# StractOrg/stract

Measured on AMD Instinct MI355X. Metric: HyperBall traversed edges/sec (GTEPS), higher is better.
Workload: dtype u8

## Files before the change

### include/hyperball.h

```cpp
#ifndef HYPERBALL_H
#define HYPERBALL_H

#include <stdint.h>

#ifdef __cplusplus
extern "C" {
#endif

#define HB_ABI_VERSION 6

#define HB_OK 0
#define HB_ERR_INVALID   (-1)
#define HB_ERR_NO_DEVICE (-2)
#define HB_ERR_HIP       (-3)
#define HB_ERR_NOMEM     (-4)
#define HB_ERR_RCCL      (-5)
#define HB_ERR_LIMIT     (-6)
#define HB_ERR_IO        (-7)


typedef struct hb_u128 {
    uint64_t lo;
    uint64_t hi;
} hb_u128;
// ... 258 lines not shown
    uint32_t rounds_run;
    uint64_t with_original;
    uint64_t filled[16];
    uint64_t unknown_orig;
    uint64_t unknown_keys;
    uint64_t no_seed;
    uint64_t seed_without_value;
    uint64_t results;
    uint64_t device_bytes;
    double   ms_total;
    double   ms_seed;
    double   ms_fill;
} hb_nearest_seed_stats;

int hb_nearest_seed(hb_ctx *ctx, const hb_nearest_seed_options *opt, hb_nearest_seed_stats *stats);
int hb_nearest_seed_count(hb_ctx *ctx, uint64_t *count);
int hb_nearest_seed_copy(hb_ctx *ctx, hb_u128 *ids, double *vals, uint64_t cap);
int hb_nearest_seed_all(hb_ctx *ctx, double *vals, uint64_t cap);
int hb_nearest_seed_top(hb_ctx *ctx, uint64_t k, hb_u128 *ids, double *vals, uint64_t *written);
int hb_nearest_seed_seeds(hb_ctx *ctx, hb_u128 *seed, uint8_t *has_seed, uint64_t cap);

int hb_rccl_unique_id(uint8_t out[128]);

#define HB_COLL_U8 0
#define HB_COLL_U32 1
#define HB_COLL_U64 2
#define HB_COLL_F64 3
#define HB_COLL_MAX 0
#define HB_COLL_SUM 1
typedef struct hb_collectives {
    void *user;
    int (*all_reduce)(void *user, void *buf, uint64_t count, int dtype, int op, void *stream);
    int (*all_gather)(void *user, const void *send, void *recv, uint64_t bytes_per_rank, void *stream);
    int (*broadcast)(void *user, void *buf, uint64_t bytes, int root, void *stream);
} hb_collectives;
int hb_set_collectives(hb_ctx *ctx, const hb_collectives *ops);
int hb_debug_staged_copy(void *dst, const void *src, uint64_t bytes, int to_device, void *stream);

int hb_pinned_alloc(uint64_t bytes, void **out);
void hb_pinned_free(void *p);

int hb_device_count(int *count);
int hb_device_name(const hb_ctx *ctx, char *name, uint64_t cap);
int hb_device_synchronize(hb_ctx *ctx);

int hb_debug_copy_registers(hb_ctx *ctx, uint8_t *out );
int hb_debug_copy_kahan(hb_ctx *ctx, double *sum, double *err);
int hb_debug_copy_sizes(hb_ctx *ctx, uint64_t *out);
int hb_debug_hll_size(hb_ctx *ctx, const uint8_t *regs, uint64_t count, uint64_t *out);
int hb_debug_state_hash(hb_ctx *ctx, uint64_t out[2]);
int hb_debug_copy_graph(hb_ctx *ctx, hb_u128 *ids, uint64_t *row_ptr, uint32_t *src);
int hb_debug_copy_plan(hb_ctx *ctx, uint64_t sizes[4], uint32_t *order, uint64_t *plan_row_ptr, uint32_t *plan_src,
                       uint64_t *level_begin);
int hb_debug_exchange(hb_ctx **ctxs, int count, int phase);
int hb_step_local(hb_ctx *ctx);
int hb_step_finish(hb_ctx *ctx, int *has_changes);

int hb_debug_h2d_rate(hb_ctx *ctx, const void *host, uint64_t bytes, int reps, double *gb_per_s);
int hb_debug_set_ingest_limits(hb_ctx *ctx, uint64_t max_records, uint64_t max_device_bytes, uint64_t chunk_records);

int hb_host_ingest(const hb_u128 *node_ids, uint64_t n, const hb_edge *edges, uint64_t m,
                   uint64_t *n_out, uint64_t *m_unique, uint64_t *m_eff, hb_u128 *ids,
                   uint64_t *row_ptr, uint32_t *src);
int hb_host_plan(uint64_t n, const uint64_t *row_ptr, const uint32_t *src, uint32_t flags,
                 uint32_t chunk, const uint32_t *tune , uint64_t sizes[4],
                 uint32_t *order, uint64_t *plan_row_ptr, uint32_t *plan_src, uint64_t *level_begin);
int hb_debug_tail_index(uint64_t n, const hb_u128 *sorted_ids, const uint32_t *dev_of, uint64_t n_pad, const hb_edge *records,
                        uint64_t count, uint64_t *ptr_out, uint32_t *to_out, uint64_t to_cap, uint64_t *to_len);

#ifdef __cplusplus
}
#endif
#endif
```

### stract_amd/_lib.py

```python
import ctypes
import os

os.environ.setdefault("OMP_WAIT_POLICY", "passive")

import numpy as np

_HERE = os.path.dirname(os.path.abspath(__file__))
LIB_PATH = os.environ.get("HB_LIB_PATH") or os.path.join(_HERE, "lib", "libhyperball.so")
LIB_EXP_PATH = os.environ.get("HB_LIB_PATH") or os.path.join(_HERE, "lib", "libhyperball_exp.so")

HB_OK = 0
HB_ERR_INVALID, HB_ERR_NO_DEVICE, HB_ERR_HIP, HB_ERR_NOMEM, HB_ERR_RCCL, HB_ERR_LIMIT, HB_ERR_IO = -1, -2, -3, -4, -5, -6, -7
HB_STORE_F64, HB_STORE_U64 = 0, 1
HB_COLL_U8, HB_COLL_U32, HB_COLL_U64, HB_COLL_F64 = 0, 1, 2, 3
HB_COLL_MAX, HB_COLL_SUM = 0, 1
HB_SKIPPED_REL_MASK = 0x6FED00

HB_FLAG_NO_FRONTIER = 0x01
HB_FLAG_NO_REORDER = 0x02
HB_FLAG_UNFUSED = 0x04
HB_FLAG_PASS_STATS = 0x08
HB_FLAG_NO_XCD_MAP = 0x20
HB_FLAG_NO_RCCL = 0x40
HB_FLAG_RCCL_SELF = 0x80
HB_FLAG_NO_SPARSE = 0x100
HB_FLAG_DEST_PARTITION = 0x200
HB_FLAG_HOST_INGEST = 0x400
HB_FLAG_HOST_PLAN = 0x800
HB_FLAG_CHANGED_ONLY = 0x1000
HB_FLAG_REFERENCE_TAIL = 0x2000
HB_FLAG_NO_INIT_PASS = 0x4000
HB_FLAG_ALL_RELS = 0x8000
HB_SAMPLE_MAX_LEVELS = 16

HB_X_TILE_EPILOGUE = 0x100
HB_X_SEED_3LAUNCH = 0x800
HB_X_NO_EDGE_OVERLAP = 0x1000
HB_X_BITMAP_SLOTWISE = 0x2000
HB_X_NO_STAGED_RESULTS = 0x4000
HB_X_SNAPSHOT_EVERY_PASS = 0x8000
HB_X_SHORT_FINAL_LIST = 0x10000
HB_X_ONE_SNAPSHOT = 0x20000
HB_X_NO_TAIL_PIPELINE = 0x100000
HB_X_TAIL_KERNEL = 0x200000
HB_X_TAIL_KERNEL_ANY = 0x400000
HB_X_FULL_INIT = 0x800000
HB_X_WIRE_64B = 0x1000000
HB_X_SCATTER_TRANSPOSE = 0x2000000
HB_X_SWEEP_ROUNDS = 0x4000000
HB_X_GENERIC_LEVEL1 = 0x8000000
HB_X_PROBE_NO_SIZE = 0x10000000

U128 = np.dtype([("lo", "<u8"), ("hi", "<u8")])
EDGE = np.dtype([("from", U128), ("to", U128), ("rel_flags", "<u8")])
assert U128.itemsize == 16 and EDGE.itemsize == 40


class HbOptions(ctypes.Structure):
    _fields_ = [
        ("struct_size", ctypes.c_uint32),
        ("device", ctypes.c_int32),
        ("flags", ctypes.c_uint32),
        ("chunk", ctypes.c_uint32),
        ("max_passes", ctypes.c_uint32),
        ("rank", ctypes.c_int32),
        ("world_size", ctypes.c_int32),
        ("rccl_id", ctypes.c_uint8 * 128),
        ("tune", ctypes.c_uint32 * 8),
    ]


class HbStats(ctypes.Structure):
    _fields_ = [
        ("n", ctypes.c_uint64),
        ("m_input", ctypes.c_uint64),
        ("m_unique", ctypes.c_uint64),
        ("m_eff", ctypes.c_uint64),
        ("passes", ctypes.c_uint64),
        ("results", ctypes.c_uint64),
        ("ms_ingest", ctypes.c_double),
        ("ms_plan", ctypes.c_double),
        ("ms_h2d", ctypes.c_double),
        ("ms_loop", ctypes.c_double),
        ("ms_loop_gpu", ctypes.c_double),
        ("ms_collective", ctypes.c_double),
        ("ms_d2h", ctypes.c_double),
        ("work_rows", ctypes.c_uint64),
        ("virtual_rows", ctypes.c_uint64),
        ("device_bytes", ctypes.c_uint64),
        ("virtual_edges", ctypes.c_uint64),
        ("levels", ctypes.c_uint64),
        ("level1_edges", ctypes.c_uint64),
        ("level1_rows", ctypes.c_uint64),
        ("direct_edges", ctypes.c_uint64),
        ("rows_with_in_edges", ctypes.c_uint64),
        ("wire_bytes", ctypes.c_uint64),
        ("ingest_peak_bytes", ctypes.c_uint64),
        ("pool_peak_bytes", ctypes.c_uint64),
        ("result_stages", ctypes.c_uint64),
        ("result_list", ctypes.c_uint64),
        ("pipelined_passes", ctypes.c_uint64),
        ("tail_kernel_passes", ctypes.c_uint64),
    ]

# ... 221 lines not shown
        return d


_P = ctypes.c_void_p
_U64 = ctypes.c_uint64
_SIGNATURES = [
    ("hb_abi_version", ctypes.c_int, []),
    ("hb_release_cached_memory", ctypes.c_int, [ctypes.c_void_p]),
    ("hb_create", ctypes.c_int, [ctypes.POINTER(HbOptions), ctypes.POINTER(_P)]),
    ("hb_destroy", None, [_P]),
    ("hb_last_error", ctypes.c_char_p, [_P]),
    ("hb_load_edges", ctypes.c_int, [_P, _P, _U64, _P, _U64]),
    ("hb_append_edges", ctypes.c_int, [_P, _P, _U64]),
    ("hb_finalize", ctypes.c_int, [_P, _P, _U64]),
    ("hb_discard_appended", ctypes.c_int, [_P]),
    ("hb_load_tail_edges", ctypes.c_int, [_P, _P, _U64]),
    ("hb_append_tail_edges", ctypes.c_int, [_P, _P, _U64]),
    ("hb_tail_segment_end", ctypes.c_int, [_P]),
    ("hb_debug_set_ingest_limits", ctypes.c_int, [_P, _U64, _U64, _U64]),
    ("hb_set_collectives", ctypes.c_int, [_P, _P]),
    ("hb_debug_staged_copy", ctypes.c_int, [_P, _P, _U64, ctypes.c_int, _P]),
    ("hb_pinned_alloc", ctypes.c_int, [_U64, ctypes.POINTER(ctypes.c_void_p)]),
    ("hb_pinned_free", None, [ctypes.c_void_p]),
    ("hb_debug_h2d_rate", ctypes.c_int, [_P, _P, _U64, ctypes.c_int, ctypes.POINTER(ctypes.c_double)]),
    ("hb_debug_tail_index", ctypes.c_int, [_U64, _P, _P, _U64, _P, _U64, _P, _P, _U64, ctypes.POINTER(ctypes.c_uint64)]),
    ("hb_load_dense", ctypes.c_int, [_P, _P, _U64, _P, _P, _U64]),
    ("hb_run", ctypes.c_int, [_P, ctypes.POINTER(HbStats)]),
    ("hb_begin", ctypes.c_int, [_P]),
    ("hb_step", ctypes.c_int, [_P, ctypes.POINTER(ctypes.c_int)]),
    ("hb_finish", ctypes.c_int, [_P]),
    ("hb_get_stats", ctypes.c_int, [_P, ctypes.POINTER(HbStats)]),
    ("hb_get_pass_stats", ctypes.c_int, [_P, _U64, ctypes.POINTER(HbPassStats)]),
    ("hb_result_count", ctypes.c_int, [_P, ctypes.POINTER(_U64)]),
    ("hb_result_copy", ctypes.c_int, [_P, _P, _P, _U64]),
    ("hb_result_ranks", ctypes.c_int, [_P, _P, _U64]),
    ("hb_result_top", ctypes.c_int, [_P, _U64, _P, _P, ctypes.POINTER(ctypes.c_uint64)]),
    ("hb_rccl_unique_id", ctypes.c_int, [_P]),
    ("hb_device_count", ctypes.c_int, [ctypes.POINTER(ctypes.c_int)]),
    ("hb_device_name", ctypes.c_int, [_P, ctypes.c_char_p, _U64]),
    ("hb_device_synchronize", ctypes.c_int, [_P]),
    ("hb_debug_copy_registers", ctypes.c_int, [_P, _P]),
    ("hb_debug_copy_kahan", ctypes.c_int, [_P, _P, _P]),
    ("hb_debug_copy_sizes", ctypes.c_int, [_P, _P]),
    ("hb_debug_hll_size", ctypes.c_int, [_P, _P, _U64, _P]),
    ("hb_debug_state_hash", ctypes.c_int, [_P, _P]),
    ("hb_debug_copy_graph", ctypes.c_int, [_P, _P, _P, _P]),
    ("hb_debug_copy_plan", ctypes.c_int, [_P, _P, _P, _P, _P, _P]),
    ("hb_debug_exchange", ctypes.c_int, [_P, ctypes.c_int, ctypes.c_int]),
    ("hb_step_local", ctypes.c_int, [_P]),
    ("hb_step_finish", ctypes.c_int, [_P, ctypes.POINTER(ctypes.c_int)]),
    ("hb_host_ingest", ctypes.c_int, [_P, _U64, _P, _U64, ctypes.POINTER(_U64), ctypes.POINTER(_U64),
                                      ctypes.POINTER(_U64), _P, _P, _P]),
    ("hb_host_plan", ctypes.c_int, [_U64, _P, _P, ctypes.c_uint32, ctypes.c_uint32, _P, _P, _P, _P, _P, _P]),
]
_SIGNATURES += [
    ("hbw_open", ctypes.c_int, [ctypes.c_char_p, ctypes.c_uint32, ctypes.POINTER(_P)]),
    ("hbw_close", None, [_P]),
    ("hbw_last_error", ctypes.c_char_p, [_P]),
    ("hbw_num_segments", ctypes.c_int, [_P, ctypes.POINTER(_U64)]),
    ("hbw_segment_info", ctypes.c_int, [_P, _U64, ctypes.c_char_p, ctypes.POINTER(_U64)]),
    ("hbw_total_rows", ctypes.c_int, [_P, ctypes.POINTER(_U64)]),
    ("hbw_read_host_edges", ctypes.c_int, [_P, _U64, _U64, _P]),
    ("hbw_read_page_edges", ctypes.c_int, [_P, _U64, _U64, _P]),
    ("hb_load_webgraph", ctypes.c_int, [_P, ctypes.c_char_p, ctypes.c_uint32]),
    ("hbw_debug_sstable", ctypes.c_int, [_P, _U64, ctypes.c_int, _P, _U64, _P, _U64, ctypes.POINTER(_U64)]),
    ("hbw_debug_crc32", ctypes.c_uint32, [_P, _U64]),
]
_SIGNATURES += [
    ("hbu_create", ctypes.c_int, [ctypes.c_int32, _U64, ctypes.POINTER(_P)]),
    ("hbu_destroy", None, [_P]),
    ("hbu_last_error", ctypes.c_char_p, [_P]),
    ("hbu_len", ctypes.c_int, [_P, ctypes.POINTER(_U64)]),
    ("hbu_batch_set", ctypes.c_int, [_P, _P, _P, _U64]),
    ("hbu_batch_get", ctypes.c_int, [_P, _P, _U64, _P, _P]),
    ("hbu_batch_upsert", ctypes.c_int, [_P, _P, _P, _U64, _P]),
    ("hbu_create_kind", ctypes.c_int, [ctypes.c_int32, _U64, ctypes.c_uint32, ctypes.POINTER(_P)]),
    ("hbu_kind", ctypes.c_int, [_P, ctypes.POINTER(ctypes.c_uint32), ctypes.POINTER(ctypes.c_uint32)]),
    ("hbu_batch_set_values", ctypes.c_int, [_P, _P, _P, _U64]),
    ("hbu_batch_get_values", ctypes.c_int, [_P, _P, _U64, _P, _P]),
    ("hbu_batch_upsert_values", ctypes.c_int, [_P, ctypes.c_uint32, _P, _P, _U64, _P]),
    ("hbu_wave_group_length", ctypes.c_uint32, []),
    ("hbu_clone", ctypes.c_int, [_P, ctypes.POINTER(_P)]),
    ("hbu_update_centralities", ctypes.c_int, [_P, _P, _P, _P, _P, _U64, _U64, ctypes.POINTER(_U64)]),
    ("hbu_update_counters", ctypes.c_int, [_P, _P, _P, _P, _U64, _P]),
    ("hbu_update_distances", ctypes.c_int, [_P, _P, _P, _P, _U64, _P, _P, ctypes.POINTER(_U64)]),
    ("hbu_graph_create", ctypes.c_int, [ctypes.c_int32, _P, _U64, _P, _P, _U64, _U64, ctypes.POINTER(_P)]),
    ("hbu_graph_len", ctypes.c_int, [_P, ctypes.POINTER(_U64), ctypes.POINTER(_U64)]),
    ("hbu_graph_destroy", None, [_P]),
    ("hbu_bloom_num_bits", _U64, [_U64, ctypes.c_double]),
    ("hbu_filter_create", ctypes.c_int, [ctypes.c_int32, ctypes.c_uint32, _U64, ctypes.POINTER(_P)]),
    ("hbu_filter_destroy", None, [_P]),
    ("hbu_filter_clear", ctypes.c_int, [_P]),
    ("hbu_filter_fill", ctypes.c_int, [_P]),
    ("hbu_filter_insert", ctypes.c_int, [_P, _P, _U64]),
    ("hbu_filter_contains", ctypes.c_int, [_P, _P, _U64, _P]),
    ("hbu_filter_union", ctypes.c_int, [_P, _P]),
    ("hbu_filter_count", ctypes.c_int, [_P, ctypes.POINTER(_U64)]),
    ("hbu_filter_export_bits", ctypes.c_int, [_P, _P]),
    ("hbu_filter_import_bits", ctypes.c_int, [_P, _P]),
    ("hbu_filter_export_ids", ctypes.c_int, [_P, _P, _U64, ctypes.POINTER(_U64)]),
    ("hbu_setup_counters", ctypes.c_int, [_P, _P, _P, _P]),
    ("hbu_round_counters", ctypes.c_int, [_P, _P, _P, _P, _P, ctypes.POINTER(_U64), ctypes.POINTER(_U64), ctypes.POINTER(_U64)]),
    ("hbu_round_distances", ctypes.c_int, [_P, _P, _P, _P, _P, ctypes.POINTER(_U64), ctypes.POINTER(_U64)]),
    ("hbu_round_centralities", ctypes.c_int, [_P, _P, _P, _P, _P, _P, _U64, ctypes.POINTER(_U64), ctypes.POINTER(_U64)]),
    ("hbu_export", ctypes.c_int, [_P, _P, _P, _U64, ctypes.POINTER(_U64)]),
    ("hbu_fold_harmonic", ctypes.c_int, [_P, _P, ctypes.c_double, ctypes.c_uint32, ctypes.POINTER(_U64), ctypes.POINTER(_U64)]),
# ... 542 lines not shown
        if rc != HB_OK:
            raise HyperballError(rc, err.value.decode(errors="replace"))

    def top(self, k):
        cnt = ctypes.c_uint64(0)
        self._check(self.lib.hb_result_count(self.h, ctypes.byref(cnt)))
        k = min(int(k), cnt.value)
        ids = np.zeros(k, dtype=U128)
        vals = np.zeros(k, dtype=np.float64)
        w = ctypes.c_uint64(0)
        self._check(self.lib.hb_result_top(self.h, k, _ptr(ids), _ptr(vals), ctypes.byref(w)))
        return ids[:w.value], vals[:w.value]

    def n(self):
        return self.stats()["n"]

    def registers(self):
        out = np.zeros((self.n(), 64), dtype=np.uint8)
        self._check(self.lib.hb_debug_copy_registers(self.h, _ptr(out)))
        return out

    def kahan(self):
        n = self.n()
        s = np.zeros(n, dtype=np.float64)
        e = np.zeros(n, dtype=np.float64)
        self._check(self.lib.hb_debug_copy_kahan(self.h, _ptr(s), _ptr(e)))
        return s, e

    def sizes(self):
        out = np.zeros(self.n(), dtype=np.uint64)
        self._check(self.lib.hb_debug_copy_sizes(self.h, _ptr(out)))
        return out

    def state_hash(self):
        out = np.zeros(2, dtype=np.uint64)
        self._check(self.lib.hb_debug_state_hash(self.h, _ptr(out)))
        return int(out[0]), int(out[1])

    def hll_size(self, regs):
        regs = np.ascontiguousarray(regs, dtype=np.uint8).reshape(-1, 64)
        out = np.zeros(len(regs), dtype=np.uint64)
        self._check(self.lib.hb_debug_hll_size(self.h, _ptr(regs), len(regs), _ptr(out)))
        return out

    def plan(self):
        sizes = np.zeros(4, dtype=np.uint64)
        self._check(self.lib.hb_debug_copy_plan(self.h, _ptr(sizes), None, None, None, None))
        n_pad, nv, slen, levels = (int(x) for x in sizes)
        order = np.zeros(n_pad, dtype=np.uint32)
        prp = np.zeros(n_pad + nv + 1, dtype=np.uint64)
        psrc = np.zeros(slen, dtype=np.uint32)
        lb = np.zeros(levels + 1, dtype=np.uint64)
        self._check(self.lib.hb_debug_copy_plan(self.h, _ptr(sizes), _ptr(order), _ptr(prp), _ptr(psrc), _ptr(lb)))
        return dict(order=order, row_ptr=prp, src=psrc, level_begin=lb, n_pad=n_pad, nv=nv)

    def graph(self):
        st = self.stats()
        ids = np.zeros(st["n"], dtype=U128)
        row_ptr = np.zeros(st["n"] + 1, dtype=np.uint64)
        src = np.zeros(st["m_eff"], dtype=np.uint32)
        self._check(self.lib.hb_debug_copy_graph(self.h, _ptr(ids), _ptr(row_ptr), _ptr(src)))
        return ids, row_ptr, src


def rccl_unique_id():
    buf = (ctypes.c_uint8 * 128)()
    rc = load().hb_rccl_unique_id(buf)
    if rc != HB_OK:
        raise HyperballError(rc, (load().hb_last_error(None) or b"").decode())
    return bytes(buf)


def host_ingest(edges, node_ids=None):
    lib = load()
    edges = np.ascontiguousarray(edges, dtype=EDGE)
    nn = 0
    if node_ids is not None:
        node_ids = np.ascontiguousarray(node_ids, dtype=U128)
        nn = len(node_ids)
    n, mu, me = ctypes.c_uint64(0), ctypes.c_uint64(0), ctypes.c_uint64(0)
    rc = lib.hb_host_ingest(_ptr(node_ids), nn, _ptr(edges), len(edges), ctypes.byref(n), ctypes.byref(mu),
                            ctypes.byref(me), None, None, None)
    if rc != HB_OK:
        raise HyperballError(rc, (lib.hb_last_error(None) or b"").decode())
    ids = np.zeros(n.value, dtype=U128)
    row_ptr = np.zeros(n.value + 1, dtype=np.uint64)
    src = np.zeros(me.value, dtype=np.uint32)
    rc = lib.hb_host_ingest(_ptr(node_ids), nn, _ptr(edges), len(edges), ctypes.byref(n), ctypes.byref(mu),
                            ctypes.byref(me), _ptr(ids), _ptr(row_ptr), _ptr(src))
    if rc != HB_OK:
        raise HyperballError(rc, (lib.hb_last_error(None) or b"").decode())
    return ids, row_ptr, src, mu.value


def host_plan(row_ptr, src, flags=0, chunk=0, tune=()):
    lib = load()
    row_ptr = np.ascontiguousarray(row_ptr, dtype=np.uint64)
    src = np.ascontiguousarray(src, dtype=np.uint32)
    n = len(row_ptr) - 1
    sizes = np.zeros(4, dtype=np.uint64)
    tn = np.zeros(8, dtype=np.uint32)
    tn[:len(tune)] = tune
    rc = lib.hb_host_plan(n, _ptr(row_ptr), _ptr(src), flags, chunk, _ptr(tn), _ptr(sizes), None, None, None, None)
    if rc != HB_OK:
        raise HyperballError(rc, (lib.hb_last_error(None) or b"").decode())
    n_pad, nv, slen, levels = (int(x) for x in sizes)
    order = np.zeros(n_pad, dtype=np.uint32)
    prp = np.zeros(n_pad + nv + 1, dtype=np.uint64)
    psrc = np.zeros(slen, dtype=np.uint32)
    lb = np.zeros(levels + 1, dtype=np.uint64)
    rc = lib.hb_host_plan(n, _ptr(row_ptr), _ptr(src), flags, chunk, _ptr(tn), _ptr(sizes), _ptr(order), _ptr(prp),
                          _ptr(psrc), _ptr(lb))
    if rc != HB_OK:
        raise HyperballError(rc, (lib.hb_last_error(None) or b"").decode())
    world = int(tn[7]) if tn[7] > 1 else 1
    if world == 1:
        order = order[:n]
    return dict(order=order, row_ptr=prp, src=psrc, level_begin=lb, n_pad=n_pad, nv=nv, slice=n_pad // world)
```

### stract_amd/csrc/hb_api.hip

```cpp
#include "hb_guard_alloc.h"
#include "hb_pool.h"
#include <hip/hip_runtime.h>
#include <rccl/rccl.h>

#include <algorithm>
#include <cmath>
#include <cstdio>
#include <cstring>
#include <string>
#include <thread>
#include <vector>

#include "hb_internal.h"
#include "hb_experiments.h"
#include "hb_kernels.hip.h"
#include "hb_walk.hip.h"
#include "hb_sample.hip.h"
#include "hb_bfs.hip.h"
#include "hb_betweenness.hip.h"
#include "hb_similarity.hip.h"
#include "hb_nearest_seed.hip.h"
#ifdef HB_EXPERIMENTS
#include "hb_experiments.hip.h"
#endif
// ... 18 lines not shown
    {
        reset(o.release());
        return *this;
    }
    DevPtr(const DevPtr &) = delete;
    DevPtr &operator=(const DevPtr &) = delete;
    ~DevPtr() { reset(); }
    T *get() const { return p; }
    explicit operator bool() const { return p != nullptr; }
    T *release()
    {
        T *q = p;
        p = nullptr;
        return q;
    }
    void reset(T *q = nullptr)
    {
        if (p) (void)hipFree(p);
        p = q;
    }
    hipError_t alloc(size_t count)
    {
        reset();
        return hipMalloc((void **)&p, count * sizeof(T));
    }

private:
    T *p = nullptr;
};

struct OwnedCsr {
    DeviceCsr d;
    OwnedCsr() = default;
    OwnedCsr(OwnedCsr &&o) noexcept : d(o.d) { o.d = DeviceCsr{}; }
    OwnedCsr(const OwnedCsr &) = delete;
    OwnedCsr &operator=(const OwnedCsr &) = delete;
    ~OwnedCsr() { reset(); }
    void reset()
    {
        for (void *q : {(void *)d.d_row_ptr, (void *)d.d_src, (void *)d.d_id_lo})
            if (q) (void)hipFree(q);
        d = DeviceCsr{};
    }
};
}

struct GraphDeviceState {
    uint64_t *d_row_ptr = nullptr;
    uint32_t *d_src = nullptr;
    uint16_t *d_src_jp = nullptr;
    bool level0_all_real = false;
    uint32_t *d_virt_rows = nullptr;
    uint16_t *d_self_jp = nullptr;
    uint4 *d_regs[2] = {nullptr, nullptr};
    uint4 *d_part = nullptr;
    uint32_t *d_bits[2] = {nullptr, nullptr};
    uint32_t *d_kdirty = nullptr;
    double *d_ksum = nullptr, *d_kerr = nullptr;
    uint64_t *d_size = nullptr;
    uint64_t *d_idlow = nullptr;
    uint32_t *d_dev_of = nullptr;
    uint32_t *d_sid_of = nullptr;
    uint32_t *d_outdeg = nullptr;
    unsigned long long *d_counters = nullptr;
    double *d_raw = nullptr, *d_bias = nullptr;
    uint8_t *d_lc = nullptr;
    uint64_t *d_out_ptr = nullptr;
    uint32_t *d_out_rows = nullptr;
    uint32_t *d_touch = nullptr;
    uint32_t *d_seeds = nullptr, *d_heavy = nullptr;
    unsigned int *d_sparse_counts = nullptr;
    bool sparse_ok = false;
    uint4 *d_pack = nullptr;
    uint32_t *d_wpop = nullptr;
    uint64_t *d_wprefix = nullptr;
    uint32_t *d_lbits = nullptr, *d_lbits_all = nullptr, *d_ubits = nullptr;
    bool ubits_valid = false;
    unsigned long long *d_rank_cnt = nullptr;
    uint32_t *d_tl_changed[2] = {nullptr, nullptr}, *d_tl_vchanged[2] = {nullptr, nullptr}, *d_tl_dirty[2] = {nullptr, nullptr};
    uint32_t *d_tl_work = nullptr, *d_tl_count = nullptr;
    bool tl_valid = false;
    uint64_t *d_tail_ptr = nullptr;
    uint32_t *d_tail_to = nullptr;
    uint64_t tail_count = 0;
    std::vector<uint64_t> tail_keys;
    std::vector<TailDoc> tail_open;
    bool tail_dirty = false;
    TailIndex *tail_index = nullptr;
    uint32_t *d_bloom = nullptr;
    unsigned long long *d_bloom_ones = nullptr;
    uint32_t *d_list = nullptr;
    double *d_out = nullptr;
    double *h_out = nullptr;
    uint64_t h_out_len = 0;
    uint64_t out_len = 0;
    uint32_t *d_cid_of = nullptr;
    std::vector<uint64_t> h_in_bits;
    struct ResultSync {
        bool on = false;
        bool valid = false;
        uint64_t changed_since = 0;
        uint32_t stages = 0;
        double *d_sent = nullptr;
        uint32_t *d_sid = nullptr;
        double *d_val = nullptr;
        unsigned long long *d_count = nullptr;
// ... 241 lines not shown
    for (void *q : {(void *)c->h_out, (void *)c->rs.h_sid, (void *)c->rs.h_val, (void *)c->rs.h_count})
        if (q) (void)hipHostFree(q);
    tail_index_free(c->tail_index);
    static_cast<GraphDeviceState &>(*c) = GraphDeviceState{};
    c->stats.device_bytes = 0;
}

template <class T>
void copy_in(const T *from, T *to)
{
    if (from) std::memcpy(to, from, from->struct_size ? std::min<size_t>(from->struct_size, sizeof(T)) : sizeof(T));
}
template <class T>
void copy_out(T *to, T &from)
{
    if (!to) return;
    const size_t sz = to->struct_size ? std::min<size_t>(to->struct_size, sizeof(T)) : sizeof(T);
    from.struct_size = (uint32_t)sz;
    std::memcpy(to, &from, sz);
}

int refuse_stale_error(hb_ctx *c, const char *who)
{
    const hipError_t stale = hipGetLastError();
    if (stale != hipSuccess) return fail(c, HB_ERR_HIP, std::string("stale HIP error before ") + who + ": " + hipGetErrorString(stale));
    return HB_OK;
}

bool find_sid(const hb_ctx *c, const hb_u128 &id, uint32_t *sid)
{
    const auto it = std::lower_bound(c->g.ids.begin(), c->g.ids.end(), id, u128_less);
    if (it == c->g.ids.end() || !u128_eq(*it, id)) return false;
    *sid = (uint32_t)(it - c->g.ids.begin());
    return true;
}

int plan_rows_word_aligned(hb_ctx *c, const char *who)
{
    const Plan &p = c->plan;
    if (p.n_pad % 32 || std::any_of(p.level_begin.begin(), p.level_begin.end(), [](uint64_t b) { return b % 32 != 0; }))
        return fail(c, HB_ERR_INVALID, std::string(who) + ": unexpected plan layout (a level does not begin on a 32-row word)");
    return HB_OK;
}

PlanTune plan_tune(uint32_t chunk, const uint32_t *tune)
{
    PlanTune t;
    t.chunk = chunk ? chunk : kDefaultChunk;
    if (tune) {
        if (tune[3] == 1) t.band_w = 0;
        else if (tune[3] >= 4 && tune[3] < 31) t.band_w = 1u << tune[3];
        if (tune[4]) t.minc = tune[4];
        if (tune[5]) t.direct_max = tune[5];
    }
    return t;
}

bool multi_rank(const hb_ctx *c) { return c->opt.world_size > 1; }
bool xbit(const hb_ctx *c, uint32_t bits) { return (HB_XBITS(c->opt.tune[1]) & bits) != 0; }
unsigned grid_blocks(const hb_ctx *c, uint64_t groups, uint64_t per_cu, uint64_t floor = 0)
{
    return (unsigned)std::max<uint64_t>(std::min<uint64_t>(groups, (uint64_t)c->num_cu * per_cu), floor);
}
bool linked(const hb_ctx *c) { return c->comm != nullptr || c->coll.all_reduce != nullptr; }

#define HB_COLL(call)                 \
    do {                              \
        const int rc_coll_ = (call);  \
        if (rc_coll_) return rc_coll_; \
    } while (0)
int coll_dtype(ncclDataType_t dt) { return dt == ncclUint8 ? HB_COLL_U8 : dt == ncclUint32 ? HB_COLL_U32 : dt == ncclUint64 ? HB_COLL_U64 : HB_COLL_F64; }
uint64_t coll_size(ncclDataType_t dt) { return dt == ncclUint8 ? 1 : dt == ncclUint32 ? 4 : 8; }
int coll_all_reduce(hb_ctx *c, void *buf, uint64_t count, ncclDataType_t dt, ncclRedOp_t op, hipStream_t s)
{
    if (c->comm) {
        HB_NCCL(ncclAllReduce(buf, buf, count, dt, op, c->comm, s));
        return HB_OK;
    }
    if (c->coll.all_reduce(c->coll.user, buf, count, coll_dtype(dt), op == ncclMax ? HB_COLL_MAX : HB_COLL_SUM, (void *)s))
        return fail(c, HB_ERR_RCCL, "the caller's all_reduce (hb_set_collectives) failed");
    return HB_OK;
}
int coll_all_gather(hb_ctx *c, const void *send, void *recv, uint64_t count, ncclDataType_t dt, hipStream_t s)
{
    if (c->comm) {
        HB_NCCL(ncclAllGather(send, recv, count, dt, c->comm, s));
        return HB_OK;
    }
    if (c->coll.all_gather(c->coll.user, send, recv, count * coll_size(dt), (void *)s))
        return fail(c, HB_ERR_RCCL, "the caller's all_gather (hb_set_collectives) failed");
    return HB_OK;
}
int coll_broadcast(hb_ctx *c, void *buf, uint64_t count, ncclDataType_t dt, int root, hipStream_t s)
{
    if (c->comm) {
        HB_NCCL(ncclBroadcast(buf, buf, count, dt, root, c->comm, s));
        return HB_OK;
    }
    if (c->coll.broadcast(c->coll.user, buf, count * coll_size(dt), root, (void *)s))
        return fail(c, HB_ERR_RCCL, "the caller's broadcast (hb_set_collectives) failed");
    return HB_OK;
}
int coll_group_start(hb_ctx *c)
{
    if (c->comm) HB_NCCL(ncclGroupStart());
    return HB_OK;
// ... 965 lines not shown
```

### stract_amd/csrc/hb_api_debug.inc

```
int hb_debug_copy_registers(hb_ctx *c, uint8_t *out)
{
    return guarded(c, [&]() -> int {
        if (!c || !out) return HB_ERR_INVALID;
        if (c->rows != RowsOf::HyperBall) return fail(c, HB_ERR_INVALID, "call hb_begin first");
        int rc = set_device(c);
        if (rc) return rc;
        if ((rc = ensure_initial_state(c))) return rc;
        const uint64_t n = c->plan.n;
        if (!n) return HB_OK;
        DevPtr<uint4> tmp;
        HB_HIP(tmp.alloc(n * 4));
        unsigned blocks = (unsigned)((n * 4 + 255) / 256);
        hipLaunchKernelGGL(hbk::gather_rows_kernel, dim3(blocks), dim3(256), 0, c->stream, (const uint4 *)c->d_regs[c->cur],
                           (const uint32_t *)c->d_dev_of, n, tmp.get());
        HB_HIP_AS("", hipMemcpyAsync(out, tmp.get(), n * 64, hipMemcpyDeviceToHost, c->stream));
        HB_HIP_AS("", hipStreamSynchronize(c->stream));
        return HB_OK;
    });
}

int hb_debug_copy_kahan(hb_ctx *c, double *sum, double *err)
{
    return guarded(c, [&]() -> int {
        if (!c) return HB_ERR_INVALID;
// ... 83 lines not shown
        hipLaunchKernelGGL(hbk::state_hash_kernel, dim3(blocks), dim3(256), 0, c->stream, (const uint4 *)c->d_regs[c->cur],
                           (const double *)c->d_ksum, (const double *)c->d_kerr, (const uint32_t *)c->d_dev_of, n, cnt);
        HB_HIP(hipGetLastError());
        std::vector<unsigned long long> h(hbk::kCounterWords);
        HB_HIP(hipMemcpyAsync(h.data(), cnt, hbk::kCounterWords * sizeof(unsigned long long), hipMemcpyDeviceToHost, c->stream));
        HB_HIP(hipStreamSynchronize(c->stream));
        for (int s = 0; s < hbk::kStripes; s++) {
            out[0] += h[4 * s];
            out[1] += h[4 * s + 1];
        }
        if (multi_rank(c)) out[1] = 0;
        return HB_OK;
    });
}

int hb_debug_copy_graph(hb_ctx *c, hb_u128 *ids, uint64_t *row_ptr, uint32_t *src)
{
    return guarded(c, [&]() -> int {
        if (!c) return HB_ERR_INVALID;
        if (!c->loaded) return fail(c, HB_ERR_INVALID, "no graph loaded");
        const uint64_t n = c->g.ids.size();
        if ((row_ptr || src) && c->g.row_ptr.size() != n + 1)
            return fail(c, HB_ERR_LIMIT, "the reduced graph is kept on the host only up to 2^26 edges (or with HB_FLAG_HOST_PLAN)");
        if (ids && n) std::memcpy(ids, c->g.ids.data(), n * sizeof(hb_u128));
        if (row_ptr) std::memcpy(row_ptr, c->g.row_ptr.data(), (n + 1) * sizeof(uint64_t));
        if (src && !c->g.src.empty()) std::memcpy(src, c->g.src.data(), c->g.src.size() * sizeof(uint32_t));
        return HB_OK;
    });
}

int hb_debug_copy_plan(hb_ctx *c, uint64_t sizes[4], uint32_t *order, uint64_t *plan_row_ptr, uint32_t *plan_src, uint64_t *level_begin)
{
    return guarded(c, [&]() -> int {
        if (!c || !sizes) return HB_ERR_INVALID;
        if (!c->loaded) return fail(c, HB_ERR_INVALID, "no graph loaded");
        int rc = set_device(c);
        if (rc) return rc;
        const Plan &p = c->plan;
        const uint64_t rows_total = p.n_pad + p.nv;
        sizes[0] = p.n_pad;
        sizes[1] = p.nv;
        sizes[2] = c->plan_entries;
        sizes[3] = p.level_begin.size() ? p.level_begin.size() - 1 : 0;
        if (order && p.n_pad) HB_HIP(hipMemcpyAsync(order, c->d_sid_of, p.n_pad * sizeof(uint32_t), hipMemcpyDeviceToHost, c->stream));
        if (plan_row_ptr) HB_HIP(hipMemcpyAsync(plan_row_ptr, c->d_row_ptr, (rows_total + 1) * sizeof(uint64_t), hipMemcpyDeviceToHost, c->stream));
        if (plan_src && c->plan_entries)
            HB_HIP(hipMemcpyAsync(plan_src, c->d_src, c->plan_entries * sizeof(uint32_t), hipMemcpyDeviceToHost, c->stream));
        HB_HIP(hipStreamSynchronize(c->stream));
        if (level_begin) std::memcpy(level_begin, p.level_begin.data(), p.level_begin.size() * sizeof(uint64_t));
        return HB_OK;
    });
}

int hb_host_ingest(const hb_u128 *node_ids, uint64_t n, const hb_edge *edges, uint64_t m, uint64_t *n_out,
                   uint64_t *m_unique, uint64_t *m_eff, hb_u128 *ids, uint64_t *row_ptr, uint32_t *src)
{
    return guarded(nullptr, [&]() -> int {
        hb_ctx *c = nullptr;
        DenseGraph g;
        std::string e = ingest_edges(node_ids, n, edges, m, &g);
        if (!e.empty()) return fail(c, HB_ERR_INVALID, e);
        const uint64_t nn = g.ids.size();
        if (n_out) *n_out = nn;
        if (m_unique) *m_unique = g.m_unique;
        if (m_eff) *m_eff = g.src.size();
        if (ids && nn) std::memcpy(ids, g.ids.data(), nn * sizeof(hb_u128));
        if (row_ptr) std::memcpy(row_ptr, g.row_ptr.data(), (nn + 1) * sizeof(uint64_t));
        if (src && !g.src.empty()) std::memcpy(src, g.src.data(), g.src.size() * sizeof(uint32_t));
        return HB_OK;
    });
}

int hb_host_plan(uint64_t n, const uint64_t *row_ptr, const uint32_t *src, uint32_t flags, uint32_t chunk,
                 const uint32_t *tune, uint64_t sizes[4], uint32_t *order, uint64_t *plan_row_ptr, uint32_t *plan_src,
                 uint64_t *level_begin)
{
    return guarded(nullptr, [&]() -> int {
        hb_ctx *c = nullptr;
        if (!sizes || (n && !row_ptr)) return fail(c, HB_ERR_INVALID, "NULL argument");
        std::vector<uint32_t> outdeg;
        const bool reorder = !(flags & HB_FLAG_NO_REORDER);
        static const uint64_t zero = 0;
        if (n == 0) row_ptr = &zero;
        if (reorder) count_out_degree(row_ptr, src, n, &outdeg);
        Plan p;
        PlanTune pt = plan_tune(chunk, tune);
        if (tune && tune[7] > 1) pt.world = tune[7];
        pt.xcd_map = !(flags & HB_FLAG_NO_XCD_MAP);
        std::string e = build_plan(n, row_ptr, src, outdeg, reorder, pt, &p);
        if (!e.empty()) return fail(c, HB_ERR_LIMIT, e);
        sizes[0] = p.n_pad;
        sizes[1] = p.nv;
        sizes[2] = p.src.size();
        sizes[3] = p.level_begin.size() ? p.level_begin.size() - 1 : 0;
        if (order && p.n_pad) std::memcpy(order, p.order.data(), p.n_pad * sizeof(uint32_t));
        if (plan_row_ptr) std::memcpy(plan_row_ptr, p.row_ptr.data(), p.row_ptr.size() * sizeof(uint64_t));
        if (plan_src && !p.src.empty()) std::memcpy(plan_src, p.src.data(), p.src.size() * sizeof(uint32_t));
        if (level_begin) std::memcpy(level_begin, p.level_begin.data(), p.level_begin.size() * sizeof(uint64_t));
        return HB_OK;
    });
}

int hb_debug_tail_index(uint64_t n, const hb_u128 *sorted_ids, const uint32_t *dev_of, uint64_t n_pad, const hb_edge *records,
                        uint64_t count, uint64_t *ptr_out, uint32_t *to_out, uint64_t to_cap, uint64_t *to_len)
{
    return guarded(nullptr, [&]() -> int {
        hb_ctx *c = nullptr;
        if ((n && (!sorted_ids || !dev_of)) || (count && !records) || !ptr_out || !to_len) return fail(c, HB_ERR_INVALID, "NULL argument");
        TailIndex *tix = n ? tail_index_build(sorted_ids, n) : nullptr;
        std::vector<uint64_t> keys, ptr;
        std::vector<uint32_t> to;
        std::vector<TailDoc> open;
        std::string e = tail_collect(tix, n, records, count, &open);
        if (e.empty()) e = tail_close_segment(tix, sorted_ids, dev_of, &open, &keys);
        tail_index_free(tix);
        if (e.empty()) e = build_tail_csr(&keys, n_pad, &ptr, &to);
        if (!e.empty()) return fail(c, HB_ERR_NOMEM, e);
        std::memcpy(ptr_out, ptr.data(), (n_pad + 1) * sizeof(uint64_t));
        *to_len = to.size();
        if (to_out && !to.empty()) std::memcpy(to_out, to.data(), std::min<uint64_t>(to.size(), to_cap) * sizeof(uint32_t));
        return HB_OK;
    });
}

int hb_debug_exchange(hb_ctx **ctxs, int count, int phase)
{
    return guarded(nullptr, [&]() -> int {
        if (!ctxs || count < 1 || !ctxs[0]) return HB_ERR_INVALID;
        hb_ctx *c = ctxs[0];
        for (int i = 0; i < count; i++) {
            hb_ctx *o = ctxs[i];
            if (!o) return fail(c, HB_ERR_INVALID, "NULL context");
            if (o->plan.n_pad != c->plan.n_pad || o->device != c->device || dest_mode(o) != dest_mode(c))
                return fail(c, HB_ERR_INVALID, "contexts differ in size, device or partition mode");
            if (phase == 0 && !o->pending_local)
                return fail(c, HB_ERR_INVALID, "every context must be between hb_step_local and hb_step_finish");
            if (dest_mode(c) && (o->opt.rank != i || o->opt.world_size != count))
                return fail(c, HB_ERR_INVALID, "destination partition: ctxs[i] must be rank i of `count`");
        }
        int rc = set_device(c);
        if (rc) return rc;
        for (int i = 0; i < count; i++) HB_HIP(hipStreamSynchronize(ctxs[i]->stream));
        const Plan &p = c->plan;
        const uint64_t S = c->slice_rows;
        if (phase == 1) {
            if (!dest_mode(c)) return HB_OK;
            for (int i = 0; i < count; i++)
                for (int j = 0; j < count; j++)
                    if (i != j && S)
                        HB_HIP(hipMemcpyAsync(ctxs[i]->d_ksum + (uint64_t)j * S, ctxs[j]->d_ksum + (uint64_t)j * S, S * sizeof(double),
                                              hipMemcpyDeviceToDevice, c->stream));
// ... 92 lines not shown
```

### stract_amd/csrc/hb_api_load.inc

```
bool device_plan(const hb_ctx *c) { return !(c->opt.flags & HB_FLAG_HOST_PLAN); }
bool deferred_times(const hb_ctx *c);

int keep_owned(hb_ctx *c, DeviceCsr *csr)
{
    if (!dest_mode(c)) return HB_OK;
    const uint64_t world = (uint64_t)std::max(c->opt.world_size, 1), rank = (uint64_t)c->opt.rank, n = c->g.ids.size();
    if (c->g.row_ptr.size() == n + 1 && n) keep_owned_rows(&c->g, world, rank);
    if (csr && csr->d_row_ptr) {
        const std::string e = gpu_keep_owned_rows((void *)c->stream, csr, n, world, rank);
        if (!e.empty()) return fail(c, e.find("memory") != std::string::npos ? HB_ERR_NOMEM : HB_ERR_HIP, e);
    }
    return HB_OK;
}

__global__ __launch_bounds__(256) void idlow_kernel(const uint64_t *lo_by_sid, const uint32_t *order, uint64_t n_pad, uint64_t *idlow)
{
    const uint64_t d = (uint64_t)blockIdx.x * 256 + threadIdx.x;
    if (d >= n_pad) return;
    const uint32_t s = order[d];
    idlow[d] = s == kNone ? 0ull : lo_by_sid[s];
}

template <class T>
T *adopt(hb_ctx *c, DevPtr<T> &b, size_t bytes)
// ... 72 lines not shown
    c->rows = RowsOf::Nobody;
    c->image = Image::None;
    c->run_open = false;
    free_graph_buffers(c);
    c->stats.n = n;
    c->stats.m_input = c->g.m_input;
    c->stats.m_unique = c->g.m_unique;
    c->stats.m_eff = m_eff;
    double t0 = now_ms();
    const bool on_device = device_plan(c);
    c->rs.on = n && !multi_rank(c) && !linked(c) && !ref_tail(c) && !xbit(c, HB_X_NO_STAGED_RESULTS) && (n >= (1u << 20) || xbit(c, HB_X_SNAPSHOT_EVERY_PASS));
    c->rs.cap = c->rs.on ? (xbit(c, HB_X_SHORT_FINAL_LIST) ? 16 : n / 8 + 4096) : 0;
    HostResultBuffers hostbuf;
    hostbuf.start(c->device, n, c->rs.cap);
    if (!in.d.d_row_ptr) in.reset();
    if (!on_device && n && c->g.row_ptr.size() != n + 1) {
        try {
            c->g.row_ptr.resize(n + 1);
            c->g.src.resize(m_eff);
        } catch (const std::bad_alloc &) {
            return fail(c, HB_ERR_NOMEM, "out of host memory for the reduced graph");
        }
        HB_HIP(hipMemcpyAsync(c->g.row_ptr.data(), in.d.d_row_ptr, (n + 1) * sizeof(uint64_t), hipMemcpyDeviceToHost, c->stream));
        if (m_eff) HB_HIP(hipMemcpyAsync(c->g.src.data(), in.d.d_src, m_eff * sizeof(uint32_t), hipMemcpyDeviceToHost, c->stream));
        HB_HIP(hipStreamSynchronize(c->stream));
    }
    if (n && !in.d.d_src) {
        HB_HIP(hipMalloc((void **)&in.d.d_src, std::max<uint64_t>(m_eff, 1) * sizeof(uint32_t)));
        if (m_eff) HB_HIP(hipMemcpyAsync(in.d.d_src, c->g.src.data(), m_eff * sizeof(uint32_t), hipMemcpyHostToDevice, c->stream));
        if (on_device) {
            HB_HIP(hipMalloc((void **)&in.d.d_row_ptr, (n + 1) * sizeof(uint64_t)));
            HB_HIP(hipMemcpyAsync(in.d.d_row_ptr, c->g.row_ptr.data(), (n + 1) * sizeof(uint64_t), hipMemcpyHostToDevice, c->stream));
        }
        in.d.m = m_eff;
    }
    bool reorder = !(c->opt.flags & HB_FLAG_NO_REORDER);
    if (multi_rank(c) && !linked(c)) reorder = false;
    DevPtr<uint64_t> d_lo(in.d.d_id_lo);
    in.d.d_id_lo = nullptr;
    DevPtr<uint32_t> d_deg;
    if (n) {
        HB_HIP(d_deg.alloc(n));
        HB_HIP(hipMemsetAsync(d_deg.get(), 0, n * sizeof(uint32_t), c->stream));
        if (m_eff) {
            const unsigned blocks = grid_blocks(c, (m_eff + 255) / 256, 16);
            hipLaunchKernelGGL(hbk::histogram_kernel, dim3(blocks), dim3(256), 0, c->stream, (const uint32_t *)in.d.d_src, m_eff, d_deg.get());
            HB_HIP(hipGetLastError());
        }
        if (linked(c)) HB_COLL(coll_all_reduce(c, d_deg.get(), n, ncclUint32, ncclSum, c->stream));
    }
    PlanTune pt = plan_tune(c->opt.chunk, c->opt.tune);
    pt.xcd_map = !(c->opt.flags & HB_FLAG_NO_XCD_MAP);
    if (dest_mode(c)) pt.world = (uint32_t)std::max(c->opt.world_size, 1);
    {
        const uint64_t w = pt.world > 1 ? pt.world : 1;
        const uint64_t n_pad_pre = (((n + w - 1) / w + kRowAlign - 1) / kRowAlign * kRowAlign) * w;
        int rc0;
        if ((rc0 = dev_alloc(c, &c->d_regs[0], n_pad_pre * 4))) return rc0;
        if ((rc0 = dev_alloc(c, &c->d_regs[1], n_pad_pre * 4))) return rc0;
    }
    std::vector<uint32_t> outdeg;
    DevicePlan dp;
    DevPtr<uint64_t> dp_row_ptr;
    DevPtr<uint32_t> dp_src, dp_order, dp_dev_of, dp_outdeg;
    if (on_device) {
        std::string perr = gpu_build_plan((void *)c->stream, n, in.d.d_row_ptr, in.d.d_src, d_deg.get(), reorder, pt, &c->plan, &dp);
        dp_row_ptr.reset(dp.d_row_ptr); dp_src.reset(dp.d_src); dp_order.reset(dp.d_order); dp_dev_of.reset(dp.d_dev_of); dp_outdeg.reset(dp.d_outdeg_dev);
        if (!perr.empty()) {
            (void)hipGetLastError();
            return fail(c, perr.find("memory") != std::string::npos ? HB_ERR_NOMEM : (perr.find("exhausted") != std::string::npos ? HB_ERR_LIMIT : HB_ERR_HIP), perr);
        }
    } else {
        outdeg.assign(n, 0);
        if (n) {
            HB_HIP(hipMemcpyAsync(outdeg.data(), d_deg.get(), n * sizeof(uint32_t), hipMemcpyDeviceToHost, c->stream));
            HB_HIP(hipStreamSynchronize(c->stream));
        }
        static const uint64_t zero = 0;
        std::string perr = build_plan(n, n ? c->g.row_ptr.data() : &zero, c->g.src.data(), outdeg, reorder, pt, &c->plan);
        if (!perr.empty()) return fail(c, perr.find("memory") != std::string::npos ? HB_ERR_NOMEM : HB_ERR_LIMIT, perr);
    }
    in.reset();
    c->stats.ms_plan = now_ms() - t0;
    const Plan &p = c->plan;
    const uint64_t rows_total = p.n_pad + p.nv;
    const uint64_t src_len = on_device ? dp.src_len : p.src.size();
    c->plan_entries = src_len;
    c->stats.work_rows = rows_total;
    c->stats.virtual_rows = p.nv;
    c->stats.levels = p.level_begin.size() > 1 ? p.level_begin.size() - 1 : 0;
    c->stats.level1_edges = p.level1_edges;
    c->stats.level1_rows = p.level1_rows;
    c->stats.direct_edges = p.direct_edges;
    c->stats.rows_with_in_edges = p.rows_with_in_edges;

    t0 = now_ms();
    const bool trace_state = std::getenv("HB_TRACE_INGEST") != nullptr;
    double t_lap = t0;
    auto lap = [&](const char *what) {
        if (!trace_state) return;
        (void)hipStreamSynchronize(c->stream);
        std::fprintf(stderr, "[hb state] %-34s %8.1f ms\n", what, now_ms() - t_lap);
        t_lap = now_ms();
    };
    c->bits_words = (rows_total + 31) / 32 + 2;
    int rc;
    if (on_device) {
        c->d_row_ptr = adopt(c, dp_row_ptr, (rows_total + 2) * sizeof(uint64_t));
        c->d_src = adopt(c, dp_src, (src_len + 4) * sizeof(uint32_t));
        c->d_sid_of = adopt(c, dp_order, std::max<uint64_t>(p.n_pad, 64) * sizeof(uint32_t));
        c->d_dev_of = adopt(c, dp_dev_of, std::max<uint64_t>(n, 64) * sizeof(uint32_t));
        c->d_outdeg = adopt(c, dp_outdeg, std::max<uint64_t>(p.n_pad, 64) * sizeof(uint32_t));
        c->m_global = dp.m_global;
    } else {
        if ((rc = dev_alloc(c, &c->d_row_ptr, rows_total + 1))) return rc;
        if ((rc = dev_alloc(c, &c->d_src, src_len + 4))) return rc;
        if ((rc = dev_alloc(c, &c->d_dev_of, n))) return rc;
        if ((rc = dev_alloc(c, &c->d_sid_of, p.n_pad))) return rc;
        if ((rc = dev_alloc(c, &c->d_outdeg, p.n_pad))) return rc;
    }
    if ((rc = dev_alloc(c, &c->d_part, p.nv * 4))) return rc;
    if ((rc = dev_alloc(c, &c->d_bits[0], c->bits_words))) return rc;
    if ((rc = dev_alloc(c, &c->d_bits[1], c->bits_words))) return rc;
    if ((rc = dev_alloc(c, &c->d_kdirty, p.n_pad / 32 + 2))) return rc;
    const uint64_t world = linked(c) ? (uint64_t)c->opt.world_size : 1;
    c->slice_rows = dest_mode(c) ? p.slice : ((p.n_pad + world - 1) / world + 63) / 64 * 64;
    c->ksum_len = std::max<uint64_t>(c->slice_rows * (dest_mode(c) ? (uint64_t)std::max(c->opt.world_size, 1) : world), p.n_pad);
    if ((rc = dev_alloc(c, &c->d_ksum, c->ksum_len))) return rc;
    if ((rc = dev_alloc(c, &c->d_kerr, p.n_pad))) return rc;
    if ((rc = dev_alloc(c, &c->d_size, p.n_pad))) return rc;
    if ((rc = dev_alloc(c, &c->d_idlow, p.n_pad))) return rc;
    if ((rc = dev_alloc(c, &c->d_counters, ((size_t)c->max_passes + 1) * hbk::kCounterWords))) return rc;
    if ((rc = dev_alloc(c, &c->d_raw, HLL64_TABLE_LEN))) return rc;
    if ((rc = dev_alloc(c, &c->d_bias, HLL64_TABLE_LEN))) return rc;
    if ((rc = dev_alloc(c, &c->d_lc, 68))) return rc;
    if ((rc = dev_alloc(c, &c->d_out, n))) return rc;
    if (c->rs.on) {
        if ((rc = dev_alloc(c, &c->rs.d_sent, p.n_pad))) return rc;
        if ((rc = dev_alloc(c, &c->rs.d_sid, c->rs.cap))) return rc;
        if ((rc = dev_alloc(c, &c->rs.d_val, c->rs.cap))) return rc;
        if ((rc = dev_alloc(c, &c->rs.d_count, 2))) return rc;
        if ((rc = dev_alloc(c, &c->rs.d_kept, hbk::kCounterWords))) return rc;
    }
    if (deferred_times(c)) {
        while (c->ev_pool.size() < 32) {
            hb_ctx::EvSet es{};
            for (auto &e : es.e)
                if (hipEventCreate(&e) != hipSuccess) return fail(c, HB_ERR_HIP, "hipEventCreate failed");
            c->ev_pool.push_back(es);
        }
    }

    lap("allocations");
    uint8_t lc[68];
    if (!build_lc_table(lc)) return fail(c, HB_ERR_INVALID, "host libm log() too close to a rounding boundary for the linear-counting table");
    HB_HIP(hipMemcpyAsync(c->d_raw, HLL64_RAW_ESTIMATE, sizeof(HLL64_RAW_ESTIMATE), hipMemcpyHostToDevice, c->stream));
    HB_HIP(hipMemcpyAsync(c->d_bias, HLL64_BIAS, sizeof(HLL64_BIAS), hipMemcpyHostToDevice, c->stream));
    HB_HIP(hipMemcpyAsync(c->d_lc, lc, 68, hipMemcpyHostToDevice, c->stream));
    if (!on_device) {
        c->stats.virtual_edges = p.row_ptr.empty() ? 0 : p.row_ptr[rows_total] - p.row_ptr[p.n_pad];
        HB_HIP(hipMemcpyAsync(c->d_row_ptr, p.row_ptr.data(), (rows_total + 1) * sizeof(uint64_t), hipMemcpyHostToDevice, c->stream));
        if (!p.src.empty())
            HB_HIP(hipMemcpyAsync(c->d_src, p.src.data(), p.src.size() * sizeof(uint32_t), hipMemcpyHostToDevice, c->stream));
        if (p.n_pad)
            HB_HIP(hipMemcpyAsync(c->d_sid_of, p.order.data(), p.n_pad * sizeof(uint32_t), hipMemcpyHostToDevice, c->stream));
        std::vector<uint32_t> outdeg_dev(p.n_pad, 0);
        c->m_global = 0;
        for (uint64_t d = 0; d < p.n_pad; d++)
            if (p.order[d] != kNone) {
                outdeg_dev[d] = outdeg[p.order[d]];
                c->m_global += outdeg[p.order[d]];
            }
        if (p.n_pad)
            HB_HIP(hipMemcpyAsync(c->d_outdeg, outdeg_dev.data(), p.n_pad * sizeof(uint32_t), hipMemcpyHostToDevice, c->stream));
        if (n) HB_HIP(hipMemcpyAsync(c->d_dev_of, p.dev_of.data(), n * sizeof(uint32_t), hipMemcpyHostToDevice, c->stream));
        HB_HIP(hipStreamSynchronize(c->stream));
    } else {
        uint64_t ends[2] = {0, 0};
        HB_HIP(hipMemcpyAsync(&ends[0], c->d_row_ptr + p.n_pad, sizeof(uint64_t), hipMemcpyDeviceToHost, c->stream));
        HB_HIP(hipMemcpyAsync(&ends[1], c->d_row_ptr + rows_total, sizeof(uint64_t), hipMemcpyDeviceToHost, c->stream));
        HB_HIP(hipStreamSynchronize(c->stream));
        c->stats.virtual_edges = ends[1] - ends[0];
    }
    lap("tables / plan arrays");
    c->out_len = n;
    c->d_cid_of = c->d_sid_of;
    if (c->rs.on && n) {
        DevPtr<uint32_t> d_flags;
        DevPtr<uint64_t> d_cpos;
        DevPtr<unsigned long long> d_words;
        const uint64_t nw = (n + 63) / 64;
        HB_HIP(d_flags.alloc(n + 1));
        HB_HIP(d_cpos.alloc(n + 2));
        HB_HIP(d_words.alloc(nw));
        if ((rc = dev_alloc(c, &c->d_cid_of, p.n_pad))) return rc;
        HB_HIP(hipMemsetAsync(d_flags.get(), 0, (n + 1) * sizeof(uint32_t), c->stream));
        const unsigned blocks = grid_blocks(c, (p.n_pad + 255) / 256, 16);
        hipLaunchKernelGGL(hbk::in_flags_kernel, dim3(blocks), dim3(256), 0, c->stream, (const uint64_t *)c->d_row_ptr, (const uint32_t *)c->d_sid_of, p.n_pad, d_flags.get());
        HB_HIP(hipGetLastError());
        const std::string e = device_prefix((void *)c->stream, d_flags.get(), n, d_cpos.get());
        if (!e.empty()) return fail(c, HB_ERR_HIP, e);
        hipLaunchKernelGGL(hbk::cid_of_kernel, dim3(blocks), dim3(256), 0, c->stream, (const uint64_t *)c->d_row_ptr, (const uint32_t *)c->d_sid_of,
                           (const uint64_t *)d_cpos.get(), p.n_pad, c->d_cid_of);
        HB_HIP(hipGetLastError());
        hipLaunchKernelGGL(hbk::pack_flags_kernel, dim3(grid_blocks(c, (nw + 3) / 4, 16)), dim3(256), 0, c->stream,
                           (const uint32_t *)d_flags.get(), n, d_words.get());
        HB_HIP(hipGetLastError());
        uint64_t n_c = 0;
        c->h_in_bits.assign(nw, 0);
        HB_HIP(hipMemcpyAsync(&n_c, d_cpos.get() + n, sizeof(uint64_t), hipMemcpyDeviceToHost, c->stream));
        HB_HIP(hipMemcpyAsync(c->h_in_bits.data(), d_words.get(), nw * sizeof(uint64_t), hipMemcpyDeviceToHost, c->stream));
        HB_HIP(hipStreamSynchronize(c->stream));
        if (n_c != p.rows_with_in_edges)
            return fail(c, HB_ERR_INVALID, "result image: " + std::to_string(n_c) + " nodes with in-edges counted on the device, the plan says " + std::to_string(p.rows_with_in_edges));
        c->out_len = n_c;
        lap("compact result image (cid per row, host bitmap)");
    }
    if (n) {
        if (!d_lo) {
            uvec<uint64_t> lo(n);
            host_gather_id_lo(c->g.ids.data(), n, lo.data());
            HB_HIP(d_lo.alloc(n));
            HB_HIP(hipMemcpyAsync(d_lo.get(), lo.data(), n * sizeof(uint64_t), hipMemcpyHostToDevice, c->stream));
            HB_HIP(hipStreamSynchronize(c->stream));
        }
        hipLaunchKernelGGL(idlow_kernel, dim3((unsigned)((p.n_pad + 255) / 256)), dim3(256), 0, c->stream, (const uint64_t *)d_lo.get(),
                           (const uint32_t *)c->d_sid_of, p.n_pad, c->d_idlow);
        HB_HIP(hipGetLastError());
        HB_HIP(hipStreamSynchronize(c->stream));
    }
    lap("id_low");
    if (src_len && !(c->opt.flags & HB_FLAG_NO_INIT_PASS)) {
        if ((rc = dev_alloc(c, &c->d_src_jp, src_len + 4))) return rc;
        const unsigned blocks = grid_blocks(c, (src_len + 255) / 256, 16);
        if ((rc = dev_alloc(c, &c->d_self_jp, p.n_pad + 4))) return rc;
        hipLaunchKernelGGL(hbk::self_jp_kernel, dim3(grid_blocks(c, (p.n_pad + 255) / 256, 16)), dim3(256), 0, c->stream,
                           (const uint64_t *)c->d_idlow, (const uint32_t *)c->d_sid_of, p.n_pad, c->d_self_jp);
        HB_HIP(hipGetLastError());
        hipLaunchKernelGGL(hbk::src_jp_kernel, dim3(blocks), dim3(256), 0, c->stream, (const uint32_t *)c->d_src, src_len, (const uint16_t *)c->d_self_jp, p.n_pad,
                           c->d_src_jp);
        HB_HIP(hipGetLastError());
        if ((rc = dev_alloc(c, &c->d_virt_rows, c->bits_words + 4))) return rc;
        unsigned long long *d_l0 = c->d_counters + 8, h_l0 = ~0ull;
        HB_HIP(hipMemsetAsync(d_l0, 0, sizeof(unsigned long long), c->stream));
        const uint64_t l0_lo = p.level_begin.size() > 1 ? p.level_begin[0] : 0, l0_hi = p.level_begin.size() > 1 ? p.level_begin[1] : 0;
        hipLaunchKernelGGL(hbk::virt_rows_kernel, dim3(grid_blocks(c, (rows_total + 255) / 256, 16)), dim3(256), 0, c->stream,
                           (const uint64_t *)c->d_row_ptr, (const uint32_t *)c->d_src, rows_total, p.n_pad, c->d_virt_rows, l0_lo, l0_hi, d_l0);
        HB_HIP(hipGetLastError());
        HB_HIP(hipMemcpyAsync(&h_l0, d_l0, sizeof(h_l0), hipMemcpyDeviceToHost, c->stream));
        HB_HIP(hipStreamSynchronize(c->stream));
        c->level0_all_real = h_l0 == 0;
        HB_HIP(hipStreamSynchronize(c->stream));
    }
    lap("self_jp / src_jp");
    {
        unsigned long long *d_bad = c->d_counters;
        unsigned long long h_bad[4] = {0, 0, 0, 0};
        HB_HIP(hipMemsetAsync(d_bad, 0, sizeof(h_bad), c->stream));
        if (rows_total) {
            const unsigned blocks = grid_blocks(c, (rows_total * 4 + 255) / 256, 16);
            hipLaunchKernelGGL(hbk::validate_plan_kernel, dim3(blocks), dim3(256), 0, c->stream, (const uint64_t *)c->d_row_ptr, (const uint32_t *)c->d_src,
                               rows_total, p.n_pad, src_len, d_bad);
            HB_HIP(hipGetLastError());
        }
        HB_HIP(hipMemcpyAsync(h_bad, d_bad, sizeof(h_bad), hipMemcpyDeviceToHost, c->stream));
        HB_HIP(hipStreamSynchronize(c->stream));
        if (h_bad[0] | h_bad[1] | h_bad[2] | h_bad[3])
            return fail(c, HB_ERR_INVALID, "work layout failed its structural check: " + std::to_string(h_bad[0]) + " bad row pointers, " +
                                               std::to_string(h_bad[1]) + " source ids out of range, " + std::to_string(h_bad[2]) +
                                               " rows of mixed source kind, " + std::to_string(h_bad[3]) + " virtual rows reading upwards");
    }
    lap("layout check");
    if ((rc = build_sparse_support(c))) return rc;
    lap("transposed work-row graph");
    decltype(c->plan.row_ptr)().swap(c->plan.row_ptr);
    decltype(c->plan.src)().swap(c->plan.src);
    {
        size_t free_b = 0, total_b = 0;
        if (hipMemGetInfo(&free_b, &total_b) == hipSuccess && free_b < total_b / 4) HB_POOL_TRIM();
    }
    lap("pool trim");
    hostbuf.join();
    if (!hostbuf.ok) return fail(c, HB_ERR_NOMEM, "hipHostMalloc(result buffers) failed");
    c->h_out = hostbuf.h_out;
    c->h_out_len = n;
    c->rs.h_sid = hostbuf.h_sid;
    c->rs.h_val = hostbuf.h_val;
    c->rs.h_count = hostbuf.h_count;
    hostbuf.release();
    lap("pinned result buffers (allocated + touched beside the load)");
    if ((rc = warm_kernels(c))) return rc;
    lap("kernels warmed");
    if (n) {
        HB_HIP(hipEventRecord(c->ev[kEvStart], c->stream));
        if (c->rs.on) {
            HB_HIP(hipEventRecord(c->rs_ready, c->stream));
            HB_HIP(hipStreamWaitEvent(c->rs_stream, c->rs_ready, 0));
            HB_HIP(hipMemcpyAsync(c->h_out, c->d_out, c->out_len * sizeof(double), hipMemcpyDeviceToHost, c->rs_stream));
            HB_HIP(hipEventRecord(c->rs_copied, c->rs_stream));
            HB_HIP(hipMemcpyAsync(c->rs.h_sid, c->rs.d_sid, c->rs.cap * sizeof(uint32_t), hipMemcpyDeviceToHost, c->stream));
            HB_HIP(hipMemcpyAsync(c->rs.h_val, c->rs.d_val, c->rs.cap * sizeof(double), hipMemcpyDeviceToHost, c->stream));
            HB_HIP(hipMemcpyAsync(c->rs.h_count, c->rs.d_count, sizeof(unsigned long long), hipMemcpyDeviceToHost, c->stream));
            HB_HIP(hipStreamWaitEvent(c->stream, c->rs_copied, 0));
        } else {
            HB_HIP(hipMemcpyAsync(c->h_out, c->d_out, c->out_len * sizeof(double), hipMemcpyDeviceToHost, c->stream));
        }
        HB_HIP(hipMemcpyAsync(c->h_counters, c->d_counters, hbk::kCounterWords * sizeof(unsigned long long), hipMemcpyDeviceToHost, c->stream));
        for (int k = 0; k < 2; k++) {
            HB_HIP(hipMemcpyAsync(c->h_slot + (size_t)k * hbk::kCounterWords, c->d_counters, hbk::kCounterWords * sizeof(unsigned long long), hipMemcpyDeviceToHost, c->stream));
            HB_HIP(hipEventRecord(c->slot_done[k], c->stream));
        }
        HB_HIP(hipEventRecord(c->ev[kEvEnd], c->stream));
        HB_HIP(hipEventSynchronize(c->slot_done[1]));
        if (c->rs.on) {
            (void)hipEventQuery(c->rs_copied);
            (void)hipGetLastError();
        }
        HB_HIP(hipStreamSynchronize(c->stream));
        float ms_warm = 0.f;
        HB_HIP(hipEventElapsedTime(&ms_warm, c->ev[kEvStart], c->ev[kEvEnd]));
    }
    HB_HIP(hipStreamSynchronize(c->stream));
    if (c->rs_stream) HB_HIP(hipStreamSynchronize(c->rs_stream));
// ... 20 lines not shown
```

### stract_amd/csrc/hb_api_pass.inc

```
using PassKernel = void (*)(const hbk::PassParams);
using SweepKernel = void (*)(const hbk::SweepParams);

template <bool REAL, bool FUSED, bool STATS, bool INIT, bool EPI4>
PassKernel dense_by_unroll(int unroll)
{
    if constexpr (!INIT) {
        if (unroll == 1) return hbk::pass_kernel<REAL, FUSED, STATS, 1, INIT, EPI4>;
    }
    if (unroll == 2) return hbk::pass_kernel<REAL, FUSED, STATS, 2, INIT, EPI4>;
    return hbk::pass_kernel<REAL, FUSED, STATS, 4, INIT, EPI4>;
}
template <bool REAL, bool FUSED>
PassKernel dense_kernel_of(bool stats, int unroll, bool init, bool epi4)
{
    if (stats) return dense_by_unroll<REAL, FUSED, true, false, false>(unroll);
    if constexpr (REAL && FUSED) {
        if (epi4) return init ? dense_by_unroll<true, true, false, true, true>(unroll) : dense_by_unroll<true, true, false, false, true>(unroll);
    }
    return init ? dense_by_unroll<REAL, FUSED, false, true, false>(unroll) : dense_by_unroll<REAL, FUSED, false, false, false>(unroll);
}
PassKernel dense_kernel(bool real, bool fused, bool stats, int unroll, bool init, bool epi4)
{
    init = init && unroll != 1;
    if (real && fused) return dense_kernel_of<true, true>(stats, unroll, init, epi4);
// ... 28 lines not shown
{
    const int unroll = (int)(c->opt.tune[1] & HB_TUNE1_UNROLL);
    return (unroll == 1 || unroll == 2 || unroll == 4) ? unroll : (real ? 2 : 4);
}
bool pass0_streams_initial_registers(const hb_ctx *c)
{
    return c->d_src_jp != nullptr && c->d_self_jp != nullptr && !(c->opt.flags & HB_FLAG_NO_INIT_PASS) && pass_unroll(c, true) != 1;
}

void launch_pass(hb_ctx *c, const hbk::PassParams &pp, bool real, bool frontier, bool fused, int level = -1)
{
    const bool stats = (c->opt.flags & HB_FLAG_PASS_STATS) != 0;
    const uint64_t ntiles = (pp.row_hi - pp.row_lo + 63) / 64;
    if (ntiles == 0) return;
    const bool init = c->t == 0 && !frontier && pass0_streams_initial_registers(c);
    uint32_t bpc = real ? (c->opt.tune[0] & 0xFFu) : ((c->opt.tune[0] >> 8) & 0xFFu);
    if (!bpc) bpc = real ? (frontier ? 32u : 64u) : (frontier ? 5u : (init ? 8u : 2u));
    PassKernel kernel;
    unsigned blocks;
    if (init && !real && level == 0 && c->level0_all_real && !stats && !xbit(c, HB_X_GENERIC_LEVEL1)) {
        kernel = hbk::init_level1_kernel;
        blocks = grid_blocks(c, ntiles, 8);
    } else {
        blocks = grid_blocks(c, ntiles, bpc);
        if (pp.xcd_map) blocks = std::max((blocks + 7) / 8 * 8, 8u);
        kernel = frontier ? bitmap_kernel(real, fused, stats, !xbit(c, HB_X_BITMAP_SLOTWISE))
                          : dense_kernel(real, fused, stats, pass_unroll(c, real), init, !xbit(c, HB_X_TILE_EPILOGUE));
    }
    hipLaunchKernelGGL(kernel, dim3(blocks), dim3(256), 0, c->stream, pp);
}

bool lean_pass0(const hb_ctx *c)
{
    return pass0_streams_initial_registers(c) && !unfused(c) && !multi_rank(c) && !linked(c) && !dest_mode(c) && !(c->opt.flags & HB_FLAG_PASS_STATS) &&
           !xbit(c, HB_X_FULL_INIT);
}
int launch_full_init(hb_ctx *c)
{
    const Plan &p = c->plan;
    if (!p.n_pad) return HB_OK;
    const unsigned blocks = (unsigned)((p.n_pad * 4 + 255) / 256);
    hipLaunchKernelGGL(hbk::init_kernel, dim3(blocks), dim3(256), 0, c->stream, c->d_idlow, (const uint32_t *)c->d_sid_of, p.n_pad, c->d_regs[0],
                       c->d_regs[1], c->d_ksum, c->d_kerr, c->d_size, c->d_bits[0], c->d_kdirty, c->d_raw, c->d_bias, c->d_lc);
    HB_HIP(hipGetLastError());
    return HB_OK;
}
int ensure_initial_state(hb_ctx *c)
{
    if (!c->lean_init) return HB_OK;
    c->lean_init = false;
    return launch_full_init(c);
}

hbk::PassParams make_params(hb_ctx *c)
{
    const Plan &p = c->plan;
    hbk::PassParams pp{};
    pp.row_ptr = c->d_row_ptr;
    pp.src = c->d_src;
    pp.src_jp = c->d_src_jp;
    pp.rd = c->d_regs[c->cur];
    pp.wr = c->d_regs[c->cur ^ 1];
    pp.part = c->d_part;
    pp.bits_rd = c->d_bits[c->cur];
    pp.bits_wr = c->d_bits[c->cur ^ 1];
    pp.kdirty = c->d_kdirty;
    pp.ksum = c->d_ksum;
    pp.kerr = c->d_kerr;
    pp.size = c->d_size;
    pp.counters = c->d_counters + (size_t)hbk::kCounterWords * c->t;
    pp.outdeg = c->d_outdeg;
    pp.raw = c->d_raw;
    pp.bias = c->d_bias;
    pp.lc = c->d_lc;
    pp.n = p.n;
    pp.n_pad = p.n_pad;
    pp.rows_total = p.n_pad + p.nv;
    if (linked(c) || dest_mode(c)) {
        pp.slice_lo = (uint64_t)c->opt.rank * c->slice_rows;
        pp.slice_hi = std::min<uint64_t>(pp.slice_lo + c->slice_rows, p.n_pad);
    } else {
        pp.slice_lo = 0;
        pp.slice_hi = p.n_pad;
    }
    pp.t_plus_1 = (double)(c->t + 1);
    pp.rd_init = nullptr;
    pp.self_jp = c->d_self_jp;
    pp.virt_rows = c->d_virt_rows;
    pp.xflags = xbit(c, HB_X_PROBE_NO_SIZE) ? 1u : 0u;
    return pp;
}

bool changed_only(const hb_ctx *c) { return dest_mode(c) && (c->opt.flags & HB_FLAG_CHANGED_ONLY); }
uint64_t packed_row_bytes(const hb_ctx *c) { return xbit(c, HB_X_WIRE_64B) ? 64 : 48; }
bool deferred_times(const hb_ctx *c) { return changed_only(c) && linked(c); }
int pass_events(hb_ctx *c, hipEvent_t **out)
{
    if (!deferred_times(c)) {
        *out = c->pipelined ? c->ev_ring[c->t & 3].e : c->ev;
        return HB_OK;
    }
    while (c->ev_pool.size() <= c->t) {
        hb_ctx::EvSet es{};
        for (auto &e : es.e)
            if (hipEventCreate(&e) != hipSuccess) return fail(c, HB_ERR_HIP, "hipEventCreate failed");
        c->ev_pool.push_back(es);
    }
    *out = c->ev_pool[c->t].e;
    return HB_OK;
}
int read_pass_times(hb_ctx *c, hipEvent_t *E, PassEvent end, hb_pass_stats *ps)
{
    HB_HIP(hipEventElapsedTime(&ps->ms_gpu, E[kEvStart], E[end]));
    HB_HIP(hipEventElapsedTime(&ps->ms_main, E[kEvLevels], E[kEvMerge]));
    if (ps->mode == 2 || (ps->mode < 2 && c->plan.level_begin.size() > 1)) HB_HIP(hipEventElapsedTime(&ps->ms_level1, E[kEvStart], E[kEvLevel1]));
    return HB_OK;
}
int resolve_pass_times(hb_ctx *c)
{
    for (uint64_t t : c->pending_times) {
        if (t >= c->pstats.size() || t >= c->ev_pool.size()) continue;
        hipEvent_t *E = c->ev_pool[t].e;
        hb_pass_stats &ps = c->pstats[t];
        HB_HIP(hipEventSynchronize(E[kEvCollective]));
        const int rc = read_pass_times(c, E, kEvCollective, &ps);
        if (rc) return rc;
        HB_HIP(hipEventElapsedTime(&ps.ms_collective, E[kEvMerge], E[kEvCollective]));
    }
    c->pending_times.clear();
    return HB_OK;
}
bool edge_overlap(const hb_ctx *c)
{
    return linked(c) && !dest_mode(c) && !ref_tail(c) && !(c->opt.flags & HB_FLAG_CHANGED_ONLY) && !xbit(c, HB_X_NO_EDGE_OVERLAP) && c->comm_stream;
}
bool edge_changed_only(const hb_ctx *c)
{
    return (c->opt.flags & HB_FLAG_CHANGED_ONLY) && !dest_mode(c) && !ref_tail(c) && (multi_rank(c) || linked(c));
}

int ensure_pack_buffers(hb_ctx *c)
{
// ... 289 lines not shown

int sweep_pass(hb_ctx *c, const hbk::PassParams &pp, hipEvent_t *E)
{
    const Plan &p = c->plan;
    hbk::SweepParams sp = make_sweep_params(c, pp, (unsigned)(c->t & 1), c->spec_guard);
    launch_sweep_seeding(c, sp, c->last_changed <= 4096 && !xbit(c, HB_X_SEED_3LAUNCH));
    HB_HIP(hipEventRecord(E[kEvLevel1], c->stream));
    const bool by_rounds = xbit(c, HB_X_SWEEP_ROUNDS);
    auto launch_rows = [&](bool real, uint64_t lo, uint64_t hi) {
        if (hi <= lo) return;
        sp.p.row_lo = lo;
        sp.p.row_hi = hi;
        const uint64_t waves = (hi - lo + 2047) / 2048;
        hipLaunchKernelGGL(sweep_rows_kernel_for(real, by_rounds), dim3(grid_blocks(c, (waves + 3) / 4, 4, 1)), dim3(256), 0, c->stream, sp);
    };
    for (size_t l = 0; l + 1 < p.level_begin.size(); l++) launch_rows(false, p.level_begin[l], p.level_begin[l + 1]);
    HB_HIP(hipEventRecord(E[kEvLevels], c->stream));
    launch_rows(true, 0, p.n_pad);
    HB_HIP(hipEventRecord(E[kEvMerge], c->stream));
    return HB_OK;
}

int level_pass(hb_ctx *c, hbk::PassParams pp, hipEvent_t *E, bool frontier, bool fused, bool lean)
{
    const Plan &p = c->plan;
    for (size_t l = 0; l + 1 < p.level_begin.size(); l++) {
        pp.row_lo = p.level_begin[l];
        pp.row_hi = p.level_begin[l + 1];
        pp.xcd_map = (l == 0 && p.xcd_groups == 8) ? 1 : 0;
        for (int x = 0; x < 8; x++) {
            pp.xcd_lo[x] = p.xcd_begin[x];
            pp.xcd_hi[x] = p.xcd_begin[x + 1];
        }

#ifdef HB_EXPERIMENTS
        const uint32_t lds_tile = std::min<uint32_t>(c->opt.tune[7], 2048u);
        if (l == 0 && !frontier && lds_tile && !(c->opt.flags & HB_FLAG_PASS_STATS) && !multi_rank(c)) {
            const uint64_t ntiles = (pp.row_hi - pp.row_lo + 63) / 64;
            const size_t lds = (size_t)lds_tile * 64;
            const uint64_t per_cu = std::max<uint64_t>(1, std::min<uint64_t>(8, (160 * 1024) / (lds + 1024)));
            unsigned blocks = grid_blocks(c, ntiles, per_cu);
            if (pp.xcd_map) blocks = std::max((blocks + 7) / 8 * 8, 8u);
            if (lds > 48 * 1024)
                HB_HIP(hipFuncSetAttribute((const void *)hbk::hub_lds_tile_kernel, hipFuncAttributeMaxDynamicSharedMemorySize, (int)lds));
            if (ntiles) hipLaunchKernelGGL(hbk::hub_lds_tile_kernel, dim3(blocks), dim3(256), lds, c->stream, pp, lds_tile);
        } else
#endif
        {
            launch_pass(c, pp, false, frontier, false, (int)l);
        }
        if (l == 0) HB_HIP(hipEventRecord(E[kEvLevel1], c->stream));
    }
    pp.xcd_map = 0;
    HB_HIP(hipEventRecord(E[kEvLevels], c->stream));
    pp.row_lo = dest_mode(c) ? pp.slice_lo : 0;
    pp.row_hi = dest_mode(c) ? pp.slice_hi : p.n_pad;
    if (edge_changed_only(c)) {
        int rc = edge_co_alloc(c);
        if (rc) return rc;
        pp.lbits = c->d_lbits;
        c->ubits_valid = false;
    }
    c->ov_ranges = 0;
    if (edge_overlap(c) && p.n_pad >= 64ull * hb_ctx::kOverlap) {
        const uint64_t tiles = p.n_pad / 64;
        for (int k = 0; k <= hb_ctx::kOverlap; k++) c->ov_lo[k] = tiles * (uint64_t)k / hb_ctx::kOverlap * 64;
        c->ov_ranges = hb_ctx::kOverlap;
        for (int k = 0; k < hb_ctx::kOverlap; k++) {
            pp.row_lo = c->ov_lo[k];
            pp.row_hi = c->ov_lo[k + 1];
            launch_pass(c, pp, true, frontier, fused);
            HB_HIP(hipEventRecord(c->ov_merged[k], c->stream));
        }
    } else {
        if (lean) pp.rd_init = c->d_regs[c->cur];
        launch_pass(c, pp, true, frontier, fused);
    }
    HB_HIP(hipEventRecord(E[kEvMerge], c->stream));
    return HB_OK;
}

int bloom_frontier_prelude(hb_ctx *c)
{
    const Plan &p = c->plan;
    hipLaunchKernelGGL(hbk::bloom_frontier_kernel, dim3((unsigned)(p.n_pad / 256 + 1)), dim3(256), 0, c->stream, (const uint32_t *)c->d_bloom,
                       (const uint64_t *)c->d_idlow, (const uint32_t *)c->d_sid_of, p.n_pad, c->bloom_bits, c->d_bits[c->cur]);
    HB_HIP(hipGetLastError());
    return HB_OK;
}

int step_local(hb_ctx *c)
{
    if (!c->run_open) return fail(c, HB_ERR_INVALID, "hb_step*: call hb_begin first");
    c->tl_valid = false;
    c->tl_declined = false;
    if (c->pending_local) return fail(c, HB_ERR_INVALID, "hb_step_local called twice");
    if (c->t >= c->max_passes) return fail(c, HB_ERR_LIMIT, "max_passes exceeded");
    c->cur_mode = c->pipelined ? kModeSweep : (c->t > 0 ? pass_mode(c, c->last_active) : kModeDense);
    const bool fused = !unfused(c);
    const bool lean = c->lean_init && c->t == 0 && c->cur_mode == kModeDense && fused && lean_pass0(c);
    if (c->lean_init && !lean) {
        const int rc_init = ensure_initial_state(c);
        if (rc_init) return rc_init;
    }
    c->lean_init = false;
    if (c->t == 0 && std::getenv("HB_TRACE_INIT")) std::fprintf(stderr, "[hb init] pass 0 runs %s\n", lean ? "lean (derives the initial state itself)" : "on the state init_kernel wrote");
// ... 383 lines not shown
```

### stract_amd/csrc/hb_aux.hip.h

```cpp
#pragma once
#include "hb_bloom.hip.h"

namespace hbk {

__global__ __launch_bounds__(256) void validate_plan_kernel(const uint64_t *row_ptr, const uint32_t *src, uint64_t rows_total, uint64_t n_pad,
                                                            uint64_t src_len, unsigned long long *bad)
{
    const uint64_t t = (uint64_t)blockIdx.x * 256 + threadIdx.x;
    const uint64_t nq = (uint64_t)gridDim.x * 64;
    const int q = threadIdx.x & 3;
    unsigned b0 = 0, b1 = 0, b2 = 0, b3 = 0;
    for (uint64_t row = t >> 2; row < rows_total; row += nq) {
        const uint64_t b = row_ptr[row], e = row_ptr[row + 1];
        if (b > e || e > src_len) {
            b0 += (q == 0);
            continue;
        }
        if (row + 1 == rows_total && e != src_len) b0 += (q == 0);
        const bool first_virtual = b < e && src[b] >= n_pad;
        for (uint64_t k = b + q; k < e; k += 4) {
            const uint32_t s = src[k];
            if (s >= rows_total) b1++;
            else {
                if ((s >= n_pad) != first_virtual) b2++;
                if (s >= n_pad && (row < n_pad ? false : s >= row)) b3++;
            }
        }
    }
    if (b0) atomicAdd(&bad[0], (unsigned long long)b0);
    if (b1) atomicAdd(&bad[1], (unsigned long long)b1);
    if (b2) atomicAdd(&bad[2], (unsigned long long)b2);
    if (b3) atomicAdd(&bad[3], (unsigned long long)b3);
}

__global__ __launch_bounds__(256) void hll_size_kernel(const uint4 *regs, uint64_t count, uint64_t *out,
                                                       const double *raw, const double *bias, const uint8_t *lc)
{
    const uint64_t t = (uint64_t)blockIdx.x * 256 + threadIdx.x;
    const uint64_t row = t >> 2;
    const uint64_t rows_pad = (count + 15) & ~15ull;
    if (row >= rows_pad) return;
    uint4 v = make_uint4(0, 0, 0, 0);
    if (row < count) v = regs[t];
    const uint64_t sz = hll_size_quad(v, raw, bias, lc);
    if (row < count && (t & 3) == 0) out[row] = sz;
}

__global__ __launch_bounds__(256) void merge_max_kernel(uint4 *dst, const uint4 *other, uint64_t count4)
{
    for (uint64_t i = (uint64_t)blockIdx.x * 256 + threadIdx.x; i < count4; i += (uint64_t)gridDim.x * 256) {
        uint4 a = dst[i];
        const uint4 b = other[i];
        Acc acc;
        acc_zero(acc);
        acc_merge(acc, a);
        acc_merge(acc, b);
        dst[i] = acc_value(acc);
    }
}

__global__ __launch_bounds__(256) void or_words_kernel(uint32_t *dst, const uint32_t *src, uint64_t words)
{
    for (uint64_t i = (uint64_t)blockIdx.x * 256 + threadIdx.x; i < words; i += (uint64_t)gridDim.x * 256) dst[i] |= src[i];
}
__global__ __launch_bounds__(256) void unpack_rows_kernel(uint4 *wr, const uint32_t *bits, const uint64_t *prefix, uint64_t n_pad, const uint4 *pack)
{
    const uint64_t t = (uint64_t)blockIdx.x * 256 + threadIdx.x;
    const uint64_t row = t >> 2;
    if (row >= n_pad) return;
    const uint32_t w = bits[row >> 5], b = (uint32_t)(row & 31u);
    if (!((w >> b) & 1u)) return;
    const uint64_t pos = prefix[row >> 5] + (uint64_t)__popc(w & ((1u << b) - 1u));
    wr[row * 4 + (t & 3)] = pack[pos * 4 + (t & 3)];
}

__global__ __launch_bounds__(256) void popcount_words_kernel(const uint32_t *bits, uint64_t words, uint32_t *out)
{
    for (uint64_t w = (uint64_t)blockIdx.x * 256 + threadIdx.x; w < words; w += (uint64_t)gridDim.x * 256) out[w] = __popc(bits[w]);
}
__global__ __launch_bounds__(64) void rank_count_kernel(const unsigned long long *counters, unsigned long long *rank_cnt, int world, int rank)
{
    unsigned long long v = threadIdx.x < kStripes ? counters[4 * threadIdx.x] : 0ull;
#pragma unroll
    for (int off = 32; off > 0; off >>= 1) v += __shfl_down(v, off);
    v = __shfl(v, 0);
// ... 345 lines not shown
```

### stract_amd/csrc/hb_experiments.h

```cpp
#pragma once
#include <stdint.h>

#define HB_TUNE1_UNROLL 0xFFu
#ifdef HB_EXPERIMENTS
#define HB_XBITS(tune1) ((uint32_t)(tune1) & ~HB_TUNE1_UNROLL)
#else
#define HB_XBITS(tune1) 0u
#endif

enum hb_xbit : uint32_t {
    HB_X_TILE_EPILOGUE = 0x100u,
    HB_X_SEED_3LAUNCH = 0x800u,
    HB_X_NO_EDGE_OVERLAP = 0x1000u,
    HB_X_BITMAP_SLOTWISE = 0x2000u,
    HB_X_NO_STAGED_RESULTS = 0x4000u,
    HB_X_SNAPSHOT_EVERY_PASS = 0x8000u,
    HB_X_SHORT_FINAL_LIST = 0x10000u,
    HB_X_ONE_SNAPSHOT = 0x20000u,
    HB_X_NO_TAIL_PIPELINE = 0x100000u,
    HB_X_TAIL_KERNEL = 0x200000u,
    HB_X_TAIL_KERNEL_ANY = 0x400000u,
    HB_X_FULL_INIT = 0x800000u,
    HB_X_WIRE_64B = 0x1000000u,
    HB_X_SCATTER_TRANSPOSE = 0x2000000u,
    HB_X_SWEEP_ROUNDS = 0x4000000u,
    HB_X_GENERIC_LEVEL1 = 0x8000000u,
    HB_X_PROBE_NO_SIZE = 0x10000000u,
};
```

### stract_amd/csrc/hb_host.cpp

```cpp
#include "hb_internal.h"

#include <algorithm>
#include <chrono>
#include <cmath>
#include <cstdio>
#include <cstdlib>
#include <cstring>
#include <sched.h>
#include <numeric>

#include <omp.h>

#include "hb_threads.h"
#ifdef _OPENMP
#include <parallel/algorithm>
#define HB_SORT(b, e) __gnu_parallel::sort((b), (e))
#define HB_SORT_CMP(b, e, c) __gnu_parallel::sort((b), (e), (c))
#define HB_STABLE_SORT_CMP(b, e, c) __gnu_parallel::stable_sort((b), (e), (c))
#else
#define HB_SORT(b, e) std::sort((b), (e))
#define HB_SORT_CMP(b, e, c) std::sort((b), (e), (c))
#define HB_STABLE_SORT_CMP(b, e, c) std::stable_sort((b), (e), (c))
#endif

// ... 376 lines not shown
    auto hot_rank = [&](uint32_t idx) -> uint32_t { return (uint32_t)(((uint64_t)idx % slice) * world + (uint64_t)idx / slice); };
    auto from_hot = [&](uint32_t hr) -> uint32_t { return (uint32_t)(((uint64_t)hr % world) * slice + (uint64_t)hr / world); };
    try {
        if (reorder && n) {
            std::vector<std::pair<uint64_t, uint32_t>> kv(n);
#pragma omp parallel for schedule(static)
            for (int64_t s = 0; s < (int64_t)n; s++)
                kv[s] = {(((uint64_t)s % world) << 32) | (uint64_t)(0xFFFFFFFFu - out_degree[s]), (uint32_t)s};
            HB_SORT(kv.begin(), kv.end());
            uint64_t pos = 0, cur_owner = 0;
            for (uint64_t i = 0; i < n; i++) {
                const uint64_t owner = kv[i].first >> 32;
                if (owner != cur_owner) {
                    cur_owner = owner;
                    pos = owner * slice;
                }
                p->order[pos++] = kv[i].second;
            }
        } else {
            std::vector<uint64_t> fill(world, 0);
            for (uint64_t s = 0; s < n; s++) {
                const uint64_t owner = s % world;
                p->order[owner * slice + fill[owner]++] = (uint32_t)s;
            }
        }
#pragma omp parallel for schedule(static)
        for (int64_t d = 0; d < (int64_t)n_pad; d++)
            if (p->order[d] != kNone) p->dev_of[p->order[d]] = (uint32_t)d;

        lap("device order");
        std::vector<uint64_t> rp(n_pad + 1, 0);
        for (uint64_t d = 0; d < n_pad; d++) {
            uint32_t s = p->order[d];
            rp[d + 1] = rp[d] + (s == kNone ? 0 : (row_ptr[s + 1] - row_ptr[s]));
        }
        uvec<uint32_t> rs(p->m_eff);
#pragma omp parallel for schedule(dynamic, 256)
        for (int64_t d = 0; d < (int64_t)n_pad; d++) {
            uint32_t s = p->order[d];
            if (s == kNone) continue;
            uint64_t b = row_ptr[s], e = row_ptr[s + 1], o = rp[d];
            for (uint64_t k = b; k < e; k++) rs[o + (k - b)] = hot_rank(p->dev_of[src[k]]);
            std::sort(rs.begin() + o, rs.begin() + o + (e - b));
        }
        lap("relabel + sort rows");

        std::vector<uint64_t> vrow_ptr;
        uvec<uint32_t> vsrc;
        vrow_ptr.push_back(0);
        std::vector<uint8_t> is_split(n_pad, 0);
        uint64_t next_vid = p->n_pad;
        p->level_begin.push_back(next_vid);
        const uint32_t kWarmSlices = tune.xcd_map ? 64u : 0u;
        auto band_of = [&](uint32_t idx) -> uint32_t {
            if (!tune.band_w || idx < tune.band_w) return 0;
            const uint64_t j = (uint64_t)idx / tune.band_w;
            if (j <= kWarmSlices) return (uint32_t)j;
            const uint64_t q = j / (kWarmSlices + 1u);
            return kWarmSlices + 1u + (uint32_t)(63 - __builtin_clzll(q));
        };
        struct Chunk { uint64_t beg; uint32_t len; uint32_t key; };
        std::vector<Chunk> chunks;
        std::vector<uint32_t> hub_rows;
        std::vector<uint64_t> hub_first;
        const uint32_t minc = std::max<uint32_t>(1, std::min(tune.minc, chunk));
        for (uint64_t d = 0; d < n_pad; d++) {
            if (rp[d + 1] - rp[d] <= tune.direct_max) continue;
            is_split[d] = 1;
            hub_rows.push_back((uint32_t)d);
        }
        auto cut_row = [&](uint64_t d, auto &&emit) {
            const uint64_t b = rp[d], e = rp[d + 1];
            uint64_t i = b;
            while (i < e) {
                const uint32_t b0 = band_of(rs[i]);
                uint64_t j = i + 1;
                while (j < e && j - i < chunk) {
                    if (j - i >= minc && band_of(rs[j]) != b0) break;
                    j++;
                }
                if (e - j < minc && e - i <= chunk) j = e;
                emit(i, (uint32_t)(j - i), b0);
                i = j;
            }
        };
        hub_first.assign(hub_rows.size() + 1, 0);
#pragma omp parallel for schedule(dynamic, 64)
        for (int64_t h = 0; h < (int64_t)hub_rows.size(); h++) {
            uint64_t cnt = 0;
            cut_row(hub_rows[h], [&](uint64_t, uint32_t, uint32_t) { cnt++; });
            hub_first[h + 1] = cnt;
        }
        for (size_t h = 0; h < hub_rows.size(); h++) hub_first[h + 1] += hub_first[h];
        chunks.resize(hub_first[hub_rows.size()]);
#pragma omp parallel for schedule(dynamic, 64)
        for (int64_t h = 0; h < (int64_t)hub_rows.size(); h++) {
            uint64_t w = hub_first[h];
            cut_row(hub_rows[h], [&](uint64_t beg, uint32_t len, uint32_t key) { chunks[w++] = {beg, len, key}; });
        }
        lap("cut chunks");
        const int groups = tune.xcd_map ? 8 : 1;
        std::vector<uint8_t> grp(chunks.size(), 0);
        std::vector<uint32_t> corder(chunks.size());
        std::iota(corder.begin(), corder.end(), 0u);
        HB_STABLE_SORT_CMP(corder.begin(), corder.end(), [&](uint32_t a, uint32_t b2) {
            if (chunks[a].key != chunks[b2].key) return chunks[a].key < chunks[b2].key;
            return chunks[a].len > chunks[b2].len;
        });
        if (groups > 1) {
            XcdQuota quota;
            for (size_t k = 0; k < chunks.size(); k++) quota.add(chunks[k].key, chunks[k].len, kWarmSlices);
            quota.finish();
            uint64_t prefix[2] = {0, 0};
            for (size_t r = 0; r < corder.size(); r++) {
                const uint32_t k = corder[r];
                const uint32_t key = chunks[k].key;
                if (key >= 1 && key <= kWarmSlices) {
                    grp[k] = (uint8_t)(key & 7u);
                } else {
                    const int cls = key == 0 ? 0 : 1;
                    grp[k] = (uint8_t)quota.group_of(cls, prefix[cls]);
                    prefix[cls] += chunks[k].len + 4;
                }
            }
            HB_STABLE_SORT_CMP(corder.begin(), corder.end(), [&](uint32_t a, uint32_t b2) { return grp[a] < grp[b2]; });
        }
        lap("sort chunks");
        std::vector<uint32_t> vid_of(chunks.size());
        {
            std::vector<uint64_t> vrp;
            vrp.reserve(chunks.size() + 8 * kRowAlign + 1);
            std::vector<int64_t> row_chunk;
            row_chunk.reserve(chunks.size() + 8 * kRowAlign);
            uint64_t off = 0;
            size_t k = 0;
            for (int x = 0; x < groups; x++) {
                p->xcd_begin[x] = next_vid + row_chunk.size();
                while (k < corder.size() && grp[corder[k]] == x) {
                    vrp.push_back(off);
                    off += chunks[corder[k]].len;
                    vid_of[corder[k]] = (uint32_t)(next_vid + row_chunk.size());
                    row_chunk.push_back((int64_t)corder[k]);
                    k++;
                }
                while (groups > 1 && row_chunk.size() % kRowAlign) {
                    vrp.push_back(off);
                    row_chunk.push_back(-1);
                }
            }
            for (int x = groups; x <= 8; x++) p->xcd_begin[x] = next_vid + row_chunk.size();
            p->xcd_groups = groups;
            vrp.push_back(off);
            vrow_ptr.swap(vrp);
            vsrc.reserve(off + row_chunk.size() + row_chunk.size() / 8 + 64ull * kRowAlign);
            vsrc.resize(off);
            p->level1_edges = off;
            p->level1_rows = chunks.size();
#pragma omp parallel for schedule(static, 4096)
            for (int64_t r = 0; r < (int64_t)row_chunk.size(); r++) {
                if (row_chunk[r] < 0) continue;
                const Chunk &c = chunks[row_chunk[r]];
                uint32_t *dst = vsrc.data() + vrow_ptr[r];
                for (uint64_t i = 0; i < c.len; i++) dst[i] = from_hot(rs[c.beg + i]);
            }
            next_vid += row_chunk.size();
        }
        lap("emit level-1 lists");
        std::vector<uint64_t> lptr(hub_rows.size() + 1, 0);
        std::vector<uint32_t> lids(chunks.size());
        for (size_t h = 0; h < hub_rows.size(); h++) {
            lptr[h] = hub_first[h];
            for (uint64_t k = hub_first[h]; k < hub_first[h + 1]; k++) lids[k] = vid_of[k];
        }
        lptr[hub_rows.size()] = chunks.size();
        auto pad_level = [&]() {
            while ((next_vid - p->n_pad) % kRowAlign) {
                vrow_ptr.push_back(vsrc.size());
                next_vid++;
            }
        };
        while (true) {
            pad_level();
            p->level_begin.push_back(next_vid);
            bool any = false;
            for (size_t h = 0; h < hub_rows.size() && !any; h++) any = (lptr[h + 1] - lptr[h]) > chunk;
            if (!any) break;
            std::vector<uint64_t> nptr(hub_rows.size() + 1, 0);
            std::vector<uint32_t> nids;
            nids.reserve(lids.size());
            for (size_t h = 0; h < hub_rows.size(); h++) {
                nptr[h] = nids.size();
                const uint64_t cnt = lptr[h + 1] - lptr[h];
                if (cnt <= chunk) {
                    nids.insert(nids.end(), lids.begin() + lptr[h], lids.begin() + lptr[h + 1]);
                    continue;
                }
                const uint64_t parts = (cnt + chunk - 1) / chunk;
                const uint64_t per = (cnt + parts - 1) / parts;
                for (uint64_t k = 0; k < parts; k++) {
                    const uint64_t b = lptr[h] + k * per, e = std::min<uint64_t>(lptr[h + 1], b + per);
                    vsrc.insert(vsrc.end(), lids.begin() + b, lids.begin() + e);
                    vrow_ptr.push_back(vsrc.size());
                    nids.push_back((uint32_t)next_vid++);
                }
            }
            nptr[hub_rows.size()] = nids.size();
            lptr.swap(nptr);
            lids.swap(nids);
        }
        if (p->level_begin.size() >= 2 && p->level_begin[p->level_begin.size() - 1] ==
                                              p->level_begin[p->level_begin.size() - 2])
            p->level_begin.pop_back();
        p->nv = next_vid - p->n_pad;
        if (next_vid >= (uint64_t)kNone) return "row id space exhausted (n + virtual rows >= 2^32 - 1)";
        std::vector<uint32_t> hub_index(n_pad, 0);
        for (size_t h = 0; h < hub_rows.size(); h++) hub_index[hub_rows[h]] = (uint32_t)h;

        lap("upper levels");
        const uint64_t rows_total = p->n_pad + p->nv;
        p->row_ptr.resize(rows_total + 1);
        uint64_t total = 0, direct = 0, with_in = 0;
        for (uint64_t d = 0; d < n_pad; d++) {
            p->row_ptr[d] = total;
            total += is_split[d] ? (lptr[hub_index[d] + 1] - lptr[hub_index[d]]) : (rp[d + 1] - rp[d]);
            if (!is_split[d]) direct += rp[d + 1] - rp[d];
            with_in += rp[d + 1] > rp[d];
        }
        p->direct_edges = direct;
        p->rows_with_in_edges = with_in;
        p->row_ptr[n_pad] = total;
        const uint64_t real_total = total;
        for (uint64_t k = 0; k < p->nv; k++) p->row_ptr[p->n_pad + k + 1] = real_total + vrow_ptr[k + 1];
        p->src.resize(real_total + vsrc.size());
#pragma omp parallel for schedule(dynamic, 4096)
        for (int64_t d = 0; d < (int64_t)n_pad; d++) {
            uint64_t o = p->row_ptr[d];
            if (is_split[d]) {
                const uint64_t b = lptr[hub_index[d]], e = lptr[hub_index[d] + 1];
                std::memcpy(p->src.data() + o, lids.data() + b, (e - b) * sizeof(uint32_t));
            } else {
                for (uint64_t k = rp[d]; k < rp[d + 1]; k++) p->src[o + (k - rp[d])] = from_hot(rs[k]);
            }
        }
        lap("assemble");
        {
            const int64_t blocks = (int64_t)((vsrc.size() + (1u << 20) - 1) >> 20);
#pragma omp parallel for schedule(static)
            for (int64_t b = 0; b < blocks; b++) {
                const uint64_t o = (uint64_t)b << 20, cnt = std::min<uint64_t>(1u << 20, vsrc.size() - o);
                std::memcpy(p->src.data() + real_total + o, vsrc.data() + o, cnt * sizeof(uint32_t));
            }
        }
    } catch (const std::bad_alloc &) {
        return "out of host memory in the planner";
    }
    return "";
}

bool build_lc_table(uint8_t lc[68])
{
    bool robust = true;
    lc[0] = 0xFF;
    lc[65] = lc[66] = lc[67] = 0xFF;
    lc[64] = 0;
    for (int v = 1; v < 64; v++) {
        double h = 64.0 * std::log(64.0 / (double)v);
        if (std::fabs(h - 40.0) < 1e-6) robust = false;
        if (h <= 40.0) {
            double fl = std::floor(h);
            if (h - fl < 1e-6 || (fl + 1.0) - h < 1e-6) robust = false;
            lc[v] = (uint8_t)fl;
        } else {
            lc[v] = 0xFF;
        }
    }
    return robust;
}

void host_scatter_f64(double *out, const uint32_t *idx, const double *val, uint64_t n)
{
    if (n < (1u << 16)) {
        for (uint64_t k = 0; k < n; k++) out[idx[k]] = val[k];
        return;
    }
#pragma omp parallel for num_threads(std::min(host_threads(), 8)) schedule(static)
    for (int64_t k = 0; k < (int64_t)n; k++) out[idx[k]] = val[k];
}

void host_gather_id_lo(const hb_u128 *ids, uint64_t n, uint64_t *lo)
{
#pragma omp parallel for num_threads(n >= (1u << 18) ? std::min(host_threads(), 16) : 1) schedule(static)
    for (int64_t s = 0; s < (int64_t)n; s++) lo[s] = ids[s].lo;
}

void host_find_sids(const hb_u128 *ids, uint64_t n, const hb_u128 *query, uint64_t count, uint32_t *sids)
{
// ... 67 lines not shown
```

### stract_amd/csrc/hb_internal.h

```cpp
#ifndef HB_INTERNAL_H
#define HB_INTERNAL_H

#include <cstdint>
#include <cstdio>
#include <cstdlib>
#include <memory>
#include <string>
#include <type_traits>
#include <utility>
#include <vector>

#include "../../include/hyperball.h"

namespace hb {

template <class T>
struct NoInitAlloc {
    using value_type = T;
    NoInitAlloc() = default;
    template <class U>
    NoInitAlloc(const NoInitAlloc<U> &) {}
    T *allocate(size_t n) { return static_cast<T *>(::operator new(n * sizeof(T))); }
    void deallocate(T *p, size_t) { ::operator delete(p); }
    template <class U, class... A>
    void construct(U *p, A &&...a)
    {
        if constexpr (sizeof...(A) == 0) ::new ((void *)p) U;
        else ::new ((void *)p) U(static_cast<A &&>(a)...);
    }
    template <class U>
    bool operator==(const NoInitAlloc<U> &) const { return true; }
    template <class U>
    bool operator!=(const NoInitAlloc<U> &) const { return false; }
};
template <class T>
using uvec = std::vector<T, NoInitAlloc<T>>;

constexpr uint32_t kNone = 0xFFFFFFFFu;
constexpr uint32_t kRowAlign = 64;
constexpr uint32_t kDefaultChunk = 64;

static inline bool u128_less(const hb_u128 &a, const hb_u128 &b)
{
    return a.hi != b.hi ? a.hi < b.hi : a.lo < b.lo;
}
static inline bool u128_eq(const hb_u128 &a, const hb_u128 &b) { return a.hi == b.hi && a.lo == b.lo; }

struct DenseGraph {
    uvec<hb_u128> ids;
    std::vector<uint64_t> row_ptr;
    std::vector<uint32_t> src;
    uint64_t m_input = 0, m_unique = 0;
};

struct Plan {
    uint64_t n = 0;
    uint64_t n_pad = 0;
    uint64_t slice = 0;
    uint64_t nv = 0;
    uint64_t m_eff = 0;
    uint32_t chunk = kDefaultChunk;
    std::vector<uint32_t> order;
    std::vector<uint32_t> dev_of;
    uvec<uint64_t> row_ptr;
    uvec<uint32_t> src;
    std::vector<uint64_t> level_begin;
    uint64_t xcd_begin[9] = {0, 0, 0, 0, 0, 0, 0, 0, 0};
    int xcd_groups = 1;
    uint64_t level1_edges = 0;
    uint64_t level1_rows = 0;
    uint64_t direct_edges = 0;
    uint64_t rows_with_in_edges = 0;
};

struct XcdQuota {
    uint64_t warm[8] = {0, 0, 0, 0, 0, 0, 0, 0};
    uint64_t flex[2] = {0, 0};
    uint64_t bound[2][8];
    static constexpr uint64_t load_of(uint32_t len) { return (uint64_t)len + 4; }
    void add(uint32_t key, uint32_t len, uint32_t warm_slices)
    {
        if (key >= 1 && key <= warm_slices) warm[key & 7u] += load_of(len);
        else flex[key == 0 ? 0 : 1] += load_of(len);
    }
    void finish()
    {
        uint64_t load[8];
        for (int x = 0; x < 8; x++) load[x] = warm[x];
        for (int c = 1; c >= 0; c--) {
            uint64_t total = flex[c];
            for (int x = 0; x < 8; x++) total += load[x];
            const uint64_t target = (total + 7) / 8;
            uint64_t q[8], sq = 0;
            for (int x = 0; x < 8; x++) {
                q[x] = target > load[x] ? target - load[x] : 0;
                sq += q[x];
            }
            if (sq == 0) {
                for (int x = 0; x < 8; x++) q[x] = 1;
                sq = 8;
            }
            uint64_t cum = 0;
            for (int x = 0; x < 8; x++) {
                bound[c][x] = (uint64_t)(((unsigned __int128)cum * flex[c]) / sq);
                cum += q[x];
            }
            for (int x = 0; x < 8; x++) {
                const uint64_t hi = x < 7 ? bound[c][x + 1] : flex[c];
                load[x] += hi - bound[c][x];
            }
        }
    }
    static constexpr uint64_t kStripes = 4096;
    uint64_t stripe(int cls) const { return flex[cls] / kStripes ? flex[cls] / kStripes : 1; }
    int group_of(int cls, uint64_t prefix) const
    {
        const uint64_t scaled = (prefix % stripe(cls)) * kStripes;
        int gsel = 0;
        for (int x = 1; x < 8; x++)
            if (bound[cls][x] <= scaled) gsel = x;
        return gsel;
    }
};

struct PlanTune {
    uint32_t chunk = kDefaultChunk;
    uint32_t band_w = 1u << 16;
    uint32_t minc = 8;
    uint32_t direct_max = 0;
    bool xcd_map = true;
    uint32_t world = 1;
};

std::string ingest_edges(const hb_u128 *node_ids, uint64_t n, const hb_edge *edges, uint64_t m,
                         DenseGraph *out, uint64_t skip_mask = HB_SKIPPED_REL_MASK);
void keep_owned_rows(DenseGraph *g, uint64_t world, uint64_t rank);
struct TailIndex;
TailIndex *tail_index_build(const hb_u128 *ids, uint64_t n);
void tail_index_free(TailIndex *t);
struct TailDoc {
    uint32_t from_sid;
    uint32_t pass;
    hb_u128 to;
};
std::string tail_collect(const TailIndex *tix, uint64_t n, const hb_edge *recs, uint64_t count, std::vector<TailDoc> *open);
std::string tail_close_segment(const TailIndex *tix, const hb_u128 *ids, const uint32_t *dev_of, std::vector<TailDoc> *open,
                               std::vector<uint64_t> *keys);
std::string build_tail_csr(std::vector<uint64_t> *keys, uint64_t n_pad, std::vector<uint64_t> *ptr, std::vector<uint32_t> *to);
std::string gpu_ingest_edges(void *stream, const hb_u128 *node_ids, uint64_t n, const hb_edge *edges, uint64_t m,
                             DenseGraph *out, struct DeviceCsr *keep = nullptr, uint64_t *peak_bytes = nullptr,
                             uint64_t skip_mask = HB_SKIPPED_REL_MASK);
constexpr uint64_t kKeepHostGraph = 1ull << 26;
struct IngestChunk {
    uint64_t *d_pair = nullptr;
    uint8_t *d_bad = nullptr;
    uint64_t count = 0, cap = 0;
};
struct IngestStream {
    std::vector<IngestChunk> chunks;
    uint64_t count = 0;
    uint64_t bytes = 0;
    uint64_t peak_bytes = 0;
    void *d_slab[2] = {nullptr, nullptr};
    uint64_t slab_cap = 0;
    void *kstream = nullptr;
    void *d_tab_keys = nullptr;
    uint32_t *d_tab_pids = nullptr;
    uint64_t tab_slots = 0;
    void *d_counter = nullptr;
    unsigned long long *h_counter = nullptr;
    uint64_t npid_known = 0;
    uint64_t unsynced = 0;
    uint64_t trace_polls = 0, trace_reads = 0;
    double trace_ms_poll = 0, trace_ms_read = 0;
    uint64_t max_records = 0;
    uint64_t max_bytes = 0;
    uint64_t chunk_records = 0;
    uint64_t skip_mask = HB_SKIPPED_REL_MASK;
    void free_all();
};
std::string gpu_ingest_append(void *stream, IngestStream *st, const hb_edge *edges, uint64_t m);
std::string gpu_ingest_spill(void *stream, IngestStream *st, std::vector<hb_edge> *out);
std::string gpu_ingest_reduce(void *stream, const hb_u128 *node_ids, uint64_t n, IngestStream *st, DenseGraph *out, struct DeviceCsr *keep,
                              uint64_t *peak_bytes = nullptr);
std::string check_dense(const hb_u128 *sorted_ids, uint64_t n, const uint64_t *row_ptr,
                        const uint32_t *src, uint64_t m);
void count_out_degree(const uint64_t *row_ptr, const uint32_t *src, uint64_t n, std::vector<uint32_t> *deg);
std::string gpu_rank_results(void *stream, const double *d_vals, uint64_t n, uint64_t expect, uint64_t *ranks_out, uint64_t *order_out = nullptr,
                             uint64_t top = 0);
std::string build_plan(uint64_t n, const uint64_t *row_ptr, const uint32_t *src,
                       const std::vector<uint32_t> &global_out_degree, bool reorder, const PlanTune &tune,
                       Plan *plan);
bool build_lc_table(uint8_t lc[68]);

struct DeviceCsr {
    uint64_t *d_row_ptr = nullptr;
    uint32_t *d_src = nullptr;
    uint64_t m = 0;
    uint64_t *d_id_lo = nullptr;
};
struct DevicePlan {
    uint64_t *d_row_ptr = nullptr;
    uint32_t *d_src = nullptr;
    uint64_t src_len = 0;
    uint32_t *d_order = nullptr;
    uint32_t *d_dev_of = nullptr;
    uint32_t *d_outdeg_dev = nullptr;
    uint64_t m_global = 0;
};
std::string device_offsets(void *stream, uint32_t *d_counts, uint64_t count, uint64_t *d_offsets, uint64_t expect);
std::string device_prefix(void *stream, const uint32_t *d_counts, uint64_t count, uint64_t *d_offsets);
std::string gpu_select_reached(void *stream, const uint8_t *d_by_sid, uint64_t n, uint32_t *d_sids, uint8_t *d_dist, uint64_t *d_count);
std::string gpu_similarity_top(void *stream, const uint64_t *d_key, const uint8_t *d_keep, uint64_t n, uint64_t top, uint32_t *h_sid, uint64_t *h_key,
                               uint64_t *written);
std::string gpu_transpose_rows(void *stream, const uint64_t *d_row_ptr, const uint32_t *d_src, uint64_t rows_total, uint64_t entries, uint64_t *d_out_ptr,
                               uint32_t *d_out_rows);
std::string gpu_keep_owned_rows(void *stream, DeviceCsr *csr, uint64_t n, uint64_t world, uint64_t rank);
std::string gpu_build_plan(void *stream, uint64_t n, const uint64_t *d_row_ptr, const uint32_t *d_src, const uint32_t *d_outdeg_sid,
                           bool reorder, const PlanTune &tune, Plan *plan, DevicePlan *out);

double now_ms();
void host_scatter_f64(double *out, const uint32_t *idx, const double *val, uint64_t n);
void host_gather_id_lo(const hb_u128 *ids, uint64_t n, uint64_t *lo);
void host_find_sids(const hb_u128 *ids, uint64_t n, const hb_u128 *query, uint64_t count, uint32_t *sids);
void host_compact_results(const double *src, const hb_u128 *idsrc, uint64_t n, hb_u128 *ids, double *vals, uint64_t cap, const uint64_t *in_bits = nullptr);

struct StoreKey {
    uint64_t k0, k1;
    uint64_t k2_index;
    bool operator<(const StoreKey &o) const
    {
        if (k0 != o.k0) return k0 < o.k0;
        if (k1 != o.k1) return k1 < o.k1;
        return k2_index < o.k2_index;
    }
    bool same_key(const StoreKey &o) const { return k0 == o.k0 && k1 == o.k1 && (k2_index >> 56) == (o.k2_index >> 56); }
    uint64_t index() const { return k2_index & ((1ull << 56) - 1); }
    static int len_of_first(uint8_t b0) { return b0 < 251 ? 1 : b0 == 251 ? 3 : b0 == 252 ? 5 : b0 == 253 ? 9 : 17; }
    int key_len() const { return len_of_first((uint8_t)(k0 >> 56)); }
    void key_bytes(uint8_t out[17]) const
    {
        for (int i = 0; i < 8; i++) out[i] = (uint8_t)(k0 >> (56 - 8 * i));
        for (int i = 0; i < 8; i++) out[8 + i] = (uint8_t)(k1 >> (56 - 8 * i));
        out[16] = (uint8_t)(k2_index >> 56);
    }
};

template <class T>
struct DefaultInitAllocator : std::allocator<T> {
    template <class U>
    struct rebind {
        using other = DefaultInitAllocator<U>;
    };
    using std::allocator<T>::allocator;
    template <class U>
    void construct(U *p) noexcept(std::is_nothrow_default_constructible<U>::value)
    {
        ::new (static_cast<void *>(p)) U;
    }
    template <class U, class... Args>
    void construct(U *p, Args &&...args)
// ... 12 lines not shown
```

### stract_amd/csrc/hb_kernels.hip.h

```cpp
#pragma once
#include <hip/hip_runtime.h>
#include <stdint.h>

#include "hb_regs.hip.h"

namespace hbk {

constexpr uint32_t kNone = 0xFFFFFFFFu;
constexpr int kTableLen = 159;

#ifdef HB_DEBUG_BOUNDS
__device__ unsigned int g_dbg_line = 0;
#define HB_DBG_ASSERT(cond)                                                  \
    do {                                                                     \
        if (!(cond)) atomicCAS(&hbk::g_dbg_line, 0u, (unsigned int)__LINE__); \
    } while (0)
#else
#define HB_DBG_ASSERT(cond) ((void)0)
#endif

constexpr int kStripes = 64;
constexpr int kCounterWords = 4 * kStripes;

__device__ __forceinline__ void block_add_counters(unsigned long long *counters, const unsigned long long v[4], unsigned mask)
{
    __shared__ unsigned long long s_part[4][4];
    const int lane = threadIdx.x & 63, wave = threadIdx.x >> 6;
    if (lane == 0) {
#pragma unroll
        for (int k = 0; k < 4; k++) s_part[wave][k] = v[k];
    }
    __syncthreads();
    if (threadIdx.x < 4 && ((mask >> threadIdx.x) & 1u)) {
        const int k = threadIdx.x;
        const unsigned long long t = s_part[0][k] + s_part[1][k] + s_part[2][k] + s_part[3][k];
        if (t) atomicAdd(&counters[(blockIdx.x & (kStripes - 1)) * 4 + k], t);
    }
}

struct PassParams {
    const uint64_t *row_ptr;
    const uint32_t *src;
    const uint16_t *src_jp;
    const uint4 *rd;
    uint4 *wr;
    uint4 *part;
    const uint32_t *bits_rd;
    uint32_t *bits_wr;
    uint32_t *kdirty;
    double *ksum;
    double *kerr;
    uint64_t *size;
    unsigned long long *counters;
    const uint32_t *outdeg;
    const double *raw;
    const double *bias;
    const uint8_t *lc;
    uint64_t row_lo, row_hi;
    int xcd_map;
    uint64_t xcd_lo[8], xcd_hi[8];
    uint64_t n, n_pad;
    uint64_t rows_total;
    uint64_t slice_lo, slice_hi;
    double t_plus_1;
    uint32_t *lbits;
    const uint32_t *ubits;
    uint4 *rd_init;
    const uint32_t *virt_rows;
    uint32_t xflags;
    const uint16_t *self_jp;
};


}
#include "hb_estimator.hip.h"
namespace hbk {

template <bool REAL, bool FUSED, bool STATS, int UNROLL, bool INIT = false, bool EPI4 = false>
__global__ __launch_bounds__(256) __attribute__((amdgpu_waves_per_eu((REAL && UNROLL >= 4) ? 3 : 4))) void pass_kernel(const PassParams p)
{
    __shared__ double s_raw[FUSED ? kTableLen : 1];
    __shared__ double s_bias[FUSED ? kTableLen : 1];
    __shared__ uint8_t s_lc[68];
    if (FUSED) {
        for (int i = threadIdx.x; i < kTableLen; i += 256) {
            s_raw[i] = p.raw[i];
            s_bias[i] = p.bias[i];
        }
        if (threadIdx.x < 65) s_lc[threadIdx.x] = p.lc[threadIdx.x];
        __syncthreads();
    }
    const int lane = threadIdx.x & 63;
    const int wave = threadIdx.x >> 6;
    const int g = lane >> 2, q = lane & 3;
    const int qshift = lane & ~3;
    uint64_t row_lo = p.row_lo, row_hi = p.row_hi, tile0 = blockIdx.x, tstride = gridDim.x;
    if (!REAL && p.xcd_map) {
        const int x = blockIdx.x & 7;
        row_lo = p.xcd_lo[x];
        row_hi = p.xcd_hi[x];
        tile0 = blockIdx.x >> 3;
        tstride = gridDim.x >> 3;
    }
    const uint64_t ntiles = (row_hi - row_lo + 63) >> 6;
    unsigned long long cnt_changed = 0, cnt_active = 0, cnt_rows = 0, cnt_out = 0;

    constexpr bool kDenseReal = REAL;
    constexpr bool kEpi4 = EPI4 && kDenseReal && FUSED;
    __shared__ uint4 s_init4[INIT ? 4 * 16 * 16 : 1];
    uint32_t *init_row = (uint32_t *)s_init4 + (INIT ? (wave * 16 + g) * 64 : 0);
    bool init_used = false;
    if (INIT) {
#pragma unroll
        for (int k = 0; k < 4; k++) s_init4[(wave * 16 + g) * 16 + ((4 * q + k + g) & 15)] = make_uint4(0, 0, 0, 0);
    }
    __shared__ uint64_t s_prow16[kEpi4 ? 4 : 1][4];
    __shared__ uint32_t s_pkd16[kEpi4 ? 4 : 1][4];
    uint64_t p_row = 0, p_szfull = 0, p_sz = 0;
    double p_sum = 0.0, p_ks = 0.0, p_ke = 0.0;
    uint32_t p_zeros = 0, p_flags = 0;
    int npend = 0;
    const bool p_lean = INIT && REAL && FUSED && p.rd_init != nullptr;
    auto flush_pending = [&]() {
        bool err_nz = false;
        if (q < npend && (p_flags & 1u) && ((p_flags & 6u) || p_lean)) {
            const uint64_t sz_old = p_sz;
            uint64_t sz_new = sz_old;
            if (p_flags & 2u) sz_new = (p_flags & 8u) ? p_szfull : hll_size_from(p_sum, p_zeros, s_raw, s_bias, s_lc);
            double ks = p_ks, ke = p_ke;
            err_nz = kahan_update(ks, ke, sz_new, sz_old, p.t_plus_1);
            if (err_nz || p_lean) {
                p.ksum[p_row] = ks;
                p.kerr[p_row] = ke;
            }
#ifdef HB_EXPERIMENTS
            if (!(p.xflags & 1u))
#endif
            if ((p_flags & 2u) || p_lean) p.size[p_row] = sz_new;
        }
        const uint64_t bal = __ballot(err_nz);
        if (lane == 0) {
            for (int k = 0; k < npend; k++) {
                const uint32_t nk16 = pack16(bal & (0x1111111111111111ull << k));
                const uint64_t r16 = s_prow16[kEpi4 ? wave : 0][k];
                const uint32_t kd16 = s_pkd16[kEpi4 ? wave : 0][k];
                if (nk16 | kd16) ((uint16_t *)p.kdirty)[r16 >> 4] = (uint16_t)nk16;
            }
        }
        npend = 0;
    };
    uint64_t nbeg = 0, nend = 0;
    uint32_t nod = 0;
    uint32_t nvirt = 0;
    uint4 nself = make_uint4(0, 0, 0, 0);
    const bool by_bitmap = INIT && p.virt_rows != nullptr;
    const bool lean = INIT && REAL && FUSED && p.rd_init != nullptr;
    auto own_counter = [&](uint64_t r) -> uint4 {
        if (INIT && REAL && FUSED && lean) return counter_quarter_of_jp((uint32_t)p.self_jp[r], q);
        return p.rd[r * 4 + q];
    };
    {
        const uint64_t r0 = row_lo + (tile0 << 6) + ((uint64_t)wave << 4) + (uint64_t)g;
        if (tile0 < ntiles && r0 < row_hi) {
            nbeg = p.row_ptr[r0];
            nend = p.row_ptr[r0 + 1];
            if (REAL && FUSED) nod = p.outdeg[r0];
            if (kDenseReal) nself = own_counter(r0);
            if (INIT && by_bitmap) nvirt = (p.virt_rows[r0 >> 5] >> (r0 & 31u)) & 1u;
        }
    }
    for (uint64_t tile = tile0; tile < ntiles; tile += tstride) {
        const uint64_t row16 = row_lo + (tile << 6) + ((uint64_t)wave << 4);
        const uint64_t row = row16 + (uint64_t)g;
        const bool valid = row < row_hi;
        const uint64_t beg = nbeg, end = nend;
        const uint32_t od = nod;
        const uint32_t virt = nvirt;
        uint4 selfv = nself;
        {
            const uint64_t nrow = row + (tstride << 6);
            nbeg = nend = 0;
            nod = 0;
            nvirt = 0;
            nself = make_uint4(0, 0, 0, 0);
            if (tile + tstride < ntiles && nrow < row_hi) {
                nbeg = p.row_ptr[nrow];
                nend = p.row_ptr[nrow + 1];
                if (REAL && FUSED) nod = p.outdeg[nrow];
                if (kDenseReal) nself = own_counter(nrow);
                if (INIT && by_bitmap) nvirt = (p.virt_rows[nrow >> 5] >> (nrow & 31u)) & 1u;
            }
        }
        uint64_t pre_sz = 0;
        double pre_ks = 0.0, pre_ke = 0.0;
        if (kDenseReal && FUSED && valid) {
            if (lean) {
                const bool real_row = ((__ballot(u4_ne(selfv, make_uint4(0, 0, 0, 0))) >> qshift) & 0xFull) != 0;
                pre_sz = real_row ? (uint64_t)s_lc[63] : 0ull;
            } else if (kEpi4) {
                if (q == npend) {
#ifdef HB_EXPERIMENTS
                    if (!(p.xflags & 1u))
#endif
                    pre_sz = p.size[row];
                    pre_ks = p.ksum[row];
                    pre_ke = p.kerr[row];
                }
            } else {
                pre_sz = p.size[row];
                if (q == 0) {
                    pre_ks = p.ksum[row];
                    pre_ke = p.kerr[row];
                }
            }
        }
        Acc acc;
        acc_zero(acc);
        if (kDenseReal && valid) acc_merge(acc, selfv);
        if (beg < end) {
            uint32_t first;
            bool real_src;
            if (INIT && by_bitmap) {
                real_src = !virt;
                first = real_src ? 0u : p.src[beg];
                HB_DBG_ASSERT(real_src == (p.src[beg] < p.n_pad));
            } else {
                first = p.src[beg];
                real_src = first < p.n_pad;
            }
            const uint4 *base = real_src ? p.rd : (const uint4 *)(p.part - p.n_pad * 4);
            for (uint64_t e = beg; e < end; e += 4 * UNROLL) {
                uint32_t idx[UNROLL];
                if (INIT && real_src) {
#pragma unroll
                    for (int u = 0; u < UNROLL; u++) {
                        const uint64_t ee = e + 4 * u + q;
                        idx[u] = (ee < end) ? (uint32_t)p.src_jp[ee] : 0u;
                    }
#pragma unroll
                    for (int u = 0; u < UNROLL; u++) {
                        const uint32_t v = idx[u];
                        if (v >> 8) __hip_atomic_fetch_max(&init_row[((v & 63u) + 4u * (uint32_t)g) & 63u], v >> 8, __ATOMIC_RELAXED, __HIP_MEMORY_SCOPE_WORKGROUP);
                    }
                    init_used = true;
                    continue;
                }
#pragma unroll
                for (int u = 0; u < UNROLL; u++) {
                    uint64_t ee = e + 4 * u + q;
                    idx[u] = (ee < end) ? p.src[ee] : kNone;
                }
#pragma unroll
                for (int u = 0; u < UNROLL; u++) {
                    if (STATS && real_src) cnt_active += (idx[u] != kNone);
                }
                {
                    uint4 r[UNROLL][4];
#pragma unroll
                    for (int u = 0; u < UNROLL; u++) {
                        uint32_t s0 = quad_bcast<0>(idx[u]), s1 = quad_bcast<1>(idx[u]);
                        uint32_t s2 = quad_bcast<2>(idx[u]), s3 = quad_bcast<3>(idx[u]);
                        s0 = (s0 != kNone) ? s0 : first;
                        s1 = (s1 != kNone) ? s1 : first;
                        s2 = (s2 != kNone) ? s2 : first;
                        s3 = (s3 != kNone) ? s3 : first;
                        HB_DBG_ASSERT(s0 < p.rows_total && s1 < p.rows_total && s2 < p.rows_total && s3 < p.rows_total);
                        HB_DBG_ASSERT((s0 < p.n_pad) == real_src && (s1 < p.n_pad) == real_src && (s2 < p.n_pad) == real_src && (s3 < p.n_pad) == real_src);
                        r[u][0] = base[(uint64_t)s0 * 4 + q];
                        r[u][1] = base[(uint64_t)s1 * 4 + q];
                        r[u][2] = base[(uint64_t)s2 * 4 + q];
                        r[u][3] = base[(uint64_t)s3 * 4 + q];
                    }
#pragma unroll
                    for (int u = 0; u < UNROLL; u++) {
#pragma unroll
                        for (int j = 0; j < 4; j++) acc_merge(acc, r[u][j]);
                    }
                }
            }
        }
        if (INIT) {
            if (__ballot(init_used)) {
                __builtin_amdgcn_fence(__ATOMIC_RELEASE, "wavefront");
                __builtin_amdgcn_wave_barrier();
                __builtin_amdgcn_fence(__ATOMIC_ACQUIRE, "wavefront");
                uint32_t wv[4];
#pragma unroll
                for (int k = 0; k < 4; k++) {
                    uint4 *cell = &s_init4[(wave * 16 + g) * 16 + ((4 * q + k + g) & 15)];
                    const uint4 c = *cell;
                    *cell = make_uint4(0, 0, 0, 0);
                    wv[k] = c.x | (c.y << 8) | (c.z << 16) | (c.w << 24);
                }
                acc_merge(acc, make_uint4(wv[0], wv[1], wv[2], wv[3]));
                __builtin_amdgcn_fence(__ATOMIC_RELEASE, "wavefront");
                __builtin_amdgcn_wave_barrier();
                init_used = false;
            }
        }
        const uint32_t prev16 = REAL ? (uint32_t)((const uint16_t *)p.bits_rd)[row16 >> 4] : 0u;
        const uint32_t kd16 = (REAL && FUSED) ? (uint32_t)((const uint16_t *)p.kdirty)[row16 >> 4] : 0u;
        const bool self_prev = (prev16 >> g) & 1u;
        const bool kd = (kd16 >> g) & 1u;
        const bool need = valid;
        const uint4 accv = acc_value(acc);
        const bool lane_diff = need && (!REAL || u4_ne(accv, selfv));
        const uint64_t bal = __ballot(lane_diff);
        const bool changed = ((bal >> qshift) & 0xFull) != 0;
        if (REAL) {
            if (need && (!FUSED || INIT || changed || self_prev || p.t_plus_1 == 1.0)) p.wr[row * 4 + q] = accv;
            if (lean && need && !changed) p.rd_init[row * 4 + q] = accv;
        } else {
            if (changed) p.part[(row - p.n_pad) * 4 + q] = accv;
        }
        const uint32_t ch16 = pack16(bal);
        if (FUSED) {
            if (lane == 0 && row16 < row_hi) ((uint16_t *)p.bits_wr)[row16 >> 4] = (uint16_t)ch16;
        }
        if (REAL && !FUSED && p.lbits && lane == 0 && row16 < row_hi) ((uint16_t *)p.lbits)[row16 >> 4] = (uint16_t)ch16;
        if (REAL && FUSED) {
            cnt_changed += __popc(ch16);
            if (changed && q == 0) cnt_out += od;
        }
        if (kEpi4) {
            double rsum;
            uint32_t zeros, big;
            hll_sum_quad(accv, rsum, zeros, big, s_lc);
            uint64_t szfull = 0;
            if (big) szfull = hll_size_from(hll_fold_quad(accv), zeros, s_raw, s_bias, s_lc);
            if (q == npend) {
                p_row = row;
                p_sum = rsum;
                p_zeros = zeros;
                p_szfull = szfull;
                p_sz = pre_sz;
                p_ks = pre_ks;
                p_ke = pre_ke;
                p_flags = (need ? 1u : 0u) | (changed ? 2u : 0u) | (kd ? 4u : 0u) | (big ? 8u : 0u);
            }
            if (lane == 0) {
                s_prow16[kEpi4 ? wave : 0][npend] = row16;
                s_pkd16[kEpi4 ? wave : 0][npend] = row16 < row_hi ? kd16 : 0u;
            }
            if (++npend == 4) flush_pending();
        }
        if (REAL && FUSED && !kEpi4) {
            bool err_nz = false;
            if (need && (changed || kd || lean)) {
                const uint64_t sz_old = kDenseReal ? pre_sz : p.size[row];
                const uint64_t sz_new = changed ? hll_size_quad(accv, s_raw, s_bias, s_lc) : sz_old;
                if (q == 0) {
                    double ks = kDenseReal ? pre_ks : p.ksum[row], ke = kDenseReal ? pre_ke : p.kerr[row];
                    err_nz = kahan_update(ks, ke, sz_new, sz_old, p.t_plus_1);
                    if (err_nz || lean) {
                        p.ksum[row] = ks;
                        p.kerr[row] = ke;
                    }
// ... 480 lines not shown
```

### stract_amd/csrc/hb_plan.hip

```cpp
#include "hb_guard_alloc.h"
#include "hb_pool.h"
#include <hip/hip_runtime.h>

#include <algorithm>
#include <cstdlib>
#include <cstring>
#include <string>
#include <vector>

#include <rocprim/rocprim.hpp>

#include "hb_internal.h"

namespace {

using hb::kNone;
using hb::kRowAlign;

#ifdef HB_DEBUG_BOUNDS
__device__ unsigned int g_plan_dbg_line = 0;
#define PL_DBG_ASSERT(cond)                                              \
    do {                                                                 \
        if (!(cond)) atomicCAS(&g_plan_dbg_line, 0u, (unsigned int)__LINE__); \
    } while (0)
// ... 72 lines not shown
        if (!p) return;
        if (slab && (char *)p >= slab && (char *)p < slab + slab_bytes) {
            const size_t off = (size_t)((char *)p - slab);
            for (size_t i = 0; i < blocks.size(); i++) {
                if (blocks[i].off != off) continue;
                blocks[i].free = true;
                if (i + 1 < blocks.size() && blocks[i + 1].free) {
                    blocks[i].size += blocks[i + 1].size;
                    blocks.erase(blocks.begin() + (long)i + 1);
                }
                if (i > 0 && blocks[i - 1].free) {
                    blocks[i - 1].size += blocks[i].size;
                    blocks.erase(blocks.begin() + (long)i);
                }
                return;
            }
            return;
        }
        for (auto &q : extra)
            if (q == p) {
                (void)hipFree(p);
                q = nullptr;
            }
    }
    template <typename T>
    hipError_t alloc_out(T **out, size_t count)
    {
        void *p = nullptr;
        hipError_t e = hipMalloc(&p, std::max<size_t>(count * sizeof(T), 256));
        if (e == hipSuccess) outputs.push_back(p);
        *out = (T *)p;
        return e;
    }
    void *disown(void *p)
    {
        for (auto &q : outputs)
            if (q == p) q = nullptr;
        return p;
    }
};

unsigned grid_for(uint64_t count, unsigned per_block = 256) { return (unsigned)std::max<uint64_t>(1, (count + per_block - 1) / per_block); }
unsigned grid_strided(uint64_t count) { return (unsigned)std::max<uint64_t>(1, std::min<uint64_t>((count + 255) / 256, 1u << 22)); }
int bits_for(uint64_t v)
{
    int b = 1;
    while (b < 64 && (1ull << b) < v) b++;
    return b;
}

struct BandParams {
    uint32_t band_w;
    uint32_t warm_slices;
};
__device__ __forceinline__ uint32_t band_of(const BandParams bp, uint32_t idx)
{
    if (!bp.band_w || idx < bp.band_w) return 0;
    const uint64_t j = (uint64_t)idx / bp.band_w;
    if (j <= bp.warm_slices) return (uint32_t)j;
    const uint64_t q = j / (bp.warm_slices + 1u);
    return bp.warm_slices + 1u + (uint32_t)(63 - __clzll((long long)q));
}

__global__ __launch_bounds__(256) void order_keys_kernel(const uint32_t *outdeg, uint64_t n, uint64_t world, uint64_t *key, uint32_t *val)
{
    const uint64_t s = (uint64_t)blockIdx.x * 256 + threadIdx.x;
    if (s >= n) return;
    key[s] = ((s % world) << 32) | (uint64_t)(0xFFFFFFFFu - outdeg[s]);
    val[s] = (uint32_t)s;
}
__device__ __forceinline__ uint64_t owner_first(uint64_t n, uint64_t world, uint64_t o)
{
    uint64_t f = 0;
    for (uint64_t j = 0; j < o; j++) f += (n > j) ? (n - j + world - 1) / world : 0;
    return f;
}
__global__ __launch_bounds__(256) void place_sorted_kernel(const uint64_t *key, const uint32_t *val, uint64_t n, uint64_t world, uint64_t slice,
                                                           uint32_t *order, uint32_t *dev_of)
{
    const uint64_t i = (uint64_t)blockIdx.x * 256 + threadIdx.x;
    if (i >= n) return;
    const uint64_t owner = key[i] >> 32;
    const uint64_t pos = owner * slice + (i - owner_first(n, world, owner));
    order[pos] = val[i];
    dev_of[val[i]] = (uint32_t)pos;
}
__global__ __launch_bounds__(256) void place_identity_kernel(uint64_t n, uint64_t world, uint64_t slice, uint32_t *order, uint32_t *dev_of)
{
    const uint64_t s = (uint64_t)blockIdx.x * 256 + threadIdx.x;
    if (s >= n) return;
    const uint64_t pos = (s % world) * slice + s / world;
    order[pos] = (uint32_t)s;
    dev_of[s] = (uint32_t)pos;
}

__global__ __launch_bounds__(256) void row_start_kernel(const uint64_t *row_ptr, uint64_t n, uint32_t *rowid)
{
    const uint64_t v = (uint64_t)blockIdx.x * 256 + threadIdx.x;
    if (v >= n) return;
    const uint64_t b = row_ptr[v];
    if (row_ptr[v + 1] > b) rowid[b] = (uint32_t)v;
}
__global__ __launch_bounds__(256) void edge_keys_kernel(const uint32_t *rowid, const uint32_t *src, uint64_t m, const uint32_t *dev_of,
                                                        uint64_t slice, uint64_t world, uint64_t *key)
{
    for (uint64_t e = (uint64_t)blockIdx.x * 256 + threadIdx.x; e < m; e += (uint64_t)gridDim.x * 256) {
        const uint64_t d = dev_of[rowid[e]];
        const uint64_t idx = dev_of[src[e]];
        const uint64_t hr = world == 1 ? idx : (idx % slice) * world + idx / slice;
        key[e] = (d << 32) | hr;
    }
}
__global__ __launch_bounds__(256) void low_half_kernel(const uint64_t *key, uint64_t m, uint32_t *out)
{
// ... 107 lines not shown
    uint64_t bound[2][8];
    uint64_t stripe[2];
    uint64_t hot_total;
};
__global__ __launch_bounds__(256) void assign_groups_kernel(const uint32_t *corder, const uint32_t *ckey, const uint64_t *prefix, uint64_t C,
                                                            uint32_t warm_slices, QuotaBounds qb, uint32_t *grp_sorted, uint8_t *grp_of_chunk,
                                                            unsigned int *group_count)
{
    __shared__ unsigned int s_cnt[8];
    if (threadIdx.x < 8) s_cnt[threadIdx.x] = 0;
    __syncthreads();
    const uint64_t r = (uint64_t)blockIdx.x * 256 + threadIdx.x;
    if (r < C) {
        const uint32_t k = corder[r];
        const uint32_t key = ckey[k];
        uint32_t gsel;
        if (key >= 1 && key <= warm_slices) {
            gsel = key & 7u;
        } else {
            const int cls = key == 0 ? 0 : 1;
            const uint64_t pre = cls == 0 ? prefix[r] : prefix[r] - qb.hot_total;
            const uint64_t scaled = (pre % qb.stripe[cls]) * hb::XcdQuota::kStripes;
            gsel = 0;
#pragma unroll
            for (int x = 1; x < 8; x++)
                if (qb.bound[cls][x] <= scaled) gsel = (uint32_t)x;
        }
        grp_sorted[r] = gsel;
        grp_of_chunk[k] = (uint8_t)gsel;
        atomicAdd(&s_cnt[gsel], 1u);
    }
    __syncthreads();
    if (threadIdx.x < 8 && s_cnt[threadIdx.x]) atomicAdd(&group_count[threadIdx.x], s_cnt[threadIdx.x]);
}
struct GroupLayout {
    uint64_t row_first[8];
    uint64_t sort_first[8];
};
__global__ __launch_bounds__(256) void level1_rows_kernel(const uint32_t *forder, const uint8_t *grp_of_chunk, const uint32_t *clen, uint64_t C,
                                                          GroupLayout gl, uint64_t first_vid, uint32_t *vid_of, uint32_t *row_chunk,
                                                          uint32_t *vlen)
{
    const uint64_t j = (uint64_t)blockIdx.x * 256 + threadIdx.x;
    if (j >= C) return;
    const uint32_t k = forder[j];
    const int x = grp_of_chunk[k];
    const uint64_t row = gl.row_first[x] + (j - gl.sort_first[x]);
    vid_of[k] = (uint32_t)row;
    row_chunk[row - first_vid] = k;
    vlen[row - first_vid] = clen[k];
}
__global__ __launch_bounds__(256) void level1_fill_kernel(const uint32_t *row_chunk, uint64_t rows, const uint64_t *vrow_ptr, const uint64_t *cbeg,
                                                          const uint32_t *clen, const uint32_t *rs, uint64_t slice, uint64_t world, uint32_t *vsrc,
                                                          uint64_t m, uint64_t C, uint64_t vsrc_cap)
{
    const uint64_t t = (uint64_t)blockIdx.x * 256 + threadIdx.x;
    const uint64_t r = t >> 2;
    const int q = (int)(t & 3);
    if (r >= rows) return;
    const uint32_t k = row_chunk[r];
    if (k == kNone) return;
    PL_DBG_ASSERT(k < C);
    const uint64_t o = vrow_ptr[r], b = cbeg[k];
    const uint32_t len = clen[k];
    PL_DBG_ASSERT(b + len <= m);
    PL_DBG_ASSERT(o + len <= vsrc_cap);
    (void)m;
    (void)C;
    (void)vsrc_cap;
    for (uint32_t i = q; i < len; i += 4) {
        const uint64_t hr = rs[b + i];
        vsrc[o + i] = (uint32_t)(world == 1 ? hr : (hr % world) * slice + hr / world);
    }
}

__global__ __launch_bounds__(256) void level_parts_kernel(const uint64_t *lptr, uint64_t H, uint32_t chunk, uint64_t *parts, uint64_t *newcnt,
                                                          uint64_t *moved)
{
    const uint64_t h = (uint64_t)blockIdx.x * 256 + threadIdx.x;
    if (h >= H) return;
    const uint64_t cnt = lptr[h + 1] - lptr[h];
    const uint64_t p = cnt > chunk ? (cnt + chunk - 1) / chunk : 0;
    parts[h] = p;
    newcnt[h] = p ? p : cnt;
    moved[h] = p ? cnt : 0;
}
__global__ __launch_bounds__(256) void level_emit_kernel(const uint64_t *lptr, const uint32_t *lids, uint64_t H, const uint64_t *parts,
                                                         const uint64_t *vidoff, const uint64_t *noff, const uint64_t *srcoff, uint64_t level_first,
                                                         uint64_t first_vid, uint32_t *vlen, uint32_t *vsrc_level, uint32_t *nids)
{
    const int lane = threadIdx.x & 63;
    const uint64_t wave = (uint64_t)blockIdx.x * 4 + (threadIdx.x >> 6), nwaves = (uint64_t)gridDim.x * 4;
    for (uint64_t h = wave; h < H; h += nwaves) {
        const uint64_t b = lptr[h], e = lptr[h + 1], cnt = e - b;
        const uint64_t p = parts[h];
        if (!p) {
            for (uint64_t i = lane; i < cnt; i += 64) nids[noff[h] + i] = lids[b + i];
            continue;
        }
        const uint64_t per = (cnt + p - 1) / p;
        for (uint64_t i = lane; i < cnt; i += 64) vsrc_level[srcoff[h] + i] = lids[b + i];
        for (uint64_t k = lane; k < p; k += 64) {
            const uint64_t pb = k * per, pe = std::min<uint64_t>(cnt, pb + per);
            const uint64_t row = level_first + vidoff[h] + k;
            vlen[row - first_vid] = (uint32_t)(pe - pb);
            nids[noff[h] + k] = (uint32_t)row;
        }
    }
}

__global__ __launch_bounds__(256) void hub_index_kernel(const uint32_t *hub_rows, uint64_t H, uint32_t *hub_index)
{
    const uint64_t h = (uint64_t)blockIdx.x * 256 + threadIdx.x;
    if (h < H) hub_index[hub_rows[h]] = (uint32_t)h;
}
__global__ __launch_bounds__(256) void real_len_kernel(const uint64_t *deg, const uint8_t *is_split, const uint32_t *hub_index, const uint64_t *lptr,
                                                       uint64_t n_pad, uint64_t *len)
{
    const uint64_t d = (uint64_t)blockIdx.x * 256 + threadIdx.x;
    if (d >= n_pad) return;
    if (is_split[d]) {
        const uint32_t h = hub_index[d];
        len[d] = lptr[h + 1] - lptr[h];
    } else {
        len[d] = deg[d];
    }
}
__global__ __launch_bounds__(256) void real_fill_kernel(const uint64_t *row_ptr, const uint8_t *is_split, const uint32_t *hub_index, const uint64_t *lptr,
                                                        const uint32_t *lids, const uint64_t *rp, const uint32_t *rs, uint64_t n_pad, uint64_t slice,
                                                        uint64_t world, uint32_t *src)
{
    const uint64_t t = (uint64_t)blockIdx.x * 256 + threadIdx.x;
    const uint64_t d = t >> 2;
    const int q = (int)(t & 3);
    if (d >= n_pad) return;
    const uint64_t o = row_ptr[d], len = row_ptr[d + 1] - o;
    if (is_split[d]) {
        const uint64_t b = lptr[hub_index[d]];
        for (uint64_t i = q; i < len; i += 4) src[o + i] = lids[b + i];
    } else {
        const uint64_t b = rp[d];
        for (uint64_t i = q; i < len; i += 4) {
            const uint64_t hr = rs[b + i];
            src[o + i] = (uint32_t)(world == 1 ? hr : (hr % world) * slice + hr / world);
        }
    }
}
__global__ __launch_bounds__(256) void virtual_row_ptr_kernel(const uint64_t *vrow_ptr, uint64_t nv, uint64_t real_total, uint64_t *row_ptr_tail)
{
    const uint64_t k = (uint64_t)blockIdx.x * 256 + threadIdx.x;
    if (k <= nv) row_ptr_tail[k] = real_total + vrow_ptr[k];
}

struct Widen32 {
    __device__ uint64_t operator()(uint32_t v) const { return v; }
};
struct DistReached {
    __device__ uint8_t operator()(uint8_t d) const { return d != 255u ? 1 : 0; }
};

}

namespace hb {

std::string device_offsets(void *stream_v, uint32_t *d_counts , uint64_t count,
                           uint64_t *d_offsets, uint64_t expect)
{
    hipStream_t stream = (hipStream_t)stream_v;
    auto wide = rocprim::make_transform_iterator(d_counts, Widen32());
    size_t bytes = 0;
    void *tmp = nullptr;
    PL_HIP(rocprim::exclusive_scan(nullptr, bytes, wide, d_offsets, (uint64_t)0, (size_t)count, rocprim::plus<uint64_t>(), stream));
    PL_HIP(hipMalloc(&tmp, std::max<size_t>(bytes, 256)));
    hipError_t e = rocprim::exclusive_scan(tmp, bytes, wide, d_offsets, (uint64_t)0, (size_t)count, rocprim::plus<uint64_t>(), stream);
    uint64_t last_off = 0;
    uint32_t last_cnt = 0;
    if (e == hipSuccess && count) e = hipMemcpyAsync(&last_off, d_offsets + (count - 1), sizeof(uint64_t), hipMemcpyDeviceToHost, stream);
    if (e == hipSuccess && count) e = hipMemcpyAsync(&last_cnt, d_counts + (count - 1), sizeof(uint32_t), hipMemcpyDeviceToHost, stream);
    if (e == hipSuccess) e = hipStreamSynchronize(stream);
    (void)hipFree(tmp);
    if (e != hipSuccess) return std::string("device_offsets: ") + hipGetErrorString(e);
    const uint64_t total = last_off + last_cnt;
    if (total != expect) return "transposed plan graph: entry count mismatch";
    e = hipMemcpyAsync(d_offsets + count, &total, sizeof(uint64_t), hipMemcpyHostToDevice, stream);
    if (e == hipSuccess) e = hipStreamSynchronize(stream);
    if (e != hipSuccess) return std::string("device_offsets: ") + hipGetErrorString(e);
    return "";
}

std::string device_prefix(void *stream_v, const uint32_t *d_counts, uint64_t count, uint64_t *d_offsets)
{
    hipStream_t stream = (hipStream_t)stream_v;
    auto wide = rocprim::make_transform_iterator(d_counts, Widen32());
    size_t bytes = 0;
    void *tmp = nullptr;
    if (!count) {
        PL_HIP(hipMemsetAsync(d_offsets, 0, sizeof(uint64_t), stream));
        return "";
    }
// ... 183 lines not shown
        return m;
    };
    if (hipMalloc((void **)&d_cnt, (n + 1) * sizeof(uint32_t)) != hipSuccess || hipMalloc((void **)&d_new_ptr, (n + 1) * sizeof(uint64_t)) != hipSuccess)
        return bail("gpu_keep_owned_rows: out of device memory");
    hipLaunchKernelGGL(owned_counts_kernel, dim3((unsigned)((n + 255) / 256)), dim3(256), 0, stream, (const uint64_t *)csr->d_row_ptr, n, world, rank, d_cnt);
    if (hipGetLastError() != hipSuccess) return bail("gpu_keep_owned_rows: launch failed");
    std::string e = device_prefix(stream_v, d_cnt, n, d_new_ptr);
    if (!e.empty()) return bail(e);
    uint64_t m_new = 0;
    if (hipMemcpyAsync(&m_new, d_new_ptr + n, sizeof(uint64_t), hipMemcpyDeviceToHost, stream) != hipSuccess || hipStreamSynchronize(stream) != hipSuccess)
        return bail("gpu_keep_owned_rows: read-back failed");
    if (m_new == csr->m) return bail("");
    if (hipMalloc((void **)&d_new_src, std::max<uint64_t>(m_new, 1) * sizeof(uint32_t)) != hipSuccess) return bail("gpu_keep_owned_rows: out of device memory");
    if (m_new) {
        const unsigned blocks = (unsigned)std::min<uint64_t>((m_new + 255) / 256, 65536);
        hipLaunchKernelGGL(owned_copy_kernel, dim3(blocks), dim3(256), 0, stream, (const uint64_t *)csr->d_row_ptr, (const uint32_t *)csr->d_src,
                           (const uint64_t *)d_new_ptr, n, m_new, d_new_src);
        if (hipGetLastError() != hipSuccess || hipStreamSynchronize(stream) != hipSuccess) return bail("gpu_keep_owned_rows: copy failed");
    }
    (void)hipFree(csr->d_row_ptr);
    (void)hipFree(csr->d_src);
    (void)hipFree(d_cnt);
    csr->d_row_ptr = d_new_ptr;
    csr->d_src = d_new_src;
    csr->m = m_new;
    return "";
}

std::string gpu_build_plan(void *stream_v, uint64_t n, const uint64_t *d_row_ptr_in, const uint32_t *d_src_in, const uint32_t *d_outdeg_sid,
                           bool reorder, const PlanTune &tune_in, Plan *p, DevicePlan *out)
{
    hipStream_t stream = (hipStream_t)stream_v;
    PlanTune tune = tune_in;
    uint32_t chunk = tune.chunk ? tune.chunk : kDefaultChunk;
    if (chunk < 4) chunk = 4;
    if (chunk > 4096) chunk = 4096;
    if (tune.direct_max == 0 || tune.direct_max > chunk) tune.direct_max = chunk;
    if (tune.minc == 0) tune.minc = 8;
    const uint32_t minc = std::max<uint32_t>(1, std::min(tune.minc, chunk));
    const uint64_t world = tune.world > 1 ? tune.world : 1;
    const uint64_t slice = ((n + world - 1) / world + kRowAlign - 1) / kRowAlign * kRowAlign;
    const uint64_t n_pad = slice * world;
    *out = DevicePlan{};
    p->n = n;
    p->slice = slice;
    p->n_pad = n_pad;
    p->chunk = chunk;
    p->nv = 0;
    p->order.clear();
    p->dev_of.clear();
    p->level_begin.clear();
    decltype(p->row_ptr)().swap(p->row_ptr);
    decltype(p->src)().swap(p->src);
    uint64_t m = 0;
    if (n) PL_HIP(hipMemcpyAsync(&m, d_row_ptr_in + n, sizeof(uint64_t), hipMemcpyDeviceToHost, stream));
    PL_HIP(hipStreamSynchronize(stream));
    p->m_eff = m;
    const bool timing = std::getenv("HB_PLAN_TIMING") != nullptr;
    double tmark = now_ms();
    auto lap = [&](const char *what) {
        if (!timing) return;
        (void)hipStreamSynchronize(stream);
        const double t = now_ms();
        std::fprintf(stderr, "[gpu plan] %-28s %8.1f ms\n", what, t - tmark);
        tmark = t;
    };

    DevMem mem;
    PL_HIP(mem.init(24 * m + m / 2 + 96 * n_pad + (512ull << 20)));
    void *tmp = nullptr;
    size_t tmp_bytes = 0;
    auto need_tmp = [&](size_t bytes) -> hipError_t {
        if (bytes <= tmp_bytes) return hipSuccess;
        if (tmp) mem.release(tmp);
        tmp_bytes = bytes + (bytes >> 3) + 256;
        char *q = nullptr;
        hipError_t e = mem.alloc(&q, tmp_bytes);
        tmp = q;
        return e;
    };

    uint32_t *d_order = nullptr, *d_dev_of = nullptr, *d_outdeg_dev = nullptr;
    PL_HIP(mem.alloc_out(&d_order, n_pad));
    PL_HIP(mem.alloc_out(&d_dev_of, n));
    PL_HIP(mem.alloc_out(&d_outdeg_dev, n_pad));
    PL_HIP(hipMemsetAsync(d_order, 0xFF, std::max<uint64_t>(n_pad, 1) * sizeof(uint32_t), stream));
    if (n) {
        if (reorder) {
            uint64_t *k_in = nullptr, *k_out = nullptr;
            uint32_t *v_in = nullptr, *v_out = nullptr;
            PL_HIP(mem.alloc(&k_in, n));
            PL_HIP(mem.alloc(&k_out, n));
            PL_HIP(mem.alloc(&v_in, n));
            PL_HIP(mem.alloc(&v_out, n));
            hipLaunchKernelGGL(order_keys_kernel, dim3(grid_for(n)), dim3(256), 0, stream, d_outdeg_sid, n, world, k_in, v_in);
            PL_HIP(hipGetLastError());
            size_t bytes = 0;
            const unsigned end_bit = 32 + (unsigned)bits_for(world);
            PL_HIP(rocprim::radix_sort_pairs(nullptr, bytes, k_in, k_out, v_in, v_out, (size_t)n, 0u, end_bit, stream));
            PL_HIP(need_tmp(bytes));
            PL_HIP(rocprim::radix_sort_pairs(tmp, bytes, k_in, k_out, v_in, v_out, (size_t)n, 0u, end_bit, stream));
            hipLaunchKernelGGL(place_sorted_kernel, dim3(grid_for(n)), dim3(256), 0, stream, (const uint64_t *)k_out, (const uint32_t *)v_out, n,
                               world, slice, d_order, d_dev_of);
            PL_HIP(hipGetLastError());
            PL_HIP(hipStreamSynchronize(stream));
            mem.release(k_in);
// ... 26 lines not shown
                           (const uint32_t *)d_dev_of, slice, world, k_in);
        PL_HIP(hipGetLastError());
        PL_HIP(hipStreamSynchronize(stream));
        mem.release(d_rowid);
        lap("  rows: keys");
        PL_HIP(mem.alloc(&k_out, m));
        const unsigned end_bit = 32 + (unsigned)bits_for(std::max<uint64_t>(n_pad, 2));
        bytes = 0;
        rocprim::double_buffer<uint64_t> keys(k_in, k_out);
        PL_HIP(rocprim::radix_sort_keys(nullptr, bytes, keys, (size_t)m, 0u, end_bit, stream));
        PL_HIP(need_tmp(bytes));
        PL_HIP(rocprim::radix_sort_keys(tmp, bytes, keys, (size_t)m, 0u, end_bit, stream));
        lap("  rows: 64-bit radix sort");
        hipLaunchKernelGGL(low_half_kernel, dim3(grid_strided(m)), dim3(256), 0, stream, (const uint64_t *)keys.current(), m, d_rs);
        PL_HIP(hipGetLastError());
        PL_HIP(hipStreamSynchronize(stream));
        mem.release(k_in);
        mem.release(k_out);
        if (tmp_bytes > (64u << 20)) {
            mem.release(tmp);
            tmp = nullptr;
            tmp_bytes = 0;
        }
    }
    uint64_t *d_deg = nullptr, *d_rp = nullptr;
    uint8_t *d_is_split = nullptr;
    unsigned long long *d_sums = nullptr;
    PL_HIP(mem.alloc(&d_deg, n_pad + 1));
    PL_HIP(mem.alloc(&d_rp, n_pad + 1));
    PL_HIP(mem.alloc(&d_is_split, n_pad + 1));
    PL_HIP(mem.alloc(&d_sums, 32));
    PL_HIP(hipMemsetAsync(d_sums, 0, 32 * sizeof(unsigned long long), stream));
    PL_HIP(hipMemsetAsync(d_deg, 0, (n_pad + 1) * sizeof(uint64_t), stream));
    if (n_pad) {
        hipLaunchKernelGGL(row_info_kernel, dim3(grid_for(n_pad)), dim3(256), 0, stream, (const uint32_t *)d_order, n_pad, d_row_ptr_in,
                           d_outdeg_sid, tune.direct_max, d_deg, d_is_split, d_outdeg_dev, d_sums);
        PL_HIP(hipGetLastError());
    }
    {
        size_t bytes = 0;
        PL_HIP(rocprim::exclusive_scan(nullptr, bytes, d_deg, d_rp, (uint64_t)0, (size_t)(n_pad + 1), rocprim::plus<uint64_t>(), stream));
        PL_HIP(need_tmp(bytes));
        PL_HIP(rocprim::exclusive_scan(tmp, bytes, d_deg, d_rp, (uint64_t)0, (size_t)(n_pad + 1), rocprim::plus<uint64_t>(), stream));
    }
    unsigned long long h_sums[32];
    PL_HIP(hipMemcpyAsync(h_sums, d_sums, sizeof(h_sums), hipMemcpyDeviceToHost, stream));
    PL_HIP(hipStreamSynchronize(stream));
    p->direct_edges = h_sums[0];
    p->rows_with_in_edges = h_sums[1];
    out->m_global = h_sums[2];
    lap("relabel + sort rows");

    const uint32_t warm_slices = tune.xcd_map ? 64u : 0u;
    const BandParams bp{tune.band_w, warm_slices};
    uint32_t *d_hub_rows = nullptr;
    uint64_t *d_cnt = nullptr;
    PL_HIP(mem.alloc(&d_hub_rows, n_pad + 1));
    PL_HIP(mem.alloc(&d_cnt, 2));
    uint64_t H = 0;
    if (n_pad) {
        auto iota = rocprim::make_counting_iterator<uint32_t>(0);
        size_t bytes = 0;
        PL_HIP(rocprim::select(nullptr, bytes, iota, d_is_split, d_hub_rows, d_cnt, (size_t)n_pad, stream));
        PL_HIP(need_tmp(bytes));
        PL_HIP(rocprim::select(tmp, bytes, iota, d_is_split, d_hub_rows, d_cnt, (size_t)n_pad, stream));
        PL_HIP(hipMemcpyAsync(&H, d_cnt, sizeof(uint64_t), hipMemcpyDeviceToHost, stream));
        PL_HIP(hipStreamSynchronize(stream));
    }
    uint64_t *d_hub_cnt = nullptr, *d_hub_first = nullptr;
    PL_HIP(mem.alloc(&d_hub_cnt, H + 1));
    PL_HIP(mem.alloc(&d_hub_first, H + 1));
    PL_HIP(hipMemsetAsync(d_hub_cnt, 0, (H + 1) * sizeof(uint64_t), stream));
    const unsigned cut_blocks = (unsigned)std::max<uint64_t>(1, std::min<uint64_t>((H + 3) / 4, 4096));
    uint64_t C = 0;
    if (H) {
        hipLaunchKernelGGL(cut_rows_kernel<false>, dim3(cut_blocks), dim3(256), 0, stream, (const uint32_t *)d_hub_rows, H, (const uint64_t *)d_rp,
                           (const uint32_t *)d_rs, chunk, minc, bp, d_hub_cnt, (const uint64_t *)nullptr, (uint64_t *)nullptr, (uint32_t *)nullptr,
                           (uint32_t *)nullptr);
        PL_HIP(hipGetLastError());
    }
    {
        size_t bytes = 0;
        PL_HIP(rocprim::exclusive_scan(nullptr, bytes, d_hub_cnt, d_hub_first, (uint64_t)0, (size_t)(H + 1), rocprim::plus<uint64_t>(), stream));
        PL_HIP(need_tmp(bytes));
        PL_HIP(rocprim::exclusive_scan(tmp, bytes, d_hub_cnt, d_hub_first, (uint64_t)0, (size_t)(H + 1), rocprim::plus<uint64_t>(), stream));
        PL_HIP(hipMemcpyAsync(&C, d_hub_first + H, sizeof(uint64_t), hipMemcpyDeviceToHost, stream));
        PL_HIP(hipStreamSynchronize(stream));
    }
    if (n_pad + C + C / 8 + 64ull * kRowAlign >= (uint64_t)kNone) return "row id space exhausted (n + virtual rows >= 2^32 - 1)";
    uint64_t *d_cbeg = nullptr;
    uint32_t *d_clen = nullptr, *d_ckey = nullptr;
    PL_HIP(mem.alloc(&d_cbeg, C + 1));
    PL_HIP(mem.alloc(&d_clen, C + 1));
    PL_HIP(mem.alloc(&d_ckey, C + 1));
    if (H) {
        hipLaunchKernelGGL(cut_rows_kernel<true>, dim3(cut_blocks), dim3(256), 0, stream, (const uint32_t *)d_hub_rows, H, (const uint64_t *)d_rp,
                           (const uint32_t *)d_rs, chunk, minc, bp, (uint64_t *)nullptr, (const uint64_t *)d_hub_first, d_cbeg, d_clen, d_ckey);
        PL_HIP(hipGetLastError());
    }
    lap("cut chunks");

    const int groups = tune.xcd_map ? 8 : 1;
    uint32_t *d_forder = nullptr;
    uint8_t *d_grp_of = nullptr;
    PL_HIP(mem.alloc(&d_forder, C + 1));
    PL_HIP(mem.alloc(&d_grp_of, C + 1));
    PL_HIP(hipMemsetAsync(d_grp_of, 0, C + 1, stream));
// ... 72 lines not shown
        mem.release(corder);
    }
    lap("sort chunks");

    const uint64_t first_vid = n_pad;
    GroupLayout gl{};
    uint64_t next_vid = first_vid;
    p->level_begin.push_back(next_vid);
    {
        uint64_t sorted_pos = 0;
        for (int x = 0; x < 8; x++) {
            p->xcd_begin[x] = next_vid;
            gl.row_first[x] = next_vid;
            gl.sort_first[x] = sorted_pos;
            if (x < groups) {
                next_vid += h_group_count[x];
                sorted_pos += h_group_count[x];
                if (groups > 1) next_vid = (next_vid - first_vid + kRowAlign - 1) / kRowAlign * kRowAlign + first_vid;
            }
        }
        p->xcd_begin[8] = next_vid;
        p->xcd_groups = groups;
    }
    const uint64_t rows_l1 = next_vid - first_vid;
    const uint64_t vrow_cap = rows_l1 + rows_l1 / 2 + 64ull * kRowAlign;
    uint32_t *d_vid_of = nullptr, *d_row_chunk = nullptr, *d_vlen = nullptr;
    PL_HIP(mem.alloc(&d_vid_of, C + 1));
    PL_HIP(mem.alloc(&d_row_chunk, rows_l1 + 1));
    PL_HIP(mem.alloc(&d_vlen, vrow_cap + 1));
    PL_HIP(hipMemsetAsync(d_row_chunk, 0xFF, (rows_l1 + 1) * sizeof(uint32_t), stream));
    PL_HIP(hipMemsetAsync(d_vlen, 0, (vrow_cap + 1) * sizeof(uint32_t), stream));
    if (C) {
        hipLaunchKernelGGL(level1_rows_kernel, dim3(grid_for(C)), dim3(256), 0, stream, (const uint32_t *)d_forder, (const uint8_t *)d_grp_of,
                           (const uint32_t *)d_clen, C, gl, first_vid, d_vid_of, d_row_chunk, d_vlen);
        PL_HIP(hipGetLastError());
    }
    uint64_t *d_vrow_ptr = nullptr;
    PL_HIP(mem.alloc(&d_vrow_ptr, vrow_cap + 2));
    uint64_t l1_edges = 0;
    {
        auto wide = rocprim::make_transform_iterator(d_vlen, Widen32());
        size_t bytes = 0;
        PL_HIP(rocprim::exclusive_scan(nullptr, bytes, wide, d_vrow_ptr, (uint64_t)0, (size_t)(rows_l1 + 1), rocprim::plus<uint64_t>(), stream));
        PL_HIP(need_tmp(bytes));
        PL_HIP(rocprim::exclusive_scan(tmp, bytes, wide, d_vrow_ptr, (uint64_t)0, (size_t)(rows_l1 + 1), rocprim::plus<uint64_t>(), stream));
        PL_HIP(hipMemcpyAsync(&l1_edges, d_vrow_ptr + rows_l1, sizeof(uint64_t), hipMemcpyDeviceToHost, stream));
        PL_HIP(hipStreamSynchronize(stream));
    }
    p->level1_edges = l1_edges;
    p->level1_rows = C;
    const uint64_t vsrc_cap = l1_edges + rows_l1 + rows_l1 / 8 + 64ull * kRowAlign;
    uint32_t *d_vsrc = nullptr;
    PL_HIP(mem.alloc(&d_vsrc, vsrc_cap + 1));
    if (rows_l1) {
        hipLaunchKernelGGL(level1_fill_kernel, dim3(grid_for(rows_l1 * 4)), dim3(256), 0, stream, (const uint32_t *)d_row_chunk, rows_l1,
                           (const uint64_t *)d_vrow_ptr, (const uint64_t *)d_cbeg, (const uint32_t *)d_clen, (const uint32_t *)d_rs, slice, world, d_vsrc, m, C,
                           vsrc_cap);
        PL_HIP(hipGetLastError());
        PL_HIP(hipStreamSynchronize(stream));
    }
    mem.release(d_row_chunk);
    mem.release(d_cbeg);
    mem.release(d_ckey);
    mem.release(d_forder);
    mem.release(d_grp_of);
    lap("emit level-1 lists");

    uint64_t *d_lptr = d_hub_first;
    uint32_t *d_lids = d_vid_of;
    uint64_t lids_len = C;
    uint64_t vsrc_len = l1_edges;
    uint64_t *d_parts = nullptr, *d_newcnt = nullptr, *d_moved = nullptr, *d_vidoff = nullptr, *d_noff = nullptr, *d_srcoff = nullptr;
    PL_HIP(mem.alloc(&d_parts, H + 1));
    PL_HIP(mem.alloc(&d_newcnt, H + 1));
    PL_HIP(mem.alloc(&d_moved, H + 1));
    PL_HIP(mem.alloc(&d_vidoff, H + 1));
    PL_HIP(mem.alloc(&d_noff, H + 1));
    PL_HIP(mem.alloc(&d_srcoff, H + 1));
    while (true) {
        next_vid = (next_vid - first_vid + kRowAlign - 1) / kRowAlign * kRowAlign + first_vid;
        p->level_begin.push_back(next_vid);
        if (!H) break;
        PL_HIP(hipMemsetAsync(d_parts + H, 0, sizeof(uint64_t), stream));
        PL_HIP(hipMemsetAsync(d_newcnt + H, 0, sizeof(uint64_t), stream));
        PL_HIP(hipMemsetAsync(d_moved + H, 0, sizeof(uint64_t), stream));
        hipLaunchKernelGGL(level_parts_kernel, dim3(grid_for(H)), dim3(256), 0, stream, (const uint64_t *)d_lptr, H, chunk, d_parts, d_newcnt, d_moved);
        PL_HIP(hipGetLastError());
        uint64_t tot[3] = {0, 0, 0};
        uint64_t *ins[3] = {d_parts, d_newcnt, d_moved}, *outs[3] = {d_vidoff, d_noff, d_srcoff};
        for (int k = 0; k < 3; k++) {
            size_t bytes = 0;
            PL_HIP(rocprim::exclusive_scan(nullptr, bytes, ins[k], outs[k], (uint64_t)0, (size_t)(H + 1), rocprim::plus<uint64_t>(), stream));
            PL_HIP(need_tmp(bytes));
            PL_HIP(rocprim::exclusive_scan(tmp, bytes, ins[k], outs[k], (uint64_t)0, (size_t)(H + 1), rocprim::plus<uint64_t>(), stream));
            PL_HIP(hipMemcpyAsync(&tot[k], outs[k] + H, sizeof(uint64_t), hipMemcpyDeviceToHost, stream));
        }
        PL_HIP(hipStreamSynchronize(stream));
        if (tot[0] == 0) break;
        if (next_vid + tot[0] >= (uint64_t)kNone || next_vid + tot[0] - first_vid > vrow_cap || vsrc_len + tot[2] > vsrc_cap)
            return "row id space exhausted (n + virtual rows >= 2^32 - 1)";
        uint32_t *d_nids = nullptr;
        PL_HIP(mem.alloc(&d_nids, tot[1] + 1));
        const unsigned eb = (unsigned)std::max<uint64_t>(1, std::min<uint64_t>((H + 3) / 4, 4096));
        hipLaunchKernelGGL(level_emit_kernel, dim3(eb), dim3(256), 0, stream, (const uint64_t *)d_lptr, (const uint32_t *)d_lids, H,
                           (const uint64_t *)d_parts, (const uint64_t *)d_vidoff, (const uint64_t *)d_noff, (const uint64_t *)d_srcoff, next_vid,
                           first_vid, d_vlen, d_vsrc + vsrc_len, d_nids);
        PL_HIP(hipGetLastError());
        PL_HIP(hipStreamSynchronize(stream));
        std::swap(d_lptr, d_noff);
        if (d_lids != d_vid_of) mem.release(d_lids);
        else mem.release(d_vid_of);
        d_lids = d_nids;
        lids_len = tot[1];
        next_vid += tot[0];
        vsrc_len += tot[2];
    }
    if (p->level_begin.size() >= 2 && p->level_begin[p->level_begin.size() - 1] == p->level_begin[p->level_begin.size() - 2])
        p->level_begin.pop_back();
    p->nv = next_vid - first_vid;
    if (next_vid >= (uint64_t)kNone) return "row id space exhausted (n + virtual rows >= 2^32 - 1)";
    (void)lids_len;
    lap("upper levels");

    const uint64_t nv = p->nv, rows_total = n_pad + nv;
    uint32_t *d_hub_index = nullptr;
    uint64_t *d_len = nullptr, *d_row_ptr = nullptr;
    PL_HIP(mem.alloc(&d_hub_index, n_pad + 1));
    PL_HIP(mem.alloc(&d_len, n_pad + 1));
    PL_HIP(mem.alloc_out(&d_row_ptr, rows_total + 2));
    PL_HIP(hipMemsetAsync(d_len, 0, (n_pad + 1) * sizeof(uint64_t), stream));
    if (H) {
        hipLaunchKernelGGL(hub_index_kernel, dim3(grid_for(H)), dim3(256), 0, stream, (const uint32_t *)d_hub_rows, H, d_hub_index);
        PL_HIP(hipGetLastError());
    }
    uint64_t real_total = 0;
    if (n_pad) {
        hipLaunchKernelGGL(real_len_kernel, dim3(grid_for(n_pad)), dim3(256), 0, stream, (const uint64_t *)d_deg, (const uint8_t *)d_is_split,
                           (const uint32_t *)d_hub_index, (const uint64_t *)d_lptr, n_pad, d_len);
        PL_HIP(hipGetLastError());
    }
    {
        size_t bytes = 0;
        PL_HIP(rocprim::exclusive_scan(nullptr, bytes, d_len, d_row_ptr, (uint64_t)0, (size_t)(n_pad + 1), rocprim::plus<uint64_t>(), stream));
        PL_HIP(need_tmp(bytes));
        PL_HIP(rocprim::exclusive_scan(tmp, bytes, d_len, d_row_ptr, (uint64_t)0, (size_t)(n_pad + 1), rocprim::plus<uint64_t>(), stream));
        PL_HIP(hipMemcpyAsync(&real_total, d_row_ptr + n_pad, sizeof(uint64_t), hipMemcpyDeviceToHost, stream));
        auto wide = rocprim::make_transform_iterator(d_vlen, Widen32());
        bytes = 0;
        PL_HIP(rocprim::exclusive_scan(nullptr, bytes, wide, d_vrow_ptr, (uint64_t)0, (size_t)(nv + 1), rocprim::plus<uint64_t>(), stream));
        PL_HIP(need_tmp(bytes));
        PL_HIP(rocprim::exclusive_scan(tmp, bytes, wide, d_vrow_ptr, (uint64_t)0, (size_t)(nv + 1), rocprim::plus<uint64_t>(), stream));
        PL_HIP(hipStreamSynchronize(stream));
    }
    hipLaunchKernelGGL(virtual_row_ptr_kernel, dim3(grid_for(nv + 1)), dim3(256), 0, stream, (const uint64_t *)d_vrow_ptr, nv, real_total,
                       d_row_ptr + n_pad);
    PL_HIP(hipGetLastError());
    const uint64_t src_len = real_total + vsrc_len;
    uint32_t *d_src = nullptr;
    PL_HIP(mem.alloc_out(&d_src, src_len + 4));
    if (n_pad) {
        hipLaunchKernelGGL(real_fill_kernel, dim3(grid_for(n_pad * 4)), dim3(256), 0, stream, (const uint64_t *)d_row_ptr, (const uint8_t *)d_is_split,
                           (const uint32_t *)d_hub_index, (const uint64_t *)d_lptr, (const uint32_t *)d_lids, (const uint64_t *)d_rp,
                           (const uint32_t *)d_rs, n_pad, slice, world, d_src);
        PL_HIP(hipGetLastError());
    }
    if (vsrc_len) PL_HIP(hipMemcpyAsync(d_src + real_total, d_vsrc, vsrc_len * sizeof(uint32_t), hipMemcpyDeviceToDevice, stream));
    PL_HIP(hipStreamSynchronize(stream));
    lap("assemble");

    out->d_row_ptr = (uint64_t *)mem.disown(d_row_ptr);
    out->d_src = (uint32_t *)mem.disown(d_src);
    out->src_len = src_len;
    out->d_order = (uint32_t *)mem.disown(d_order);
    out->d_dev_of = (uint32_t *)mem.disown(d_dev_of);
    out->d_outdeg_dev = (uint32_t *)mem.disown(d_outdeg_dev);
#ifdef HB_DEBUG_BOUNDS
    {
        unsigned int line = 0;
        (void)hipDeviceSynchronize();
        if (hipMemcpyFromSymbol(&line, HIP_SYMBOL(g_plan_dbg_line), sizeof(line)) == hipSuccess && line)
            return "HB_DEBUG_BOUNDS: planner index check failed at hb_plan.hip line " + std::to_string(line);
    }
#endif
    return "";
}

}
```

Before: 111.5.

## Order row sources live-first and skip dead-source suffixes in later passes

The planner now partitions each row's source list so sources with nonzero in-degree (live) come first, and records a per-row live prefix length. On single-rank runs, passes after the first read only that live prefix, because sources with no incoming edges never change after initialization. The change also adds experimental cold-band rules, validation of the live-prefix invariant, and debug and host-plan entry points. In exchange the planner does extra fill and reduction work and stores an additional u16 array per row.

```diff
diff --git a/include/hyperball.h b/include/hyperball.h
--- a/include/hyperball.h
+++ b/include/hyperball.h
@@ -334,6 +334,7 @@
 int hb_debug_copy_graph(hb_ctx *ctx, hb_u128 *ids, uint64_t *row_ptr, uint32_t *src);
 int hb_debug_copy_plan(hb_ctx *ctx, uint64_t sizes[4], uint32_t *order, uint64_t *plan_row_ptr, uint32_t *plan_src,
                        uint64_t *level_begin);
+int hb_debug_copy_live_len(hb_ctx *ctx, uint16_t *live_len, uint64_t *dead_edges);
 int hb_debug_exchange(hb_ctx **ctxs, int count, int phase);
 int hb_step_local(hb_ctx *ctx);
 int hb_step_finish(hb_ctx *ctx, int *has_changes);
@@ -347,6 +348,9 @@
 int hb_host_plan(uint64_t n, const uint64_t *row_ptr, const uint32_t *src, uint32_t flags,
                  uint32_t chunk, const uint32_t *tune , uint64_t sizes[4],
                  uint32_t *order, uint64_t *plan_row_ptr, uint32_t *plan_src, uint64_t *level_begin);
+int hb_host_plan_live(uint64_t n, const uint64_t *row_ptr, const uint32_t *src, uint32_t flags,
+                      uint32_t chunk, const uint32_t *tune, uint64_t sizes[4], uint32_t *order, uint64_t *plan_row_ptr,
+                      uint32_t *plan_src, uint64_t *level_begin, uint16_t *live_len, uint64_t *dead_edges);
 int hb_debug_tail_index(uint64_t n, const hb_u128 *sorted_ids, const uint32_t *dev_of, uint64_t n_pad, const hb_edge *records,
                         uint64_t count, uint64_t *ptr_out, uint32_t *to_out, uint64_t to_cap, uint64_t *to_len);
 
diff --git a/stract_amd/_lib.py b/stract_amd/_lib.py
--- a/stract_amd/_lib.py
+++ b/stract_amd/_lib.py
@@ -34,6 +34,8 @@
 HB_SAMPLE_MAX_LEVELS = 16
 
 HB_X_TILE_EPILOGUE = 0x100
+HB_X_COLD_ONE_BAND = 0x200
+HB_X_COLD_FIRST_KEPT = 0x400
 HB_X_SEED_3LAUNCH = 0x800
 HB_X_NO_EDGE_OVERLAP = 0x1000
 HB_X_BITMAP_SLOTWISE = 0x2000
@@ -41,6 +43,8 @@
 HB_X_SNAPSHOT_EVERY_PASS = 0x8000
 HB_X_SHORT_FINAL_LIST = 0x10000
 HB_X_ONE_SNAPSHOT = 0x20000
+HB_X_COLD_DOUBLING = 0x40000
+HB_X_FULL_ROWS = 0x80000
 HB_X_NO_TAIL_PIPELINE = 0x100000
 HB_X_TAIL_KERNEL = 0x200000
 HB_X_TAIL_KERNEL_ANY = 0x400000
@@ -50,6 +54,7 @@
 HB_X_SWEEP_ROUNDS = 0x4000000
 HB_X_GENERIC_LEVEL1 = 0x8000000
 HB_X_PROBE_NO_SIZE = 0x10000000
+HB_X_FULL_NODE_ROWS = 0x20000000
 
 U128 = np.dtype([("lo", "<u8"), ("hi", "<u8")])
 EDGE = np.dtype([("from", U128), ("to", U128), ("rel_flags", "<u8")])
@@ -377,6 +382,8 @@
     ("hb_host_ingest", ctypes.c_int, [_P, _U64, _P, _U64, ctypes.POINTER(_U64), ctypes.POINTER(_U64),
                                       ctypes.POINTER(_U64), _P, _P, _P]),
     ("hb_host_plan", ctypes.c_int, [_U64, _P, _P, ctypes.c_uint32, ctypes.c_uint32, _P, _P, _P, _P, _P, _P]),
+    ("hb_host_plan_live", ctypes.c_int, [_U64, _P, _P, ctypes.c_uint32, ctypes.c_uint32, _P, _P, _P, _P, _P, _P, _P, _P]),
+    ("hb_debug_copy_live_len", ctypes.c_int, [_P, _P, _P]),
 ]
 _SIGNATURES += [
     ("hbw_open", ctypes.c_int, [ctypes.c_char_p, ctypes.c_uint32, ctypes.POINTER(_P)]),
@@ -1025,7 +1032,10 @@
         psrc = np.zeros(slen, dtype=np.uint32)
         lb = np.zeros(levels + 1, dtype=np.uint64)
         self._check(self.lib.hb_debug_copy_plan(self.h, _ptr(sizes), _ptr(order), _ptr(prp), _ptr(psrc), _ptr(lb)))
-        return dict(order=order, row_ptr=prp, src=psrc, level_begin=lb, n_pad=n_pad, nv=nv)
+        live = np.zeros(n_pad + nv, dtype=np.uint16)
+        dead = np.zeros(1, dtype=np.uint64)
+        self._check(self.lib.hb_debug_copy_live_len(self.h, _ptr(live), _ptr(dead)))
+        return dict(order=order, row_ptr=prp, src=psrc, level_begin=lb, n_pad=n_pad, nv=nv, live_len=live, dead_edges=int(dead[0]))
 
     def graph(self):
         st = self.stats()
@@ -1067,7 +1077,7 @@
 
 
 def host_plan(row_ptr, src, flags=0, chunk=0, tune=()):
-    lib = load()
+    lib = load(experiments=len(tune) > 1 and (int(tune[1]) & ~0xFF) != 0)
     row_ptr = np.ascontiguousarray(row_ptr, dtype=np.uint64)
     src = np.ascontiguousarray(src, dtype=np.uint32)
     n = len(row_ptr) - 1
@@ -1082,11 +1092,14 @@
     prp = np.zeros(n_pad + nv + 1, dtype=np.uint64)
     psrc = np.zeros(slen, dtype=np.uint32)
     lb = np.zeros(levels + 1, dtype=np.uint64)
-    rc = lib.hb_host_plan(n, _ptr(row_ptr), _ptr(src), flags, chunk, _ptr(tn), _ptr(sizes), _ptr(order), _ptr(prp),
-                          _ptr(psrc), _ptr(lb))
+    live = np.zeros(n_pad + nv, dtype=np.uint16)
+    dead = np.zeros(1, dtype=np.uint64)
+    rc = lib.hb_host_plan_live(n, _ptr(row_ptr), _ptr(src), flags, chunk, _ptr(tn), _ptr(sizes), _ptr(order), _ptr(prp),
+                               _ptr(psrc), _ptr(lb), _ptr(live), _ptr(dead))
     if rc != HB_OK:
         raise HyperballError(rc, (lib.hb_last_error(None) or b"").decode())
     world = int(tn[7]) if tn[7] > 1 else 1
     if world == 1:
         order = order[:n]
-    return dict(order=order, row_ptr=prp, src=psrc, level_begin=lb, n_pad=n_pad, nv=nv, slice=n_pad // world)
+    return dict(order=order, row_ptr=prp, src=psrc, level_begin=lb, n_pad=n_pad, nv=nv, slice=n_pad // world, live_len=live,
+                dead_edges=int(dead[0]))
diff --git a/stract_amd/csrc/hb_api.hip b/stract_amd/csrc/hb_api.hip
--- a/stract_amd/csrc/hb_api.hip
+++ b/stract_amd/csrc/hb_api.hip
@@ -94,6 +94,7 @@
     bool level0_all_real = false;
     uint32_t *d_virt_rows = nullptr;
     uint16_t *d_self_jp = nullptr;
+    uint16_t *d_live_len = nullptr;
     uint4 *d_regs[2] = {nullptr, nullptr};
     uint4 *d_part = nullptr;
     uint32_t *d_bits[2] = {nullptr, nullptr};
@@ -441,6 +442,9 @@
         else if (tune[3] >= 4 && tune[3] < 31) t.band_w = 1u << tune[3];
         if (tune[4]) t.minc = tune[4];
         if (tune[5]) t.direct_max = tune[5];
+        if (HB_XBITS(tune[1]) & HB_X_COLD_DOUBLING) t.cold_rule = kColdDoubling;
+        else if (HB_XBITS(tune[1]) & HB_X_COLD_ONE_BAND) t.cold_rule = kColdOneBand;
+        else if (HB_XBITS(tune[1]) & HB_X_COLD_FIRST_KEPT) t.cold_rule = kColdFirstKept;
     }
     return t;
 }
diff --git a/stract_amd/csrc/hb_api_debug.inc b/stract_amd/csrc/hb_api_debug.inc
--- a/stract_amd/csrc/hb_api_debug.inc
+++ b/stract_amd/csrc/hb_api_debug.inc
@@ -159,6 +159,21 @@
     });
 }
 
+int hb_debug_copy_live_len(hb_ctx *c, uint16_t *live_len, uint64_t *dead_edges)
+{
+    return guarded(c, [&]() -> int {
+        if (!c) return HB_ERR_INVALID;
+        if (!c->loaded) return fail(c, HB_ERR_INVALID, "no graph loaded");
+        int rc = set_device(c);
+        if (rc) return rc;
+        const uint64_t rows_total = c->plan.n_pad + c->plan.nv;
+        if (live_len && rows_total) HB_HIP(hipMemcpyAsync(live_len, c->d_live_len, rows_total * sizeof(uint16_t), hipMemcpyDeviceToHost, c->stream));
+        HB_HIP(hipStreamSynchronize(c->stream));
+        if (dead_edges) *dead_edges = c->plan.dead_edges;
+        return HB_OK;
+    });
+}
+
 int hb_host_ingest(const hb_u128 *node_ids, uint64_t n, const hb_edge *edges, uint64_t m, uint64_t *n_out,
                    uint64_t *m_unique, uint64_t *m_eff, hb_u128 *ids, uint64_t *row_ptr, uint32_t *src)
 {
@@ -181,6 +196,13 @@
 int hb_host_plan(uint64_t n, const uint64_t *row_ptr, const uint32_t *src, uint32_t flags, uint32_t chunk,
                  const uint32_t *tune, uint64_t sizes[4], uint32_t *order, uint64_t *plan_row_ptr, uint32_t *plan_src,
                  uint64_t *level_begin)
+{
+    return hb_host_plan_live(n, row_ptr, src, flags, chunk, tune, sizes, order, plan_row_ptr, plan_src, level_begin, nullptr, nullptr);
+}
+
+int hb_host_plan_live(uint64_t n, const uint64_t *row_ptr, const uint32_t *src, uint32_t flags, uint32_t chunk,
+                      const uint32_t *tune, uint64_t sizes[4], uint32_t *order, uint64_t *plan_row_ptr, uint32_t *plan_src,
+                      uint64_t *level_begin, uint16_t *live_len, uint64_t *dead_edges)
 {
     return guarded(nullptr, [&]() -> int {
         hb_ctx *c = nullptr;
@@ -204,6 +226,8 @@
         if (plan_row_ptr) std::memcpy(plan_row_ptr, p.row_ptr.data(), p.row_ptr.size() * sizeof(uint64_t));
         if (plan_src && !p.src.empty()) std::memcpy(plan_src, p.src.data(), p.src.size() * sizeof(uint32_t));
         if (level_begin) std::memcpy(level_begin, p.level_begin.data(), p.level_begin.size() * sizeof(uint64_t));
+        if (live_len && !p.live_len.empty()) std::memcpy(live_len, p.live_len.data(), p.live_len.size() * sizeof(uint16_t));
+        if (dead_edges) *dead_edges = p.dead_edges;
         return HB_OK;
     });
 }
diff --git a/stract_amd/csrc/hb_api_load.inc b/stract_amd/csrc/hb_api_load.inc
--- a/stract_amd/csrc/hb_api_load.inc
+++ b/stract_amd/csrc/hb_api_load.inc
@@ -148,6 +148,7 @@
     PlanTune pt = plan_tune(c->opt.chunk, c->opt.tune);
     pt.xcd_map = !(c->opt.flags & HB_FLAG_NO_XCD_MAP);
     if (dest_mode(c)) pt.world = (uint32_t)std::max(c->opt.world_size, 1);
+    pt.live_prefix = !multi_rank(c);
     {
         const uint64_t w = pt.world > 1 ? pt.world : 1;
         const uint64_t n_pad_pre = (((n + w - 1) / w + kRowAlign - 1) / kRowAlign * kRowAlign) * w;
@@ -159,9 +160,11 @@
     DevicePlan dp;
     DevPtr<uint64_t> dp_row_ptr;
     DevPtr<uint32_t> dp_src, dp_order, dp_dev_of, dp_outdeg;
+    DevPtr<uint16_t> dp_live;
     if (on_device) {
         std::string perr = gpu_build_plan((void *)c->stream, n, in.d.d_row_ptr, in.d.d_src, d_deg.get(), reorder, pt, &c->plan, &dp);
         dp_row_ptr.reset(dp.d_row_ptr); dp_src.reset(dp.d_src); dp_order.reset(dp.d_order); dp_dev_of.reset(dp.d_dev_of); dp_outdeg.reset(dp.d_outdeg_dev);
+        dp_live.reset(dp.d_live_len);
         if (!perr.empty()) {
             (void)hipGetLastError();
             return fail(c, perr.find("memory") != std::string::npos ? HB_ERR_NOMEM : (perr.find("exhausted") != std::string::npos ? HB_ERR_LIMIT : HB_ERR_HIP), perr);
@@ -208,7 +211,9 @@
         c->d_dev_of = adopt(c, dp_dev_of, std::max<uint64_t>(n, 64) * sizeof(uint32_t));
         c->d_outdeg = adopt(c, dp_outdeg, std::max<uint64_t>(p.n_pad, 64) * sizeof(uint32_t));
         c->m_global = dp.m_global;
+        c->d_live_len = adopt(c, dp_live, (rows_total + 64) * sizeof(uint16_t));
     } else {
+        if ((rc = dev_alloc(c, &c->d_live_len, rows_total + 64))) return rc;
         if ((rc = dev_alloc(c, &c->d_row_ptr, rows_total + 1))) return rc;
         if ((rc = dev_alloc(c, &c->d_src, src_len + 4))) return rc;
         if ((rc = dev_alloc(c, &c->d_dev_of, n))) return rc;
@@ -258,6 +263,8 @@
         HB_HIP(hipMemcpyAsync(c->d_row_ptr, p.row_ptr.data(), (rows_total + 1) * sizeof(uint64_t), hipMemcpyHostToDevice, c->stream));
         if (!p.src.empty())
             HB_HIP(hipMemcpyAsync(c->d_src, p.src.data(), p.src.size() * sizeof(uint32_t), hipMemcpyHostToDevice, c->stream));
+        if (!p.live_len.empty())
+            HB_HIP(hipMemcpyAsync(c->d_live_len, p.live_len.data(), p.live_len.size() * sizeof(uint16_t), hipMemcpyHostToDevice, c->stream));
         if (p.n_pad)
             HB_HIP(hipMemcpyAsync(c->d_sid_of, p.order.data(), p.n_pad * sizeof(uint32_t), hipMemcpyHostToDevice, c->stream));
         std::vector<uint32_t> outdeg_dev(p.n_pad, 0);
@@ -351,20 +358,22 @@
     lap("self_jp / src_jp");
     {
         unsigned long long *d_bad = c->d_counters;
-        unsigned long long h_bad[4] = {0, 0, 0, 0};
+        unsigned long long h_bad[6] = {0, 0, 0, 0, 0, 0};
         HB_HIP(hipMemsetAsync(d_bad, 0, sizeof(h_bad), c->stream));
         if (rows_total) {
             const unsigned blocks = grid_blocks(c, (rows_total * 4 + 255) / 256, 16);
             hipLaunchKernelGGL(hbk::validate_plan_kernel, dim3(blocks), dim3(256), 0, c->stream, (const uint64_t *)c->d_row_ptr, (const uint32_t *)c->d_src,
-                               rows_total, p.n_pad, src_len, d_bad);
+                               rows_total, p.n_pad, src_len, d_bad, (const uint16_t *)c->d_live_len, multi_rank(c) ? 1 : 0);
             HB_HIP(hipGetLastError());
         }
         HB_HIP(hipMemcpyAsync(h_bad, d_bad, sizeof(h_bad), hipMemcpyDeviceToHost, c->stream));
         HB_HIP(hipStreamSynchronize(c->stream));
-        if (h_bad[0] | h_bad[1] | h_bad[2] | h_bad[3])
+        if (h_bad[0] | h_bad[1] | h_bad[2] | h_bad[3] | h_bad[4] | h_bad[5])
             return fail(c, HB_ERR_INVALID, "work layout failed its structural check: " + std::to_string(h_bad[0]) + " bad row pointers, " +
                                                std::to_string(h_bad[1]) + " source ids out of range, " + std::to_string(h_bad[2]) +
-                                               " rows of mixed source kind, " + std::to_string(h_bad[3]) + " virtual rows reading upwards");
+                                               " rows of mixed source kind, " + std::to_string(h_bad[3]) + " virtual rows reading upwards, " +
+                                               std::to_string(h_bad[4]) + " live prefixes longer than their row, " + std::to_string(h_bad[5]) +
+                                               " sources on the wrong side of a live prefix");
     }
     lap("layout check");
     if ((rc = build_sparse_support(c))) return rc;
diff --git a/stract_amd/csrc/hb_api_pass.inc b/stract_amd/csrc/hb_api_pass.inc
--- a/stract_amd/csrc/hb_api_pass.inc
+++ b/stract_amd/csrc/hb_api_pass.inc
@@ -104,6 +104,10 @@
     return launch_full_init(c);
 }
 
+bool live_prefixes(const hb_ctx *c)
+{
+    return c->d_live_len != nullptr && !multi_rank(c) && !linked(c) && !dest_mode(c) && !ref_tail(c) && !xbit(c, HB_X_FULL_ROWS);
+}
 hbk::PassParams make_params(hb_ctx *c)
 {
     const Plan &p = c->plan;
@@ -140,6 +144,7 @@
     pp.self_jp = c->d_self_jp;
     pp.virt_rows = c->d_virt_rows;
     pp.xflags = xbit(c, HB_X_PROBE_NO_SIZE) ? 1u : 0u;
+    pp.live_len = (c->t >= 1 && live_prefixes(c)) ? c->d_live_len : nullptr;
     return pp;
 }
 
@@ -535,6 +540,7 @@
         if (l == 0) HB_HIP(hipEventRecord(E[kEvLevel1], c->stream));
     }
     pp.xcd_map = 0;
+    if (xbit(c, HB_X_FULL_NODE_ROWS)) pp.live_len = nullptr;
     HB_HIP(hipEventRecord(E[kEvLevels], c->stream));
     pp.row_lo = dest_mode(c) ? pp.slice_lo : 0;
     pp.row_hi = dest_mode(c) ? pp.slice_hi : p.n_pad;
diff --git a/stract_amd/csrc/hb_aux.hip.h b/stract_amd/csrc/hb_aux.hip.h
--- a/stract_amd/csrc/hb_aux.hip.h
+++ b/stract_amd/csrc/hb_aux.hip.h
@@ -4,12 +4,12 @@
 namespace hbk {
 
 __global__ __launch_bounds__(256) void validate_plan_kernel(const uint64_t *row_ptr, const uint32_t *src, uint64_t rows_total, uint64_t n_pad,
-                                                            uint64_t src_len, unsigned long long *bad)
+                                                            uint64_t src_len, unsigned long long *bad, const uint16_t *live_len, int full_rows)
 {
     const uint64_t t = (uint64_t)blockIdx.x * 256 + threadIdx.x;
     const uint64_t nq = (uint64_t)gridDim.x * 64;
     const int q = threadIdx.x & 3;
-    unsigned b0 = 0, b1 = 0, b2 = 0, b3 = 0;
+    unsigned b0 = 0, b1 = 0, b2 = 0, b3 = 0, b4 = 0, b5 = 0;
     for (uint64_t row = t >> 2; row < rows_total; row += nq) {
         const uint64_t b = row_ptr[row], e = row_ptr[row + 1];
         if (b > e || e > src_len) {
@@ -18,10 +18,16 @@
         }
         if (row + 1 == rows_total && e != src_len) b0 += (q == 0);
         const bool first_virtual = b < e && src[b] >= n_pad;
+        const uint64_t live = live_len[row];
+        if (live > e - b || ((first_virtual || full_rows) && live != e - b)) {
+            b4 += (q == 0);
+            continue;
+        }
         for (uint64_t k = b + q; k < e; k += 4) {
             const uint32_t s = src[k];
             if (s >= rows_total) b1++;
             else {
+                if (s < n_pad && !full_rows && (row_ptr[s + 1] > row_ptr[s]) != (k - b < live)) b5++;
                 if ((s >= n_pad) != first_virtual) b2++;
                 if (s >= n_pad && (row < n_pad ? false : s >= row)) b3++;
             }
@@ -31,6 +37,8 @@
     if (b1) atomicAdd(&bad[1], (unsigned long long)b1);
     if (b2) atomicAdd(&bad[2], (unsigned long long)b2);
     if (b3) atomicAdd(&bad[3], (unsigned long long)b3);
+    if (b4) atomicAdd(&bad[4], (unsigned long long)b4);
+    if (b5) atomicAdd(&bad[5], (unsigned long long)b5);
 }
 
 __global__ __launch_bounds__(256) void hll_size_kernel(const uint4 *regs, uint64_t count, uint64_t *out,
diff --git a/stract_amd/csrc/hb_experiments.h b/stract_amd/csrc/hb_experiments.h
--- a/stract_amd/csrc/hb_experiments.h
+++ b/stract_amd/csrc/hb_experiments.h
@@ -10,6 +10,8 @@
 
 enum hb_xbit : uint32_t {
     HB_X_TILE_EPILOGUE = 0x100u,
+    HB_X_COLD_ONE_BAND = 0x200u,
+    HB_X_COLD_FIRST_KEPT = 0x400u,
     HB_X_SEED_3LAUNCH = 0x800u,
     HB_X_NO_EDGE_OVERLAP = 0x1000u,
     HB_X_BITMAP_SLOTWISE = 0x2000u,
@@ -17,6 +19,8 @@
     HB_X_SNAPSHOT_EVERY_PASS = 0x8000u,
     HB_X_SHORT_FINAL_LIST = 0x10000u,
     HB_X_ONE_SNAPSHOT = 0x20000u,
+    HB_X_COLD_DOUBLING = 0x40000u,
+    HB_X_FULL_ROWS = 0x80000u,
     HB_X_NO_TAIL_PIPELINE = 0x100000u,
     HB_X_TAIL_KERNEL = 0x200000u,
     HB_X_TAIL_KERNEL_ANY = 0x400000u,
@@ -26,4 +30,5 @@
     HB_X_SWEEP_ROUNDS = 0x4000000u,
     HB_X_GENERIC_LEVEL1 = 0x8000000u,
     HB_X_PROBE_NO_SIZE = 0x10000000u,
+    HB_X_FULL_NODE_ROWS = 0x20000000u,
 };
diff --git a/stract_amd/csrc/hb_host.cpp b/stract_amd/csrc/hb_host.cpp
--- a/stract_amd/csrc/hb_host.cpp
+++ b/stract_amd/csrc/hb_host.cpp
@@ -452,13 +452,7 @@
         uint64_t next_vid = p->n_pad;
         p->level_begin.push_back(next_vid);
         const uint32_t kWarmSlices = tune.xcd_map ? 64u : 0u;
-        auto band_of = [&](uint32_t idx) -> uint32_t {
-            if (!tune.band_w || idx < tune.band_w) return 0;
-            const uint64_t j = (uint64_t)idx / tune.band_w;
-            if (j <= kWarmSlices) return (uint32_t)j;
-            const uint64_t q = j / (kWarmSlices + 1u);
-            return kWarmSlices + 1u + (uint32_t)(63 - __builtin_clzll(q));
-        };
+        auto band_of = [&](uint32_t idx) -> uint32_t { return plan_band_of(tune.band_w, kWarmSlices, tune.cold_rule, idx); };
         struct Chunk { uint64_t beg; uint32_t len; uint32_t key; };
         std::vector<Chunk> chunks;
         std::vector<uint32_t> hub_rows;
@@ -527,6 +521,9 @@
         }
         lap("sort chunks");
         std::vector<uint32_t> vid_of(chunks.size());
+        const bool split_live = world == 1 && tune.live_prefix;
+        auto has_in = [&](uint32_t idx) -> bool { return rp[(uint64_t)idx + 1] > rp[idx]; };
+        std::vector<uint16_t> live1;
         {
             std::vector<uint64_t> vrp;
             vrp.reserve(chunks.size() + 8 * kRowAlign + 1);
@@ -556,12 +553,22 @@
             vsrc.resize(off);
             p->level1_edges = off;
             p->level1_rows = chunks.size();
+            live1.assign(row_chunk.size(), 0);
 #pragma omp parallel for schedule(static, 4096)
             for (int64_t r = 0; r < (int64_t)row_chunk.size(); r++) {
                 if (row_chunk[r] < 0) continue;
                 const Chunk &c = chunks[row_chunk[r]];
                 uint32_t *dst = vsrc.data() + vrow_ptr[r];
-                for (uint64_t i = 0; i < c.len; i++) dst[i] = from_hot(rs[c.beg + i]);
+                if (!split_live) {
+                    for (uint64_t i = 0; i < c.len; i++) dst[i] = from_hot(rs[c.beg + i]);
+                } else {
+                    uint64_t w = 0;
+                    for (uint64_t i = 0; i < c.len; i++)
+                        if (has_in(rs[c.beg + i])) dst[w++] = rs[c.beg + i];
+                    live1[r] = (uint16_t)w;
+                    for (uint64_t i = 0; i < c.len; i++)
+                        if (!has_in(rs[c.beg + i])) dst[w++] = rs[c.beg + i];
+                }
             }
             next_vid += row_chunk.size();
         }
@@ -632,16 +639,34 @@
         const uint64_t real_total = total;
         for (uint64_t k = 0; k < p->nv; k++) p->row_ptr[p->n_pad + k + 1] = real_total + vrow_ptr[k + 1];
         p->src.resize(real_total + vsrc.size());
-#pragma omp parallel for schedule(dynamic, 4096)
+        p->live_len.resize(rows_total);
+        uint64_t dead = 0;
+#pragma omp parallel for schedule(dynamic, 4096) reduction(+ : dead)
         for (int64_t d = 0; d < (int64_t)n_pad; d++) {
             uint64_t o = p->row_ptr[d];
             if (is_split[d]) {
                 const uint64_t b = lptr[hub_index[d]], e = lptr[hub_index[d] + 1];
                 std::memcpy(p->src.data() + o, lids.data() + b, (e - b) * sizeof(uint32_t));
+                p->live_len[d] = (uint16_t)(e - b);
+            } else if (!split_live) {
+                for (uint64_t k = rp[d]; k < rp[d + 1]; k++) p->src[o + (k - rp[d])] = from_hot(rs[k]);
+                p->live_len[d] = (uint16_t)(rp[d + 1] - rp[d]);
             } else {
-                for (uint64_t k = rp[d]; k < rp[d + 1]; k++) p->src[o + (k - rp[d])] = from_hot(rs[k]);
-            }
-        }
+                uint64_t w = o;
+                for (uint64_t k = rp[d]; k < rp[d + 1]; k++)
+                    if (has_in(rs[k])) p->src[w++] = rs[k];
+                p->live_len[d] = (uint16_t)(w - o);
+                dead += rp[d + 1] - rp[d] - (w - o);
+                for (uint64_t k = rp[d]; k < rp[d + 1]; k++)
+                    if (!has_in(rs[k])) p->src[w++] = rs[k];
+            }
+        }
+        for (uint64_t k = 0; k < p->nv; k++) {
+            const uint64_t len = vrow_ptr[k + 1] - vrow_ptr[k];
+            p->live_len[n_pad + k] = (split_live && k < live1.size()) ? live1[k] : (uint16_t)len;
+            dead += len - p->live_len[n_pad + k];
+        }
+        p->dead_edges = dead;
         lap("assemble");
         {
             const int64_t blocks = (int64_t)((vsrc.size() + (1u << 20) - 1) >> 20);
diff --git a/stract_amd/csrc/hb_internal.h b/stract_amd/csrc/hb_internal.h
--- a/stract_amd/csrc/hb_internal.h
+++ b/stract_amd/csrc/hb_internal.h
@@ -71,6 +71,8 @@
     uint64_t level1_rows = 0;
     uint64_t direct_edges = 0;
     uint64_t rows_with_in_edges = 0;
+    uvec<uint16_t> live_len;
+    uint64_t dead_edges = 0;
 };
 
 struct XcdQuota {
@@ -123,6 +125,19 @@
     }
 };
 
+enum : uint32_t { kColdDoubling = 0, kColdOneBand = 1, kColdFirstKept = 2 };
+constexpr uint32_t kColdRuleDefault = kColdOneBand;
+static constexpr uint32_t plan_band_of(uint32_t band_w, uint32_t warm_slices, uint32_t cold_rule, uint32_t idx)
+{
+    if (!band_w || idx < band_w) return 0;
+    const uint64_t j = (uint64_t)idx / band_w;
+    if (j <= warm_slices) return (uint32_t)j;
+    const uint64_t q = j / (warm_slices + 1u);
+    if (cold_rule == kColdOneBand) return warm_slices + 1u;
+    if (cold_rule == kColdFirstKept) return warm_slices + 1u + (q >= 2 ? 1u : 0u);
+    return warm_slices + 1u + (uint32_t)(63 - __builtin_clzll(q));
+}
+
 struct PlanTune {
     uint32_t chunk = kDefaultChunk;
     uint32_t band_w = 1u << 16;
@@ -130,6 +145,8 @@
     uint32_t direct_max = 0;
     bool xcd_map = true;
     uint32_t world = 1;
+    bool live_prefix = true;
+    uint32_t cold_rule = kColdRuleDefault;
 };
 
 std::string ingest_edges(const hb_u128 *node_ids, uint64_t n, const hb_edge *edges, uint64_t m,
@@ -207,6 +224,7 @@
     uint32_t *d_dev_of = nullptr;
     uint32_t *d_outdeg_dev = nullptr;
     uint64_t m_global = 0;
+    uint16_t *d_live_len = nullptr;
 };
 std::string device_offsets(void *stream, uint32_t *d_counts, uint64_t count, uint64_t *d_offsets, uint64_t expect);
 std::string device_prefix(void *stream, const uint32_t *d_counts, uint64_t count, uint64_t *d_offsets);
diff --git a/stract_amd/csrc/hb_kernels.hip.h b/stract_amd/csrc/hb_kernels.hip.h
--- a/stract_amd/csrc/hb_kernels.hip.h
+++ b/stract_amd/csrc/hb_kernels.hip.h
@@ -69,6 +69,7 @@
     const uint32_t *virt_rows;
     uint32_t xflags;
     const uint16_t *self_jp;
+    const uint16_t *live_len;
 };
 
 
@@ -151,6 +152,8 @@
     };
     uint64_t nbeg = 0, nend = 0;
     uint32_t nod = 0;
+    uint32_t nlive = 0;
+    const bool by_live = !INIT && p.live_len != nullptr;
     uint32_t nvirt = 0;
     uint4 nself = make_uint4(0, 0, 0, 0);
     const bool by_bitmap = INIT && p.virt_rows != nullptr;
@@ -164,6 +167,7 @@
         if (tile0 < ntiles && r0 < row_hi) {
             nbeg = p.row_ptr[r0];
             nend = p.row_ptr[r0 + 1];
+            if (!INIT && by_live) nlive = (uint32_t)p.live_len[r0];
             if (REAL && FUSED) nod = p.outdeg[r0];
             if (kDenseReal) nself = own_counter(r0);
             if (INIT && by_bitmap) nvirt = (p.virt_rows[r0 >> 5] >> (r0 & 31u)) & 1u;
@@ -173,7 +177,14 @@
         const uint64_t row16 = row_lo + (tile << 6) + ((uint64_t)wave << 4);
         const uint64_t row = row16 + (uint64_t)g;
         const bool valid = row < row_hi;
-        const uint64_t beg = nbeg, end = nend;
+        const uint64_t beg = nbeg;
+        uint64_t end = nend;
+        uint32_t dead = 0;
+        if (!INIT && by_live) {
+            HB_DBG_ASSERT(beg + nlive <= end);
+            dead = (uint32_t)(end - beg) - nlive;
+            end = beg + nlive;
+        }
         const uint32_t od = nod;
         const uint32_t virt = nvirt;
         uint4 selfv = nself;
@@ -181,11 +192,13 @@
             const uint64_t nrow = row + (tstride << 6);
             nbeg = nend = 0;
             nod = 0;
+            nlive = 0;
             nvirt = 0;
             nself = make_uint4(0, 0, 0, 0);
             if (tile + tstride < ntiles && nrow < row_hi) {
                 nbeg = p.row_ptr[nrow];
                 nend = p.row_ptr[nrow + 1];
+                if (!INIT && by_live) nlive = (uint32_t)p.live_len[nrow];
                 if (REAL && FUSED) nod = p.outdeg[nrow];
                 if (kDenseReal) nself = own_counter(nrow);
                 if (INIT && by_bitmap) nvirt = (p.virt_rows[nrow >> 5] >> (nrow & 31u)) & 1u;
@@ -217,6 +230,8 @@
         Acc acc;
         acc_zero(acc);
         if (kDenseReal && valid) acc_merge(acc, selfv);
+        if (!REAL && !INIT && dead && beg < end) acc_merge(acc, p.part[(row - p.n_pad) * 4 + q]);
+        if (STATS && !INIT && dead && q == 0) cnt_active += dead;
         if (beg < end) {
             uint32_t first;
             bool real_src;
@@ -302,7 +317,7 @@
         const uint32_t kd16 = (REAL && FUSED) ? (uint32_t)((const uint16_t *)p.kdirty)[row16 >> 4] : 0u;
         const bool self_prev = (prev16 >> g) & 1u;
         const bool kd = (kd16 >> g) & 1u;
-        const bool need = valid;
+        const bool need = valid && (REAL || INIT || !dead || beg < end);
         const uint4 accv = acc_value(acc);
         const bool lane_diff = need && (!REAL || u4_ne(accv, selfv));
         const uint64_t bal = __ballot(lane_diff);
diff --git a/stract_amd/csrc/hb_plan.hip b/stract_amd/csrc/hb_plan.hip
--- a/stract_amd/csrc/hb_plan.hip
+++ b/stract_amd/csrc/hb_plan.hip
@@ -148,14 +148,42 @@
 struct BandParams {
     uint32_t band_w;
     uint32_t warm_slices;
+    uint32_t cold_rule;
 };
-__device__ __forceinline__ uint32_t band_of(const BandParams bp, uint32_t idx)
-{
-    if (!bp.band_w || idx < bp.band_w) return 0;
-    const uint64_t j = (uint64_t)idx / bp.band_w;
-    if (j <= bp.warm_slices) return (uint32_t)j;
-    const uint64_t q = j / (bp.warm_slices + 1u);
-    return bp.warm_slices + 1u + (uint32_t)(63 - __clzll((long long)q));
+__device__ __forceinline__ uint32_t band_of(const BandParams bp, uint32_t idx) { return hb::plan_band_of(bp.band_w, bp.warm_slices, bp.cold_rule, idx); }
+
+__device__ __forceinline__ uint32_t quad_fill_live_first(const uint32_t *list, uint32_t len, const uint64_t *deg, uint32_t *dst)
+{
+    const int lane = threadIdx.x & 63, q = lane & 3, q0 = lane & ~3;
+    uint32_t live = 0;
+    for (uint32_t i = q; i < len; i += 4) live += deg[list[i]] != 0;
+    live += __shfl_xor(live, 1);
+    live += __shfl_xor(live, 2);
+    uint32_t nl = 0, nd = live;
+    for (uint32_t i0 = 0; __ballot(i0 < len) != 0; i0 += 4) {
+        const uint32_t i = i0 + q;
+        const bool in = i < len;
+        const uint32_t s = in ? list[i] : 0u;
+        const uint32_t f = (in && deg[s] != 0) ? 1u : 0u, d = (in && !f) ? 1u : 0u;
+        uint32_t fb = 0, db = 0, ft = 0, dt = 0;
+#pragma unroll
+        for (int k = 0; k < 4; k++) {
+            const uint32_t fk = __shfl(f, q0 + k), dk = __shfl(d, q0 + k);
+            if (k < q) {
+                fb += fk;
+                db += dk;
+            }
+            ft += fk;
+            dt += dk;
+        }
+        PL_DBG_ASSERT(!f || nl + fb < live);
+        PL_DBG_ASSERT(!d || (nd + db >= live && nd + db < len));
+        if (f) dst[nl + fb] = s;
+        if (d) dst[nd + db] = s;
+        nl += ft;
+        nd += dt;
+    }
+    return live;
 }
 
 __global__ __launch_bounds__(256) void order_keys_kernel(const uint32_t *outdeg, uint64_t n, uint64_t world, uint64_t *key, uint32_t *val)
@@ -369,7 +397,7 @@
 }
 __global__ __launch_bounds__(256) void level1_fill_kernel(const uint32_t *row_chunk, uint64_t rows, const uint64_t *vrow_ptr, const uint64_t *cbeg,
                                                           const uint32_t *clen, const uint32_t *rs, uint64_t slice, uint64_t world, uint32_t *vsrc,
-                                                          uint64_t m, uint64_t C, uint64_t vsrc_cap)
+                                                          uint64_t m, uint64_t C, uint64_t vsrc_cap, const uint64_t *deg, uint16_t *live1)
 {
     const uint64_t t = (uint64_t)blockIdx.x * 256 + threadIdx.x;
     const uint64_t r = t >> 2;
@@ -385,6 +413,11 @@
     (void)m;
     (void)C;
     (void)vsrc_cap;
+    if (live1) {
+        const uint32_t live = quad_fill_live_first(rs + b, len, deg, vsrc + o);
+        if (q == 0) live1[r] = (uint16_t)live;
+        return;
+    }
     for (uint32_t i = q; i < len; i += 4) {
         const uint64_t hr = rs[b + i];
         vsrc[o + i] = (uint32_t)(world == 1 ? hr : (hr % world) * slice + hr / world);
@@ -445,7 +478,7 @@
 }
 __global__ __launch_bounds__(256) void real_fill_kernel(const uint64_t *row_ptr, const uint8_t *is_split, const uint32_t *hub_index, const uint64_t *lptr,
                                                         const uint32_t *lids, const uint64_t *rp, const uint32_t *rs, uint64_t n_pad, uint64_t slice,
-                                                        uint64_t world, uint32_t *src)
+                                                        uint64_t world, uint32_t *src, const uint64_t *deg, uint16_t *live_len, int split_live)
 {
     const uint64_t t = (uint64_t)blockIdx.x * 256 + threadIdx.x;
     const uint64_t d = t >> 2;
@@ -455,13 +488,32 @@
     if (is_split[d]) {
         const uint64_t b = lptr[hub_index[d]];
         for (uint64_t i = q; i < len; i += 4) src[o + i] = lids[b + i];
+        if (q == 0) live_len[d] = (uint16_t)len;
+    } else if (split_live) {
+        const uint32_t live = quad_fill_live_first(rs + rp[d], (uint32_t)len, deg, src + o);
+        if (q == 0) live_len[d] = (uint16_t)live;
     } else {
         const uint64_t b = rp[d];
         for (uint64_t i = q; i < len; i += 4) {
             const uint64_t hr = rs[b + i];
             src[o + i] = (uint32_t)(world == 1 ? hr : (hr % world) * slice + hr / world);
         }
-    }
+        if (q == 0) live_len[d] = (uint16_t)len;
+    }
+}
+__global__ __launch_bounds__(256) void virtual_live_kernel(const uint32_t *vlen, const uint16_t *live1, uint64_t rows_l1, uint64_t nv, uint16_t *live_tail)
+{
+    const uint64_t k = (uint64_t)blockIdx.x * 256 + threadIdx.x;
+    if (k < nv) live_tail[k] = (live1 && k < rows_l1) ? live1[k] : (uint16_t)vlen[k];
+}
+__global__ __launch_bounds__(256) void dead_edges_kernel(const uint64_t *row_ptr, const uint16_t *live_len, uint64_t rows_total, unsigned long long *dead)
+{
+    unsigned long long acc = 0;
+    for (uint64_t r = (uint64_t)blockIdx.x * 256 + threadIdx.x; r < rows_total; r += (uint64_t)gridDim.x * 256)
+        acc += (row_ptr[r + 1] - row_ptr[r]) - (uint64_t)live_len[r];
+#pragma unroll
+    for (int off = 32; off > 0; off >>= 1) acc += __shfl_down(acc, off);
+    if ((threadIdx.x & 63) == 0 && acc) atomicAdd(dead, acc);
 }
 __global__ __launch_bounds__(256) void virtual_row_ptr_kernel(const uint64_t *vrow_ptr, uint64_t nv, uint64_t real_total, uint64_t *row_ptr_tail)
 {
@@ -751,6 +803,7 @@
     p->level_begin.clear();
     decltype(p->row_ptr)().swap(p->row_ptr);
     decltype(p->src)().swap(p->src);
+    decltype(p->live_len)().swap(p->live_len);
     uint64_t m = 0;
     if (n) PL_HIP(hipMemcpyAsync(&m, d_row_ptr_in + n, sizeof(uint64_t), hipMemcpyDeviceToHost, stream));
     PL_HIP(hipStreamSynchronize(stream));
@@ -883,7 +936,7 @@
     lap("relabel + sort rows");
 
     const uint32_t warm_slices = tune.xcd_map ? 64u : 0u;
-    const BandParams bp{tune.band_w, warm_slices};
+    const BandParams bp{tune.band_w, warm_slices, tune.cold_rule};
     uint32_t *d_hub_rows = nullptr;
     uint64_t *d_cnt = nullptr;
     PL_HIP(mem.alloc(&d_hub_rows, n_pad + 1));
@@ -1062,10 +1115,16 @@
     const uint64_t vsrc_cap = l1_edges + rows_l1 + rows_l1 / 8 + 64ull * kRowAlign;
     uint32_t *d_vsrc = nullptr;
     PL_HIP(mem.alloc(&d_vsrc, vsrc_cap + 1));
+    const bool split_live = world == 1 && tune.live_prefix;
+    uint16_t *d_live1 = nullptr;
+    if (split_live) {
+        PL_HIP(mem.alloc(&d_live1, rows_l1 + 1));
+        PL_HIP(hipMemsetAsync(d_live1, 0, (rows_l1 + 1) * sizeof(uint16_t), stream));
+    }
     if (rows_l1) {
         hipLaunchKernelGGL(level1_fill_kernel, dim3(grid_for(rows_l1 * 4)), dim3(256), 0, stream, (const uint32_t *)d_row_chunk, rows_l1,
                            (const uint64_t *)d_vrow_ptr, (const uint64_t *)d_cbeg, (const uint32_t *)d_clen, (const uint32_t *)d_rs, slice, world, d_vsrc, m, C,
-                           vsrc_cap);
+                           vsrc_cap, (const uint64_t *)d_deg, d_live1);
         PL_HIP(hipGetLastError());
         PL_HIP(hipStreamSynchronize(stream));
     }
@@ -1167,17 +1226,34 @@
     PL_HIP(hipGetLastError());
     const uint64_t src_len = real_total + vsrc_len;
     uint32_t *d_src = nullptr;
+    uint16_t *d_live_len = nullptr;
     PL_HIP(mem.alloc_out(&d_src, src_len + 4));
+    PL_HIP(mem.alloc_out(&d_live_len, rows_total + 64));
     if (n_pad) {
         hipLaunchKernelGGL(real_fill_kernel, dim3(grid_for(n_pad * 4)), dim3(256), 0, stream, (const uint64_t *)d_row_ptr, (const uint8_t *)d_is_split,
                            (const uint32_t *)d_hub_index, (const uint64_t *)d_lptr, (const uint32_t *)d_lids, (const uint64_t *)d_rp,
-                           (const uint32_t *)d_rs, n_pad, slice, world, d_src);
-        PL_HIP(hipGetLastError());
+                           (const uint32_t *)d_rs, n_pad, slice, world, d_src, (const uint64_t *)d_deg, d_live_len, split_live ? 1 : 0);
+        PL_HIP(hipGetLastError());
+    }
+    if (nv) {
+        hipLaunchKernelGGL(virtual_live_kernel, dim3(grid_for(nv)), dim3(256), 0, stream, (const uint32_t *)d_vlen, (const uint16_t *)d_live1, rows_l1, nv,
+                           d_live_len + n_pad);
+        PL_HIP(hipGetLastError());
+    }
+    p->dead_edges = 0;
+    if (rows_total) {
+        PL_HIP(hipMemsetAsync(d_sums, 0, sizeof(unsigned long long), stream));
+        hipLaunchKernelGGL(dead_edges_kernel, dim3((unsigned)std::min<uint64_t>(grid_for(rows_total), 2048)), dim3(256), 0, stream, (const uint64_t *)d_row_ptr,
+                           (const uint16_t *)d_live_len, rows_total, d_sums);
+        PL_HIP(hipGetLastError());
+        PL_HIP(hipMemcpyAsync(h_sums, d_sums, sizeof(unsigned long long), hipMemcpyDeviceToHost, stream));
     }
     if (vsrc_len) PL_HIP(hipMemcpyAsync(d_src + real_total, d_vsrc, vsrc_len * sizeof(uint32_t), hipMemcpyDeviceToDevice, stream));
     PL_HIP(hipStreamSynchronize(stream));
+    if (rows_total) p->dead_edges = h_sums[0];
     lap("assemble");
 
+    out->d_live_len = (uint16_t *)mem.disown(d_live_len);
     out->d_row_ptr = (uint64_t *)mem.disown(d_row_ptr);
     out->d_src = (uint32_t *)mem.disown(d_src);
     out->src_len = src_len;
```

Measured after the change: 111.7 (median of 2 runs). No clear change (+0.2%).
